# serycjon/MFT

Hardware: AMD Instinct MI355X
Metric: tracked frames/sec at 512x512, 12 RAFT iters; flow EPE vs reference (higher is better)
Workload: dtype f32 (update-block products as split fp16 x 3 on the fp16 matrix cores, fp32 accumulation; error per product <= ~2^-23, see DESIGN.md section 4 and parity below); 1 GPU; MFT.track on synthetic 512x512 video, deltas [inf,1,2,4,8,16,32], 7/7.00/7 (min/mean/max) flow pairs per timed frame, 12 RAFT iters, seeded synthetic weights (BASELINE.json configs[1]); parallelism=single GPU, frames_resident_in_hbm=True, preroll_frames=32

## Files before the change

include/mftx.h:

```cpp
#ifndef MFTX_H
#define MFTX_H

#include <stddef.h>
#include <stdint.h>

#ifdef __cplusplus
extern "C" {
#endif

#define MFTX_VERSION 400

#define MFTX_E_ARG (-1)
#define MFTX_E_ALIGN (-2)
#define MFTX_E_WORKSPACE (-3)
#define MFTX_E_STATE (-4)

#define MFTX_MAX_CANDIDATES 16

int mftx_version(void);
const char *mftx_last_error_string(void);

#define MFTX_PROFILE_CATEGORIES 14
int mftx_profile_begin(void);
int mftx_profile_end(double *ms, double *work, long long *count, int n);

int mftx_corr_pyramid(const float *f1, const float *f2, int P, int C, int h, int w,
                      float *lvl0, float *lvl1, float *lvl2, float *lvl3, void *stream);
int mftx_corr_pyramid_split(const float *f1, const float *f2, int P, int C, int h, int w,
                            float *lvl0, float *lvl1, float *lvl2, float *lvl3, float *f2_scratch, void *stream);
int mftx_corr_pyramid_layout(int h, int w, long long *stride, int *block_grid);

int mftx_corr_lookup(const float *lvl0, const float *lvl1, const float *lvl2, const float *lvl3,
                     const float *coords, int P, int h, int w, int r,
                     float *out, int ld_out, void *stream);

#define MFTX_LOOKUP_CONVC1_WEIGHT_BYTES 393216
int mftx_pack_lookup_convc1_weights(const float *wpk, int ld_w, void *wfused, void *stream);
int mftx_corr_lookup_convc1(const float *lvl0, const float *lvl1, const float *lvl2, const float *lvl3,
                            const float *coords, int P, int h, int w, const void *wfused, const float *bias,
                            float *out, int ld_out, int out_split, void *stream);

#define MFTX_FLOW_BRANCH_WEIGHT_BYTES 352256
int mftx_pack_flow_branch_weights(const float *w98, const float *w2pk, void *wflow, void *stream);
int mftx_flow_branch(const float *coords, int P, int h, int w, const void *wflow, const float *b1, const float *b2,
                     float *out, int ld_out, float *hx, int ld_hx, void *stream);

int mftx_fmap_pyramid(const float *f2, int P, int C, int h, int w, float *lvl1, float *lvl2, float *lvl3, void *stream);
int mftx_corr_lookup_ondemand(const float *f1, const float *f2l0, const float *f2l1, const float *f2l2, const float *f2l3,
                              const float *coords, int P, int C, int h, int w, int r,
                              float *out, int ld_out, void *stream);

typedef struct mftx_conv_desc {
    const float *a0; int lda0; int c0;
    const float *a1; int lda1; int c1;
    const float *wpk; const float *bias;
    float *out; int ldo;
    int P, h, w;
    int N;
    int kh, kw;
    int act;
    float out_scale;
    const float *addend; int ld_addend;
    int stride, hin, win, pad_y, pad_x, residual_mode;
    int arith;
    int a_split, out_split;
} mftx_conv_desc;
#define MFTX_ARITH_F32 0
#define MFTX_ARITH_SPLIT 1
int mftx_conv2d(const mftx_conv_desc *d, void *stream);
int mftx_conv2d_tile(const mftx_conv_desc *d, int tile, void *stream);

int mftx_pack_tile_conv_weights(const float *wpk, int N, int taps, int cin, int cin_pad, void *wtile, void *stream);
int mftx_tile_conv2d(const mftx_conv_desc *d, const void *wtile, void *stream);
#define MFTX_OU_HEADS_WTILE_BYTES 6635520
int mftx_pack_ou_heads_weights(const float *w1pk, int cin_pad, const float *w2pk, void *wtile, void *wproj, void *stream);
int mftx_ou_heads(const float *a_split, int lda, int P, int h, int w, const void *wtile, const float *b1, const void *wproj, const float *b2,
                  float *T, float *out, int ld_out, void *stream);
int mftx_gru_half(const float *h_in, int ld_hin, const float *motion, int ld_mo, const void *wzr, const void *wq, const float *pre_zr,
                  const float *pre_q, float *z, const float *hf_in, float *hf_out, float *h_out, int ld_hout, int P, int h, int w, int pass,
                  void *stream);
int mftx_tile_conv_fills_chip(int P, int h, int w);
#define MFTX_FLOW_HEAD_WEIGHT_BYTES 32768
int mftx_pack_flow_head_weights(const float *w2pk, void *wproj, void *stream);
int mftx_flow_head(const float *hsplit, int ld_h, int P, int h, int w, const void *wtile, const float *b1, const void *wproj,
                   const float *b2, float *T, float *delta, float *coords, void *stream);
int mftx_split_weights(const float *wpk, void *out, long long n_floats, void *stream);
#define MFTX_SPLIT_LIMIT 65504.0f
int mftx_count_not_below(const float *x, long long n, float limit, unsigned *count, void *stream);

typedef struct mftx_raft mftx_raft;
#define MFTX_RAFT_NUM_WEIGHTS 34
int mftx_raft_create(const float *const *weights, int n_weights, mftx_raft **out);
void mftx_raft_destroy(mftx_raft *r);
size_t mftx_raft_workspace_bytes(int P, int h, int w);
int mftx_raft_set_ondemand(mftx_raft *r, int on);
int mftx_raft_set_split_weights(mftx_raft *r, const void *const *split, int n);
int mftx_raft_arith(const mftx_raft *r);
int mftx_raft_set_lookup_fused(mftx_raft *r, const void *wfused);
int mftx_raft_set_flow_fused(mftx_raft *r, const void *wflow);
int mftx_raft_set_tile_weights(mftx_raft *r, const void *const *tile, int n);
int mftx_raft_set_flow_head(mftx_raft *r, const void *wproj);
int mftx_raft_set_ou_heads(mftx_raft *r, const void *wtile, const void *wproj);
int mftx_raft_set_coords_trace(mftx_raft *r, float *trace);
#define MFTX_RAFT_OPT_FORK 0
#define MFTX_RAFT_OPT_PRESPLIT 1
#define MFTX_RAFT_OPT_GROUP 2
#define MFTX_RAFT_OPT_FUSE_LOOKUP 3
#define MFTX_RAFT_OPT_GRAPH 4
#define MFTX_RAFT_OPT_FUSE_FLOW 5
#define MFTX_RAFT_OPT_TILE_CONV 6
#define MFTX_RAFT_OPT_FUSE_HEAD 7
#define MFTX_RAFT_OPT_TILE_VOLUME 8
#define MFTX_RAFT_OPT_FUSE_GRU 9
#define MFTX_RAFT_OPT_TILE_CELLS 10
#define MFTX_RAFT_OPT_FUSE_OU 11
#define MFTX_RAFT_OPT_TILE_CONV2P 12
int mftx_raft_set_option(mftx_raft *r, int option, int value);
#define MFTX_RAFT_PLAN_FIELDS 14
#define MFTX_FLOW_FUSED 0
#define MFTX_FLOW_SIDE 1
#define MFTX_FLOW_FIRST 2
#define MFTX_FLOW_AFTER_LOOKUP 3
#define MFTX_FLOW_WITH_LOOKUP 4
int mftx_raft_plan(const mftx_raft *r, int P, int h, int w, int ctx_supplied, int *out, int n);
int mftx_raft_set_nonfinite_counter(mftx_raft *r, unsigned *counter);
int mftx_raft_clear_graphs(mftx_raft *r);
int mftx_raft_graph_stats(const mftx_raft *r, unsigned long long *captures, unsigned long long *replays);
size_t mftx_raft_workspace_bytes_for(const mftx_raft *r, int P, int h, int w);
int mftx_raft_workspace_layout(int P, int h, int w, size_t *offsets, int n);
int mftx_raft_workspace_layout_for(const mftx_raft *r, int P, int h, int w, size_t *offsets, int n);
int mftx_raft_refine(mftx_raft *r, int P, int h, int w, int iters,
                     const float *fmap1, const float *fmap2, const float *net, const float *inp,
                     const float *flow_init,
                     int pad_left, int pad_right, int pad_top, int pad_bottom,
                     float *flow, float *occl, float *sigma, float *packed, float *flow_lr,
                     void *workspace, size_t workspace_bytes, void *stream);
int mftx_raft_refine_gather(mftx_raft *r, int P, int h, int w, int iters, const float *const *fmap1,
                            const float *const *fmap2, const float *const *net, const float *const *inp,
                            const float *flow_init, int pad_left, int pad_right, int pad_top, int pad_bottom,
                            float *flow, float *occl, float *sigma, float *packed, float *flow_lr_out,
                            void *workspace, size_t workspace_bytes, void *stream);
size_t mftx_raft_frame_prepare_bytes(int h, int w);
int mftx_raft_frame_prepare(mftx_raft *r, int h, int w, const float *fmap, const float *inp, float *ctx_zr1, float *ctx_q1,
                            float *ctx_zr2, float *ctx_q2, void *fmap_split, void *scratch, size_t scratch_bytes, void *stream);
int mftx_raft_refine_gather_ex(mftx_raft *r, int P, int h, int w, int iters, const float *const *fmap1,
                               const float *const *fmap2, const float *const *net, const float *const *inp,
                               const float *const *ctx_parts, const void *const *fmap1_split, const void *fmap2_split,
                               const float *flow_init, int pad_left, int pad_right, int pad_top, int pad_bottom,
                               float *flow, float *occl, float *sigma, float *packed, float *flow_lr_out,
                               void *workspace, size_t workspace_bytes, void *stream);
int mftx_volume_query_split(const float *in, void *out, long long n_floats, void *stream);

typedef struct mftx_encoder mftx_encoder;
int mftx_encoder_create(const float *const *weights, int n_weights, int instance_norm, mftx_encoder **out);
int mftx_encoder_set_split_weights(mftx_encoder *e, const void *const *split, int n);
int mftx_encoder_set_graph(mftx_encoder *e, int on);
void mftx_encoder_destroy(mftx_encoder *e);
size_t mftx_encoder_workspace_bytes(int H0, int W0);
int mftx_encoder_forward(mftx_encoder *e, const uint8_t *img, int H0, int W0, float *out0, float *out1,
                         void *workspace, size_t workspace_bytes, void *stream);
int mftx_encoder_prep(const uint8_t *img, int H0, int W0, float *out, void *stream);
size_t mftx_instance_norm_workspace_bytes(int C);
int mftx_instance_norm(float *x, int rows, int C, const float *res, int mode, int split, void *workspace,
                       size_t workspace_bytes, void *stream);

int mftx_convex_upsample(const float *flow_lr, const float *ou, int ld_ou, const float *mask,
                         int P, int h, int w,
                         int pad_left, int pad_right, int pad_top, int pad_bottom,
                         float *flow, float *occl, float *sigma, float *packed, void *stream);

int mftx_chain(const float *flowL, const float *occlL, const float *sigmaL,
               const float *flowR, const float *occlR, const float *sigmaR,
               int H, int W, float *flowO, float *occlO, float *sigmaO, void *stream);

int mftx_warp_backward(const float *flow, const float *img, int C, int H, int W, float *out, void *stream);

int mftx_select(int K, const float *const *flow, const float *const *occl, const float *const *sigma,
                float thr, int H, int W,
                float *flowO, float *occlO, float *sigmaO, int8_t *chosen, void *stream);

int mftx_chain_select(int K,
                      const float *const *flowL, const float *const *occlL, const float *const *sigmaL,
                      const float *const *flowR, const float *const *occlR, const float *const *sigmaR,
                      float thr, int H, int W,
                      float *flowO, float *occlO, float *sigmaO, int8_t *chosen, void *stream);

int mftx_chain_select_packed(int K,
                             const float *const *flowL, const float *const *occlL, const float *const *sigmaL,
                             const float *const *packedR,
                             float thr, int H, int W,
                             float *flowO, float *occlO, float *sigmaO, int8_t *chosen, void *stream);

int mftx_chain_select_multi(int T, const int *K,
                            const float *const *flowL, const float *const *occlL, const float *const *sigmaL,
                            const float *const *packedR,
                            float thr, int H, int W,
                            float *const *flowO, float *const *occlO, float *const *sigmaO, int8_t *const *chosen,
                            void *stream);

int mftx_sample_points(int T, const float *const *flow, const float *const *occl, const float *const *sigma,
                       int H, int W, int N, const int *tmpl, const float *xy,
                       float *table, long long row_stride, int column, void *stream);

#define MFTX_SPLAT_F32 0
#define MFTX_SPLAT_U8 1
int mftx_splat_forward(const float *flow, const void *img, int img_dtype, const uint8_t *mask, int C, int H, int W,
                       int S, int V, long long *acc, void *stream);

int mftx_splat_resolve(long long *acc, int C, int H, int W, int V, float fill, int clear, float *out, void *stream);

int mftx_overlay_edit(const float *flow, const float *occl, const uint8_t *edit, const uint8_t *frame, int H, int W,
                      int S, float alpha_div, long long *acc, uint8_t *out, void *stream);

int mftx_overlay_dots(const uint8_t *frame, uint8_t *out, int H, int W, const float *table, long long row_stride,
                      int N, double radius, int b, int g, int r, void *stream);

size_t mftx_quantize_workspace_bytes(void);
int mftx_quantize_u16(const float *x, long long n, uint16_t *q, float *lohi,
                      void *workspace, size_t workspace_bytes, void *stream);
int mftx_dequantize_u16(const uint16_t *q, long long n, float lo, float hi, float *x, void *stream);

size_t mftx_trackstore_workspace_bytes(void);
int mftx_trackstore_append(const float *flow, const float *occl, const float *sigma, int H, int W,
                           uint16_t *packed, float *lohi, void *workspace, size_t workspace_bytes, void *stream);

size_t mftx_trackstore_append_multi_workspace_bytes(int T);
int mftx_trackstore_append_multi(int T, const float *const *flow, const float *const *occl, const float *const *sigma,
                                 int H, int W, uint16_t *const *packed, float *const *lohi,
                                 void *workspace, size_t workspace_bytes, void *stream);

int mftx_trackstore_unpack(const uint16_t *packed, const float *lohi, int H, int W,
                           float *flow, float *occl, float *sigma, void *stream);

int mftx_trackstore_query(const uint16_t *const *chunks, const float *const *lohi_chunks, int n_chunks, int frames_per_chunk,
                          const int *slots, int T, int H, int W, int N, const float *xy,
                          float *table, long long row_stride, int column0, void *stream);

int mftx_trackstore_locate(const uint16_t *const *frames, const float *const *lohis, const int *group_start, int G,
                           const int *order, const int *group_of, int H, int W, int N, const float *xy,
                           float occlusion_threshold, unsigned long long *keys, float *table, int *cell, void *stream);

int mftx_trackstore_invert(const uint16_t *const *frames, const float *const *lohis, int G, int H, int W,
                           float occlusion_threshold, unsigned long long *keys ,
                           float *table, int *cell, void *stream);

int mftx_trackstore_invert_atlas(const uint16_t *const *frames, const float *const *lohis, const int *first_of ,
                                 const int *rank_of , int G, int J, int H, int W, float occlusion_threshold,
                                 unsigned long long *keys , float *table, int *cell, int *entry, void *stream);

int mftx_copy_bytes(const void *src, void *dst, long long n, void *stream);

int mftx_png_unfilter(uint8_t *rows, int height, int row_bytes, int bpp);

#ifdef __cplusplus
}
#endif
#endif
```

mft_amd/_lib.py:

```python
from __future__ import annotations

import ctypes as C
import os
from pathlib import Path

_HERE = Path(__file__).resolve().parent
LIB_PATH = _HERE / "libmftx.so"

MAX_CANDIDATES = 16
NUM_RAFT_WEIGHTS = 34
LOOKUP_CONVC1_WEIGHT_BYTES = 393216
FLOW_BRANCH_WEIGHT_BYTES = 352256
FLOW_HEAD_WEIGHT_BYTES = 32768
OU_HEADS_WTILE_BYTES = 6635520
SPLIT_LIMIT = 65504.0


class ConvDesc(C.Structure):
    _fields_ = [("a0", C.c_void_p), ("lda0", C.c_int), ("c0", C.c_int),
                ("a1", C.c_void_p), ("lda1", C.c_int), ("c1", C.c_int),
                ("wpk", C.c_void_p), ("bias", C.c_void_p),
                ("out", C.c_void_p), ("ldo", C.c_int),
                ("P", C.c_int), ("h", C.c_int), ("w", C.c_int),
                ("N", C.c_int), ("kh", C.c_int), ("kw", C.c_int),
                ("act", C.c_int), ("out_scale", C.c_float),
                ("addend", C.c_void_p), ("ld_addend", C.c_int),
                ("stride", C.c_int), ("hin", C.c_int), ("win", C.c_int), ("pad_y", C.c_int), ("pad_x", C.c_int),
                ("residual_mode", C.c_int), ("arith", C.c_int), ("a_split", C.c_int), ("out_split", C.c_int)]


_PP = C.POINTER(C.c_void_p)

SIGNATURES = {
    "mftx_version": (C.c_int, []),
    "mftx_last_error_string": (C.c_char_p, []),
    "mftx_profile_begin": (C.c_int, []),
    "mftx_profile_end": (C.c_int, [C.POINTER(C.c_double), C.POINTER(C.c_double), C.POINTER(C.c_longlong), C.c_int]),
    "mftx_corr_pyramid": (C.c_int, [C.c_void_p, C.c_void_p, C.c_int, C.c_int, C.c_int, C.c_int,
                                    C.c_void_p, C.c_void_p, C.c_void_p, C.c_void_p, C.c_void_p]),
    "mftx_corr_pyramid_split": (C.c_int, [C.c_void_p, C.c_void_p, C.c_int, C.c_int, C.c_int, C.c_int,
                                          C.c_void_p, C.c_void_p, C.c_void_p, C.c_void_p, C.c_void_p, C.c_void_p]),
    "mftx_corr_pyramid_layout": (C.c_int, [C.c_int, C.c_int, C.POINTER(C.c_longlong), C.POINTER(C.c_int)]),
    "mftx_corr_lookup": (C.c_int, [C.c_void_p] * 5 + [C.c_int] * 4 + [C.c_void_p, C.c_int, C.c_void_p]),
    "mftx_fmap_pyramid": (C.c_int, [C.c_void_p] + [C.c_int] * 4 + [C.c_void_p] * 4),
    "mftx_corr_lookup_ondemand": (C.c_int, [C.c_void_p] * 6 + [C.c_int] * 5 + [C.c_void_p, C.c_int, C.c_void_p]),
    "mftx_raft_set_ondemand": (C.c_int, [C.c_void_p, C.c_int]),
    "mftx_raft_workspace_bytes_for": (C.c_size_t, [C.c_void_p, C.c_int, C.c_int, C.c_int]),
    "mftx_conv2d": (C.c_int, [C.POINTER(ConvDesc), C.c_void_p]),
    "mftx_conv2d_tile": (C.c_int, [C.POINTER(ConvDesc), C.c_int, C.c_void_p]),
    "mftx_encoder_set_split_weights": (C.c_int, [C.c_void_p, _PP, C.c_int]),
    "mftx_raft_set_split_weights": (C.c_int, [C.c_void_p, _PP, C.c_int]),
    "mftx_raft_arith": (C.c_int, [C.c_void_p]),
    "mftx_raft_set_lookup_fused": (C.c_int, [C.c_void_p, C.c_void_p]),
    "mftx_raft_set_flow_fused": (C.c_int, [C.c_void_p, C.c_void_p]),
    "mftx_raft_set_tile_weights": (C.c_int, [C.c_void_p, _PP, C.c_int]),
    "mftx_raft_set_flow_head": (C.c_int, [C.c_void_p, C.c_void_p]),
    "mftx_raft_set_ou_heads": (C.c_int, [C.c_void_p, C.c_void_p, C.c_void_p]),
    "mftx_pack_ou_heads_weights": (C.c_int, [C.c_void_p, C.c_int, C.c_void_p, C.c_void_p, C.c_void_p, C.c_void_p]),
    "mftx_ou_heads": (C.c_int, [C.c_void_p, C.c_int, C.c_int, C.c_int, C.c_int, C.c_void_p, C.c_void_p, C.c_void_p, C.c_void_p, C.c_void_p,
                                C.c_void_p, C.c_int, C.c_void_p]),
    "mftx_pack_flow_head_weights": (C.c_int, [C.c_void_p, C.c_void_p, C.c_void_p]),
    "mftx_flow_head": (C.c_int, [C.c_void_p, C.c_int, C.c_int, C.c_int, C.c_int] + [C.c_void_p] * 8),
    "mftx_pack_tile_conv_weights": (C.c_int, [C.c_void_p, C.c_int, C.c_int, C.c_int, C.c_int, C.c_void_p, C.c_void_p]),
    "mftx_tile_conv2d": (C.c_int, [C.POINTER(ConvDesc), C.c_void_p, C.c_void_p]),
    "mftx_pack_flow_branch_weights": (C.c_int, [C.c_void_p, C.c_void_p, C.c_void_p, C.c_void_p]),
    "mftx_flow_branch": (C.c_int, [C.c_void_p, C.c_int, C.c_int, C.c_int, C.c_void_p, C.c_void_p, C.c_void_p, C.c_void_p,
                                   C.c_int, C.c_void_p, C.c_int, C.c_void_p]),
    "mftx_raft_set_option": (C.c_int, [C.c_void_p, C.c_int, C.c_int]),
    "mftx_raft_plan": (C.c_int, [C.c_void_p, C.c_int, C.c_int, C.c_int, C.c_int, C.POINTER(C.c_int), C.c_int]),
    "mftx_raft_set_coords_trace": (C.c_int, [C.c_void_p, C.c_void_p]),
    "mftx_gru_half": (C.c_int, [C.c_void_p, C.c_int, C.c_void_p, C.c_int, C.c_void_p, C.c_void_p, C.c_void_p, C.c_void_p, C.c_void_p, C.c_void_p,
                                C.c_void_p, C.c_void_p, C.c_int, C.c_int, C.c_int, C.c_int, C.c_int, C.c_void_p]),
    "mftx_tile_conv_fills_chip": (C.c_int, [C.c_int, C.c_int, C.c_int]),
    "mftx_raft_clear_graphs": (C.c_int, [C.c_void_p]),
    "mftx_raft_set_nonfinite_counter": (C.c_int, [C.c_void_p, C.c_void_p]),
    "mftx_raft_graph_stats": (C.c_int, [C.c_void_p, C.POINTER(C.c_ulonglong), C.POINTER(C.c_ulonglong)]),
    "mftx_pack_lookup_convc1_weights": (C.c_int, [C.c_void_p, C.c_int, C.c_void_p, C.c_void_p]),
    "mftx_corr_lookup_convc1": (C.c_int, [C.c_void_p] * 5 + [C.c_int] * 3 + [C.c_void_p, C.c_void_p, C.c_void_p,
                                                                            C.c_int, C.c_int, C.c_void_p]),
    "mftx_split_weights": (C.c_int, [C.c_void_p, C.c_void_p, C.c_longlong, C.c_void_p]),
    "mftx_count_not_below": (C.c_int, [C.c_void_p, C.c_longlong, C.c_float, C.c_void_p, C.c_void_p]),
    "mftx_raft_create": (C.c_int, [_PP, C.c_int, C.POINTER(C.c_void_p)]),
    "mftx_raft_destroy": (None, [C.c_void_p]),
    "mftx_raft_workspace_bytes": (C.c_size_t, [C.c_int, C.c_int, C.c_int]),
    "mftx_raft_workspace_layout": (C.c_int, [C.c_int, C.c_int, C.c_int, C.POINTER(C.c_size_t), C.c_int]),
    "mftx_raft_workspace_layout_for": (C.c_int, [C.c_void_p, C.c_int, C.c_int, C.c_int, C.POINTER(C.c_size_t), C.c_int]),
    "mftx_raft_refine": (C.c_int, [C.c_void_p, C.c_int, C.c_int, C.c_int, C.c_int,
                                   C.c_void_p, C.c_void_p, C.c_void_p, C.c_void_p, C.c_void_p,
                                   C.c_int, C.c_int, C.c_int, C.c_int,
                                   C.c_void_p, C.c_void_p, C.c_void_p, C.c_void_p, C.c_void_p,
                                   C.c_void_p, C.c_size_t, C.c_void_p]),
    "mftx_raft_refine_gather": (C.c_int, [C.c_void_p, C.c_int, C.c_int, C.c_int, C.c_int,
                                          _PP, _PP, _PP, _PP, C.c_void_p,
                                          C.c_int, C.c_int, C.c_int, C.c_int,
                                          C.c_void_p, C.c_void_p, C.c_void_p, C.c_void_p, C.c_void_p,
                                          C.c_void_p, C.c_size_t, C.c_void_p]),
    "mftx_raft_refine_gather_ex": (C.c_int, [C.c_void_p, C.c_int, C.c_int, C.c_int, C.c_int,
                                             _PP, _PP, _PP, _PP, _PP, _PP, C.c_void_p, C.c_void_p,
                                             C.c_int, C.c_int, C.c_int, C.c_int,
                                             C.c_void_p, C.c_void_p, C.c_void_p, C.c_void_p, C.c_void_p,
                                             C.c_void_p, C.c_size_t, C.c_void_p]),
    "mftx_raft_frame_prepare_bytes": (C.c_size_t, [C.c_int, C.c_int]),
    "mftx_raft_frame_prepare": (C.c_int, [C.c_void_p, C.c_int, C.c_int] + [C.c_void_p] * 8 + [C.c_size_t, C.c_void_p]),
    "mftx_volume_query_split": (C.c_int, [C.c_void_p, C.c_void_p, C.c_longlong, C.c_void_p]),
    "mftx_encoder_create": (C.c_int, [_PP, C.c_int, C.c_int, C.POINTER(C.c_void_p)]),
    "mftx_encoder_destroy": (None, [C.c_void_p]),
    "mftx_encoder_set_graph": (C.c_int, [C.c_void_p, C.c_int]),
    "mftx_encoder_workspace_bytes": (C.c_size_t, [C.c_int, C.c_int]),
    "mftx_encoder_forward": (C.c_int, [C.c_void_p, C.c_void_p, C.c_int, C.c_int, C.c_void_p, C.c_void_p,
                                       C.c_void_p, C.c_size_t, C.c_void_p]),
    "mftx_encoder_prep": (C.c_int, [C.c_void_p, C.c_int, C.c_int, C.c_void_p, C.c_void_p]),
    "mftx_instance_norm_workspace_bytes": (C.c_size_t, [C.c_int]),
    "mftx_instance_norm": (C.c_int, [C.c_void_p, C.c_int, C.c_int, C.c_void_p, C.c_int, C.c_int, C.c_void_p, C.c_size_t, C.c_void_p]),
    "mftx_convex_upsample": (C.c_int, [C.c_void_p, C.c_void_p, C.c_int, C.c_void_p] + [C.c_int] * 7
                             + [C.c_void_p] * 5),
    "mftx_chain": (C.c_int, [C.c_void_p] * 6 + [C.c_int, C.c_int] + [C.c_void_p] * 4),
    "mftx_warp_backward": (C.c_int, [C.c_void_p, C.c_void_p, C.c_int, C.c_int, C.c_int, C.c_void_p, C.c_void_p]),
    "mftx_select": (C.c_int, [C.c_int, _PP, _PP, _PP, C.c_float, C.c_int, C.c_int] + [C.c_void_p] * 5),
    "mftx_chain_select": (C.c_int, [C.c_int] + [_PP] * 6 + [C.c_float, C.c_int, C.c_int] + [C.c_void_p] * 5),
    "mftx_chain_select_packed": (C.c_int, [C.c_int] + [_PP] * 4 + [C.c_float, C.c_int, C.c_int] + [C.c_void_p] * 5),
    "mftx_chain_select_multi": (C.c_int, [C.c_int, C.POINTER(C.c_int)] + [_PP] * 4 + [C.c_float, C.c_int, C.c_int] + [_PP] * 4
                                + [C.c_void_p]),
    "mftx_sample_points": (C.c_int, [C.c_int, _PP, _PP, _PP, C.c_int, C.c_int, C.c_int, C.c_void_p, C.c_void_p,
                                     C.c_void_p, C.c_longlong, C.c_int, C.c_void_p]),
    "mftx_splat_forward": (C.c_int, [C.c_void_p, C.c_void_p, C.c_int, C.c_void_p, C.c_int, C.c_int, C.c_int, C.c_int, C.c_int,
                                     C.c_void_p, C.c_void_p]),
    "mftx_splat_resolve": (C.c_int, [C.c_void_p, C.c_int, C.c_int, C.c_int, C.c_int, C.c_float, C.c_int, C.c_void_p, C.c_void_p]),
    "mftx_overlay_edit": (C.c_int, [C.c_void_p, C.c_void_p, C.c_void_p, C.c_void_p, C.c_int, C.c_int, C.c_int, C.c_float,
                                    C.c_void_p, C.c_void_p, C.c_void_p]),
    "mftx_overlay_dots": (C.c_int, [C.c_void_p, C.c_void_p, C.c_int, C.c_int, C.c_void_p, C.c_longlong, C.c_int, C.c_double,
                                    C.c_int, C.c_int, C.c_int, C.c_void_p]),
    "mftx_quantize_workspace_bytes": (C.c_size_t, []),
    "mftx_quantize_u16": (C.c_int, [C.c_void_p, C.c_longlong, C.c_void_p, C.c_void_p, C.c_void_p, C.c_size_t, C.c_void_p]),
    "mftx_dequantize_u16": (C.c_int, [C.c_void_p, C.c_longlong, C.c_float, C.c_float, C.c_void_p, C.c_void_p]),
    "mftx_trackstore_workspace_bytes": (C.c_size_t, []),
    "mftx_trackstore_append": (C.c_int, [C.c_void_p, C.c_void_p, C.c_void_p, C.c_int, C.c_int, C.c_void_p, C.c_void_p,
                                         C.c_void_p, C.c_size_t, C.c_void_p]),
    "mftx_trackstore_append_multi_workspace_bytes": (C.c_size_t, [C.c_int]),
    "mftx_trackstore_append_multi": (C.c_int, [C.c_int, _PP, _PP, _PP, C.c_int, C.c_int, _PP, _PP, C.c_void_p, C.c_size_t,
                                               C.c_void_p]),
    "mftx_trackstore_invert_atlas": (C.c_int, [C.c_void_p, C.c_void_p, C.c_void_p, C.c_void_p, C.c_int, C.c_int, C.c_int, C.c_int,
                                               C.c_float, C.c_void_p, C.c_void_p, C.c_void_p, C.c_void_p, C.c_void_p]),
    "mftx_trackstore_unpack": (C.c_int, [C.c_void_p, C.c_void_p, C.c_int, C.c_int, C.c_void_p, C.c_void_p, C.c_void_p,
                                         C.c_void_p]),
    "mftx_trackstore_query": (C.c_int, [_PP, _PP, C.c_int, C.c_int, C.c_void_p, C.c_int, C.c_int, C.c_int, C.c_int, C.c_void_p,
                                        C.c_void_p, C.c_longlong, C.c_int, C.c_void_p]),
    "mftx_trackstore_locate": (C.c_int, [C.c_void_p, C.c_void_p, C.c_void_p, C.c_int, C.c_void_p, C.c_void_p, C.c_int, C.c_int,
                                         C.c_int, C.c_void_p, C.c_float, C.c_void_p, C.c_void_p, C.c_void_p, C.c_void_p]),
    "mftx_trackstore_invert": (C.c_int, [C.c_void_p, C.c_void_p, C.c_int, C.c_int, C.c_int, C.c_float, C.c_void_p, C.c_void_p,
                                         C.c_void_p, C.c_void_p]),
    "mftx_png_unfilter":(C.c_int, [C.c_void_p, C.c_int, C.c_int, C.c_int]),
    "mftx_copy_bytes": (C.c_int, [C.c_void_p, C.c_void_p, C.c_longlong, C.c_void_p]),
}

_lib = None


class MftxError(RuntimeError):
    pass


def load():
    global _lib
    if _lib is not None:
        return _lib
    path = Path(os.environ.get("MFTX_LIB", LIB_PATH))
    if not path.exists():
        raise MftxError(f"{path} not found: build it with `python -c 'import __graft_entry__ as g; g.build()'` "
                        "(there is no CPU fallback for the MFT hot path)")
    lib = C.CDLL(str(path))
    for name, (res, args) in SIGNATURES.items():
        fn = getattr(lib, name)
        fn.restype = res
        fn.argtypes = args
    _lib = lib
    return lib


def check(code, what):
    if code != 0:
        msg = load().mftx_last_error_string().decode(errors="replace")
        raise MftxError(f"{what} failed ({code}): {msg}")


def ptr_array(ptrs):
    arr = (C.c_void_p * len(ptrs))(*ptrs)
    return C.cast(arr, _PP), arr
```

mft_amd/csrc/flow_branch.hip:

```cpp
#include "common.h"
#include "profile.h"
#include "device_prims.h"

namespace mftx {

constexpr int FB_TH = 8, FB_TW = 16;
constexpr int FB_HW = FB_TW + 2;
constexpr int FB_HCELLS = (FB_TH + 2) * FB_HW;
constexpr int FB_CELL = 528;
constexpr int FB_FCOLS = 26;
constexpr int FB_FROW = 28;
constexpr int FB_OFF_FLOW = 192 * FB_CELL;
constexpr int FB_FLOW_BYTES = 4 * 2 * 16 * FB_FROW * 4;
constexpr int FB_RED_ROW = 68;
constexpr int FB_LDS = 4 * 128 * FB_RED_ROW * 4;
static_assert(FB_OFF_FLOW + FB_FLOW_BYTES <= FB_LDS, "stage 3 is the largest user of LDS");
constexpr unsigned FB_W1_BYTES = 7 * 4 * 2 * 1024;
constexpr unsigned FB_W2_BYTES = 2 * 4 * 18 * 2 * 1024;
constexpr unsigned FB_WBYTES = FB_W1_BYTES + FB_W2_BYTES;

#ifdef MFTX_LF_TRACE
__device__ unsigned long long fb_trace_buf[8][16];
#define FB_T(code) do { if (blockIdx.x == 0 && tcount < 16) { unsigned long long t_; asm volatile("s_memtime %0\n\ts_waitcnt lgkmcnt(0)" : "=s"(t_) :: "memory"); \
                        if ((threadIdx.x & 63) == 0) fb_trace_buf[threadIdx.x >> 6][tcount] = ((unsigned long long)(code) << 56) | (t_ & 0x00ffffffffffffffull); ++tcount; } } while (0)
#else
#define FB_T(code) do { } while (0)
#endif

struct FlowBranchArgs {
    const float *coords;
    const void *wf;
    const float *b1, *b2;
    float *out; int ld_out;
    float *hx; int ld_hx;
    const float *T, *b2h;
    float *coords_out, *delta_out;
    int P, h, w, tiles_x, tiles_y;
};

__global__ __launch_bounds__(512, 2) void flow_branch_kernel(FlowBranchArgs p) {
    extern __shared__ __attribute__((aligned(16))) unsigned char fb_lds[];
    unsigned char *lds = fb_lds;
    const int tid = (int)threadIdx.x, lane = tid & 63, wv = __builtin_amdgcn_readfirstlane(tid >> 6);
    const int tile = (int)blockIdx.x;
    const int tx_ = tile % p.tiles_x, ty_ = (tile / p.tiles_x) % p.tiles_y, img = tile / (p.tiles_x * p.tiles_y);
    const int x0 = tx_ * FB_TW, y0 = ty_ * FB_TH;
    const long long img_base = (long long)img * p.h * p.w;
    const float k2048 = __builtin_bit_cast(float, __builtin_amdgcn_readfirstlane(0x45000000));
    const uint4 *__restrict__ wf = reinterpret_cast<const uint4 *>(p.wf);
#ifdef MFTX_LF_TRACE
    int tcount = 0;
#endif
    FB_T(1);

    const int j1 = wv & 3;
    f16x8 w1h[7], w1l[7];
#pragma unroll
    for (int g = 0; g < 7; ++g) {
        const uint4 *src = wf + ((g * 4 + j1) * 2) * 64 + lane;
        w1h[g] = __builtin_bit_cast(f16x8, src[0]);
        w1l[g] = __builtin_bit_cast(f16x8, src[64]);
    }
    f32x4 bias1[4];
#pragma unroll
    for (int b = 0; b < 4; ++b) bias1[b] = *reinterpret_cast<const f32x4 *>(p.b1 + 32 * j1 + 8 * b + 4 * (lane >> 5));

    unsigned *fsp = reinterpret_cast<unsigned *>(lds + FB_OFF_FLOW);
    if (tid < 16 * FB_FCOLS) {
        const int r = tid / FB_FCOLS, c = tid - r * FB_FCOLS;
        const int yy = y0 - 4 + r, xx = x0 - 4 + c;
        float2 f = make_float2(0.f, 0.f);
        unsigned hw = 0u, lw = 0u;
        if (yy >= 0 && yy < p.h && xx >= 0 && xx < p.w) {
            const long long cell = img_base + (long long)yy * p.w + xx;
            float2 cd = *reinterpret_cast<const float2 *>(p.coords + 2 * cell);
            if (p.T) {
                float sx = 0.f, sy = 0.f;
#pragma unroll
                for (int dy = 0; dy < 3; ++dy)
#pragma unroll
                    for (int dx = 0; dx < 3; ++dx) {
                        const int ny = yy + dy - 1, nx = xx + dx - 1;
                        if (ny >= 0 && ny < p.h && nx >= 0 && nx < p.w) {
                            const float2 t = *reinterpret_cast<const float2 *>(p.T + (cell + (long long)(dy - 1) * p.w + (dx - 1)) * 18 + 2 * (3 * dy + dx));
                            sx += t.x;
                            sy += t.y;
                        }
                    }
                const float dlx = sx + p.b2h[0], dly = sy + p.b2h[1];
                cd.x += dlx;
                cd.y += dly;
                if (r >= 4 && r < 4 + FB_TH && c >= 4 && c < 4 + FB_TW) {
                    *reinterpret_cast<float2 *>(p.coords_out + 2 * cell) = cd;
                    *reinterpret_cast<float2 *>(p.delta_out + 2 * cell) = make_float2(dlx, dly);
                }
            }
            f.x = cd.x - (float)xx;
            f.y = cd.y - (float)yy;
            const unsigned sx = split_halves(f.x), sy = split_halves(f.y);
            hw = (sx & 0xffffu) | (sy << 16);
            lw = (sx >> 16) | (sy & 0xffff0000u);
            if (p.hx && r >= 4 && r < 4 + FB_TH && c >= 4 && c < 4 + FB_TW) {
                char *dst = reinterpret_cast<char *>(p.hx + cell * p.ld_hx) + split_row_offset(382);
                *reinterpret_cast<unsigned *>(dst) = hw;
                *reinterpret_cast<unsigned *>(dst + 16) = lw;
            }
        }
#pragma unroll
        for (int sft = 0; sft < 4; ++sft) {
            if (c >= sft) {
                fsp[((sft * 2 + 0) * 16 + r) * FB_FROW + c - sft] = hw;
                fsp[((sft * 2 + 1) * 16 + r) * FB_FROW + c - sft] = lw;
            }
            if (c >= FB_FCOLS - 4 && c - sft + 4 < FB_FROW) {
                fsp[((sft * 2 + 0) * 16 + r) * FB_FROW + c - sft + 4] = 0u;
                fsp[((sft * 2 + 1) * 16 + r) * FB_FROW + c - sft + 4] = 0u;
            }
        }
    }
    FB_T(2);
    lds_barrier();
    FB_T(3);

    const float inv2048 = 1.f / 2048.f;
    {
#pragma unroll 1
        for (int mi = 0; mi < 3; ++mi) {
            const int i = (wv >> 2) + 2 * mi;
            const int m = 32 * i + (lane & 31), mc = m < FB_HCELLS ? m : FB_HCELLS - 1;
            const int ry = mc / FB_HW, rx = mc - ry * FB_HW;
            const int c0 = rx + 4 * (lane >> 5), sft = c0 & 3;
            const unsigned char *arow = lds + FB_OFF_FLOW + (((sft * 2) * 16 + ry) * FB_FROW + (c0 - sft)) * 4;
            const unsigned padmask = (lane >> 5) ? 0u : 0xffffffffu;
            f32x16 acc1, accx1;
#pragma unroll
            for (int r = 0; r < 16; ++r) { acc1[r] = 0.f; accx1[r] = 0.f; }
            u32x4 ahw[7], alw[7];
#pragma unroll
            for (int g = 0; g < 7; ++g) {
                ahw[g] = *reinterpret_cast<const u32x4 *>(arow + g * FB_FROW * 4);
                alw[g] = *reinterpret_cast<const u32x4 *>(arow + (16 + g) * FB_FROW * 4);
            }
#pragma unroll
            for (int g = 0; g < 7; ++g) {
                ahw[g][3] &= padmask;
                alw[g][3] &= padmask;
                const f16x8 ah = __builtin_bit_cast(f16x8, ahw[g]), al = __builtin_bit_cast(f16x8, alw[g]);
                acc1 = mfma_f16(w1h[g], ah, acc1);
                accx1 = mfma_f16(w1l[g], ah, accx1);
                accx1 = mfma_f16(w1h[g], al, accx1);
            }
            FB_T(4);
            const int yy = y0 - 1 + ry, xx = x0 - 1 + rx;
            const unsigned keep = (m < FB_HCELLS && yy >= 0 && yy < p.h && xx >= 0 && xx < p.w) ? 0xffffffffu : 0u;
            unsigned char *cellp = lds + m * FB_CELL + (4 * j1) * 32 + (lane >> 5) * 8;
#pragma unroll
            for (int b = 0; b < 4; ++b) {
                float v[4];
#pragma unroll
                for (int e = 0; e < 4; ++e) {
                    const float t = acc1[4 * b + e] + accx1[4 * b + e] * inv2048 + bias1[b][e];
                    v[e] = (t + __builtin_fabsf(t)) * 0.5f;
                }
                unsigned h0, l0, h1, l1;
                split_pair(v[0], v[1], k2048, h0, l0);
                split_pair(v[2], v[3], k2048, h1, l1);
                *reinterpret_cast<uint2 *>(cellp + b * 32) = make_uint2(h0 & keep, h1 & keep);
                *reinterpret_cast<uint2 *>(cellp + b * 32 + 16) = make_uint2(l0 & keep, l1 & keep);
            }
            FB_T(5);
        }
    }
    lds_barrier();
    FB_T(6);

    const int nt = wv & 1, kq = wv >> 1;
    const uint4 *__restrict__ w2 = wf + FB_W1_BYTES / 16 + (nt * 4 + kq) * 18 * 128 + lane;
    f32x16 acc[4], accx[4];
#pragma unroll
    for (int i = 0; i < 4; ++i)
#pragma unroll
        for (int r = 0; r < 16; ++r) { acc[i][r] = 0.f; accx[i][r] = 0.f; }
    const unsigned char *abase[4];
    {
        const int r = lane & 31;
#pragma unroll
        for (int i = 0; i < 4; ++i)
            abase[i] = lds + ((2 * i + (r >> 4)) * FB_HW + (r & 15)) * FB_CELL + (lane >> 5) * 32 + kq * 128;
    }
    constexpr int PF = 3;
    uint4 bq[PF][2];
#pragma unroll
    for (int s = 0; s < PF; ++s) { bq[s][0] = w2[s * 128]; bq[s][1] = w2[s * 128 + 64]; }
    f16x8 ah[2][4], al[2][4];
    auto read_a = [&](int s, int set) {
        const int tap = s >> 1, gg = s & 1;
        const int off = ((tap / 3) * FB_HW + tap % 3) * FB_CELL + gg * 64;
#pragma unroll
        for (int i = 0; i < 4; ++i) {
            ah[set][i] = *reinterpret_cast<const f16x8 *>(abase[i] + off);
            al[set][i] = *reinterpret_cast<const f16x8 *>(abase[i] + off + 16);
        }
    };
    read_a(0, 0);
#pragma unroll
    for (int s = 0; s < 18; ++s) {
        const int set = s & 1;
        const f16x8 bh = __builtin_bit_cast(f16x8, bq[s % PF][0]), bl = __builtin_bit_cast(f16x8, bq[s % PF][1]);
        __builtin_amdgcn_sched_barrier(0);
        if (s + 1 < 18) read_a(s + 1, set ^ 1);
        if (s + PF < 18) { bq[s % PF][0] = w2[(s + PF) * 128]; bq[s % PF][1] = w2[(s + PF) * 128 + 64]; }
        __builtin_amdgcn_sched_barrier(0);
#pragma unroll
        for (int i = 0; i < 4; ++i) acc[i] = mfma_f16(bh, ah[set][i], acc[i]);
#pragma unroll
        for (int i = 0; i < 4; ++i) accx[i] = mfma_f16(bl, ah[set][i], accx[i]);
#pragma unroll
        for (int i = 0; i < 4; ++i) accx[i] = mfma_f16(bh, al[set][i], accx[i]);
        __builtin_amdgcn_sched_barrier(0);
    }
    FB_T(7);
    lds_barrier();

    float *red = reinterpret_cast<float *>(lds);
#pragma unroll
    for (int i = 0; i < 4; ++i)
#pragma unroll
        for (int b = 0; b < 4; ++b) {
            f32x4 v;
#pragma unroll
            for (int e = 0; e < 4; ++e) v[e] = acc[i][4 * b + e] + accx[i][4 * b + e] * inv2048;
            *reinterpret_cast<f32x4 *>(red + (kq * 128 + 32 * i + (lane & 31)) * FB_RED_ROW + 32 * nt + 8 * b + 4 * (lane >> 5)) = v;
        }
    FB_T(8);
    lds_barrier();
    FB_T(9);
#pragma unroll
    for (int it = 0; it < 2; ++it) {
        const int item = tid + 512 * it, m = item >> 3, g8 = item & 7;
        const int yy = y0 + (m >> 4), xx = x0 + (m & 15);
        const float *src = red + m * FB_RED_ROW + 8 * g8;
        f32x4 u = *reinterpret_cast<const f32x4 *>(src), v = *reinterpret_cast<const f32x4 *>(src + 4);
#pragma unroll
        for (int q = 1; q < 4; ++q) {
            u += *reinterpret_cast<const f32x4 *>(src + q * 128 * FB_RED_ROW);
            v += *reinterpret_cast<const f32x4 *>(src + q * 128 * FB_RED_ROW + 4);
        }
        const f32x4 bu = *reinterpret_cast<const f32x4 *>(p.b2 + 8 * g8), bv = *reinterpret_cast<const f32x4 *>(p.b2 + 8 * g8 + 4);
#pragma unroll
        for (int e = 0; e < 4; ++e) { u[e] = relu_keep_nan(u[e] + bu[e]); v[e] = relu_keep_nan(v[e] + bv[e]); }
        f16x8 hi, lo;
        split8(u, v, k2048, hi, lo);
        if (yy < p.h && xx < p.w) {
            const long long cell = img_base + (long long)yy * p.w + xx;
            uint4 *dst = reinterpret_cast<uint4 *>(reinterpret_cast<char *>(p.out + cell * p.ld_out) + g8 * 32);
            dst[0] = __builtin_bit_cast(uint4, hi);
            dst[1] = __builtin_bit_cast(uint4, lo);
        }
    }
    FB_T(10);
}

#ifdef MFTX_LF_TRACE
extern "C" int mftx_debug_fb_trace(unsigned long long *out) {
    if (hipMemcpyFromSymbol(out, HIP_SYMBOL(fb_trace_buf), sizeof(unsigned long long) * 8 * 16) != hipSuccess) return -1;
    unsigned long long z[8 * 16] = {};
    return hipMemcpyToSymbol(HIP_SYMBOL(fb_trace_buf), z, sizeof z) == hipSuccess ? 0 : -1;
}
#endif

__global__ void pack_flow_branch_kernel(const float *__restrict__ w98, const float *__restrict__ w2pk, uint4 *__restrict__ out) {
    const int idx = (int)(blockIdx.x * blockDim.x + threadIdx.x);
    const int n1 = (int)(FB_W1_BYTES / 16), n2 = (int)(FB_W2_BYTES / 16);
    if (idx >= n1 + n2) return;
    float v[8];
    int part;
    if (idx < n1) {
        const int lane = idx & 63, j = (idx >> 7) & 3, g = idx >> 9;
        part = (idx >> 6) & 1;
        const int n = 32 * j + (lane & 31);
#pragma unroll
        for (int e = 0; e < 8; ++e) {
            const int s = 8 * (lane >> 5) + e;
            v[e] = s < 14 ? w98[(g * 14 + s) * 128 + n] : 0.f;
        }
    } else {
        const int k = idx - n1;
        const int lane = k & 63, step = (k >> 7) % 18, kq = ((k >> 7) / 18) & 3, nt = (k >> 7) / 72;
        part = (k >> 6) & 1;
        const int tap = step >> 1, g = 2 * kq + (step & 1);
        const int n = 32 * nt + (lane & 31);
#pragma unroll
        for (int e = 0; e < 8; ++e) v[e] = w2pk[((long long)n * 9 + tap) * 128 + 16 * g + 8 * (lane >> 5) + e];
    }
    unsigned w[4];
#pragma unroll
    for (int e = 0; e < 4; ++e) {
        const unsigned a = split_halves(v[2 * e]), b = split_halves(v[2 * e + 1]);
        w[e] = part ? ((a >> 16) | (b & 0xffff0000u)) : ((a & 0xffffu) | (b << 16));
    }
    out[idx] = make_uint4(w[0], w[1], w[2], w[3]);
}

int launch_pack_flow_branch(const float *w98, const float *w2pk, void *out, hipStream_t s) {
    const int n = (int)(FB_WBYTES / 16);
    hipLaunchKernelGGL(pack_flow_branch_kernel, dim3((n + 255) / 256), dim3(256), 0, s, w98, w2pk, reinterpret_cast<uint4 *>(out));
    return check_launch("pack_flow_branch");
}

int launch_flow_branch(const float *coords, int P, int h, int w, const void *wf, const float *b1, const float *b2, float *out,
                       int ld_out, float *hx, int ld_hx, hipStream_t s, const float *T, const float *b2h, float *coords_out, float *delta_out) {
    if (T && (!b2h || !coords_out || !delta_out || coords_out == coords || (reinterpret_cast<uintptr_t>(T) & 7) || (reinterpret_cast<uintptr_t>(coords_out) & 7) ||
              (reinterpret_cast<uintptr_t>(delta_out) & 7)))
        return fail(MFTX_E_ARG, "flow_branch: a pending flow-head update needs its bias, a SECOND coordinate buffer and a delta buffer, 8-byte aligned");
    if (!coords || !wf || !b1 || !b2 || !out) return fail(MFTX_E_ARG, "flow_branch: null pointer");
    if (P <= 0 || h <= 0 || w <= 0) return fail(MFTX_E_ARG, "flow_branch: bad sizes");
    if (ld_out < 64 || ld_out % 8 || (reinterpret_cast<uintptr_t>(out) & 31) || (hx && (ld_hx < 384 || ld_hx % 8 || (reinterpret_cast<uintptr_t>(hx) & 31))))
        return fail(MFTX_E_ALIGN, "flow_branch: split-form rows are 32-byte aligned with strides in multiples of 8");
    if (!aligned16(wf) || !aligned16(b2) || (reinterpret_cast<uintptr_t>(coords) & 7)) return fail(MFTX_E_ALIGN, "flow_branch: weights / bias / coordinates misaligned");
    FlowBranchArgs a{coords, wf, b1, b2, out, ld_out, hx, ld_hx, T, b2h, coords_out, delta_out, P, h, w, cdiv(w, FB_TW), cdiv(h, FB_TH)};
    const long long tiles = (long long)P * a.tiles_x * a.tiles_y;
    if (tiles > 0x7fffffffLL) return fail(MFTX_E_ARG, "flow_branch: too many tiles");
    static bool attr_set = false;
    if (!attr_set) {
        if (hipFuncSetAttribute(reinterpret_cast<const void *>(flow_branch_kernel), hipFuncAttributeMaxDynamicSharedMemorySize, FB_LDS) != hipSuccess)
            return fail(MFTX_E_STATE, "flow_branch: cannot reserve %d bytes of LDS", FB_LDS);
        attr_set = true;
    }
    ProfScope prof(PC_FLOW_FUSED, s, 2.0 * P * h * w * (98.0 * 128 + 1152.0 * 64));
    hipLaunchKernelGGL(flow_branch_kernel, dim3((unsigned)tiles), dim3(512), FB_LDS, s, a);
    return check_launch("flow_branch");
}

}
```

mft_amd/csrc/raft_engine.hip:

```cpp
#include "common.h"
#include "profile.h"
#include "motion_front.h"
#include "graph_cache.h"
#include <cstdlib>
#include <new>

namespace mftx {


struct InitGather { int on; PairPtrs netp, inpp; };
struct CtxTable { const float **table; const float *own[4]; int supplied; PairPtrs parts[4]; };
__global__ void init_state_kernel(const float *__restrict__ net, const float *__restrict__ inp,
                                  const float *__restrict__ flow_init, float *hx, float *hf, float *coords1, int M, int h,
                                  int w, InitGather ga, CtxTable ct) {
    const long long i = (long long)blockIdx.x * blockDim.x + threadIdx.x;
    if (i >= (long long)M * 64) return;
    if (ct.table != nullptr && i < (long long)(M / (h * w)) * 4) {
        const int b = (int)(i >> 2), k = (int)(i & 3);
        ct.table[i] = ct.supplied ? ct.parts[k].p[b] : ct.own[k] + (long long)b * h * w * ((k & 1) ? 128 : 256);
    }
    const int m = (int)(i >> 6), q = (int)(i & 63);
    if (ga.on) {
        const int b = m / (h * w);
        net = ga.netp.p[b] - (long long)b * h * w * 128;
        inp = ga.inpp.p[b] - (long long)b * h * w * 128;
    }
    const float4 v = (q < 32) ? reinterpret_cast<const float4 *>(net)[(long long)m * 32 + q]
                              : reinterpret_cast<const float4 *>(inp)[(long long)m * 32 + (q - 32)];
    if (hf != nullptr) {
        store_split4v(hx + (long long)m * 384, 4 * q, v);
        if (q < 32) reinterpret_cast<float4 *>(hf + (long long)m * 128)[q] = v;
    } else {
        reinterpret_cast<float4 *>(hx + (long long)m * 384)[q] = v;
    }
    if (q == 0) {
        const int rem = m % (h * w);
        float cx = (float)(rem % w), cy = (float)(rem / w);
        if (flow_init != nullptr) {
            cx += flow_init[2 * (long long)m];
            cy += flow_init[2 * (long long)m + 1];
        }
        coords1[2 * (long long)m] = cx;
        coords1[2 * (long long)m + 1] = cy;
    }
}

__global__ __launch_bounds__(256) void convf1_kernel(ConvF1Args q) {
    __shared__ __attribute__((aligned(16))) float patch[2][7][48];
    const int half = threadIdx.x >> 7;
    convf1_strip(q, blockIdx.x * 2 + half, patch[half], threadIdx.x & 127);
}

__global__ __launch_bounds__(256) void lookup_convf1_kernel(LookupArgs lp, ConvF1Args q, int lookup_blocks, int f1_blocks) {
    __shared__ __attribute__((aligned(16))) float patch[2][7][48];
    const int total = lookup_blocks + f1_blocks;
    const int b = blockIdx.x;
    const int f_lo = (int)((long long)b * f1_blocks / total), f_hi = (int)((long long)(b + 1) * f1_blocks / total);
    if (f_hi > f_lo) {
        const int half = threadIdx.x >> 7;
        convf1_strip(q, f_lo * 2 + half, patch[half], threadIdx.x & 127);
    } else {
        lookup_block_body<2>(lp, b - f_lo, lookup_blocks);
    }
}

__global__ void ou_gather_kernel(const float *__restrict__ hx, const float *__restrict__ corr, int ld_corr,
                                 const float *__restrict__ coords1, const float *__restrict__ delta,
                                 float *__restrict__ ouin, float *__restrict__ flow_lr, int M, int h, int w, int split) {
    const long long i = (long long)blockIdx.x * blockDim.x + threadIdx.x;
    if (i >= (long long)M * 178) return;
    const int m = (int)(i / 178), q = (int)(i - (long long)m * 178);
    float4 v;
    if (split) {
        if (q < 64) v = load_split4(hx + (long long)m * 384, 4 * q);
        else if (q < 145) v = reinterpret_cast<const float4 *>(corr + (long long)m * ld_corr)[q - 64];
        else if (q == 145) {
            const int rem = m % (h * w);
            const float fx = coords1[2 * (long long)m] - (float)(rem % w);
            const float fy = coords1[2 * (long long)m + 1] - (float)(rem / w);
            v = make_float4(fx, fy, delta[2 * (long long)m], delta[2 * (long long)m + 1]);
            flow_lr[2 * (long long)m] = fx;
            flow_lr[2 * (long long)m + 1] = fy;
        } else v = load_split4(hx + (long long)m * 384 + 256, 4 * (q - 146));
        store_split4v(ouin + (long long)m * 712, 4 * q, v);
        return;
    }
    if (q < 64) v = reinterpret_cast<const float4 *>(hx + (long long)m * 384)[q];
    else if (q < 145) v = reinterpret_cast<const float4 *>(corr + (long long)m * ld_corr)[q - 64];
    else if (q == 145) {
        const int rem = m % (h * w);
        const float fx = coords1[2 * (long long)m] - (float)(rem % w);
        const float fy = coords1[2 * (long long)m + 1] - (float)(rem / w);
        v = make_float4(fx, fy, delta[2 * (long long)m], delta[2 * (long long)m + 1]);
        flow_lr[2 * (long long)m] = fx;
        flow_lr[2 * (long long)m + 1] = fy;
    } else v = reinterpret_cast<const float4 *>(hx + (long long)m * 384 + 256)[q - 146];
    reinterpret_cast<float4 *>(ouin + (long long)m * 712)[q] = v;
}

enum WeightSlot {
    W_CONVC1, B_CONVC1, W_CONVC2, B_CONVC2, W_CONVF1, B_CONVF1, W_CONVF2, B_CONVF2, W_CONV, B_CONV,
    W_ZR1_DYN, W_ZR1_INP, B_ZR1, W_Q1_DYN, W_Q1_INP, B_Q1, W_ZR2_DYN, W_ZR2_INP, B_ZR2, W_Q2_DYN, W_Q2_INP, B_Q2,
    W_FH1, B_FH1, W_FH2, B_FH2, W_MASK0, B_MASK0, W_MASK2, B_MASK2,
    W_OU1, B_OU1, W_OU2, B_OU2, W_COUNT
};

struct Workspace {
    float *lvl[4];
    float *f2l[3];
    float *coords1, *corr, *cor1, *corflo, *flo1, *hx, *z, *rh, *fh, *delta, *mask, *ouin, *ouh, *ou, *flow_lr;
    float *pre_zr[2], *pre_q[2];
    float *f2s;
    float *hf;
    float *hb, *hfb;
    const float **ctx;
    int ld_corr;
    size_t bytes;
};

static Workspace carve(void *base, int P, int h, int w, bool ondemand = false, bool split = false) {
    Workspace ws{};
    const size_t N = (size_t)h * w, M = (size_t)P * N;
    size_t off = 0;
    auto take = [&](size_t floats) {
        float *p = base ? reinterpret_cast<float *>(static_cast<char *>(base) + off) : nullptr;
        off += (floats * sizeof(float) + 255) & ~size_t(255);
        return p;
    };
    const PyramidLayout L = pyramid_layout(h, w);
    for (int l = 0; l < 4; ++l) ws.lvl[l] = take(ondemand ? 0 : M * (size_t)L.stride[l]);
    for (int l = 1; l < 4; ++l) ws.f2l[l - 1] = take(ondemand ? (size_t)P * (h >> l) * (w >> l) * 256 : 0);
    ws.coords1 = take(M * 2);
    ws.ld_corr = 324;
    ws.corr = take(M * ws.ld_corr);
    ws.cor1 = take(M * 256);
    ws.corflo = take(M * 256);
    ws.flo1 = take(M * 128);
    ws.hx = take(M * 384);
    ws.z = take(M * 128);
    ws.rh = take(M * 128);
    ws.fh = take(M * 256);
    ws.delta = take(M * 2);
    ws.mask = take(M * 576);
    ws.ouin = take(M * 712);
    ws.ouh = take(M * 256);
    ws.ou = take(M * 4);
    ws.flow_lr = take(M * 2);
    for (int pass = 0; pass < 2; ++pass) { ws.pre_zr[pass] = take(M * 256); ws.pre_q[pass] = take(M * 128); }
    ws.f2s = take(ondemand || !split ? 0 : M * 256);
    ws.hf = take(split ? M * 128 : 0);
    ws.hb = take(split ? M * 128 : 0);
    ws.hfb = take(split ? M * 128 : 0);
    ws.ctx = reinterpret_cast<const float **>(take(split ? (size_t)P * 8 : 0));
    ws.bytes = off;
    return ws;
}

}

using namespace mftx;

static constexpr uint32_t RAFT_MAGIC = 0x4d465458;
struct mftx_raft {
    uint32_t magic = RAFT_MAGIC;
    int ondemand = 0;
    int arith = MFTX_ARITH_F32;
    const float *w[W_COUNT] = {};
    const float *wg[W_COUNT] = {};
    hipStream_t side = nullptr;
    hipEvent_t ev_fork = nullptr, ev_join = nullptr;
    float *coords_trace = nullptr;
    GraphCache *graphs = nullptr;
    const void *wfused = nullptr;
    const void *wflow = nullptr;
    const void *wproj = nullptr;
    const void *wt[W_COUNT] = {};
    const void *wou = nullptr, *wouproj = nullptr;
    int opt[13] = { -1,  1,  1,  1,  1,  1,  1,
                    1,  1,  1,  0,  1,  1};
    unsigned *nonfinite = nullptr;
};
static_assert(MFTX_RAFT_OPT_TILE_CONV2P == 12, "mftx_raft::opt lists one default per option");
static constexpr int GEMM_SLOTS[] = {W_CONVC1, W_CONVC2, W_CONVF2, W_CONV, W_ZR1_DYN, W_ZR1_INP, W_Q1_DYN, W_Q1_INP,
                                     W_ZR2_DYN, W_ZR2_INP, W_Q2_DYN, W_Q2_INP, W_FH1, W_MASK0, W_MASK2, W_OU1};

extern "C" int mftx_raft_create(const float *const *weights, int n_weights, mftx_raft **out) {
    if (!weights || !out) return fail(MFTX_E_ARG, "raft_create: null pointer");
    if (n_weights != W_COUNT) return fail(MFTX_E_ARG, "raft_create: expected %d weight tensors, got %d", (int)W_COUNT, n_weights);
    for (int i = 0; i < W_COUNT; ++i) {
        if (!weights[i]) return fail(MFTX_E_ARG, "raft_create: weight %d is null", i);
        if (!aligned16(weights[i])) return fail(MFTX_E_ALIGN, "raft_create: weight %d not 16-byte aligned", i);
    }
    mftx_raft *r = new (std::nothrow) mftx_raft;
    if (!r) return fail(MFTX_E_ARG, "raft_create: out of host memory");
    r->graphs = new (std::nothrow) GraphCache;
    for (int i = 0; i < W_COUNT; ++i) r->w[i] = r->wg[i] = weights[i];
    *out = r;
    return 0;
}

extern "C" void mftx_raft_destroy(mftx_raft *r) {
    if (r && r->magic == RAFT_MAGIC) {
        r->magic = 0;
        if (r->ev_fork) (void)hipEventDestroy(r->ev_fork);
        if (r->ev_join) (void)hipEventDestroy(r->ev_join);
        if (r->side) (void)hipStreamDestroy(r->side);
        delete r->graphs;
        delete r;
    }
}

static int ensure_side_stream(mftx_raft *r) {
    if (r->side) return 0;
    hipError_t e = hipStreamCreateWithFlags(&r->side, hipStreamNonBlocking);
    if (e == hipSuccess) e = hipEventCreateWithFlags(&r->ev_fork, hipEventDisableTiming);
    if (e == hipSuccess) e = hipEventCreateWithFlags(&r->ev_join, hipEventDisableTiming);
    if (e != hipSuccess) return fail((int)e, "raft_refine: side stream: %s", hipGetErrorString(e));
    return 0;
}

extern "C" size_t mftx_raft_workspace_bytes(int P, int h, int w) {
    if (P <= 0 || h <= 0 || w <= 0) return 0;
    return carve(nullptr, P, h, w).bytes;
}

extern "C" int mftx_raft_set_ondemand(mftx_raft *r, int on) {
    if (!r || r->magic != RAFT_MAGIC) return fail(MFTX_E_STATE, "raft_set_ondemand: bad handle");
    r->ondemand = on ? 1 : 0;
    if (r->graphs) r->graphs->clear();
    return 0;
}

extern "C" int mftx_raft_set_split_weights(mftx_raft *r, const void *const *split, int n) {
    if (!r || r->magic != RAFT_MAGIC) return fail(MFTX_E_STATE, "raft_set_split_weights: bad handle");
    if (r->graphs) r->graphs->clear();
    if (!split) {
        for (int i = 0; i < W_COUNT; ++i) r->wg[i] = r->w[i];
        r->arith = MFTX_ARITH_F32;
        return 0;
    }
    if (n != W_COUNT) return fail(MFTX_E_ARG, "raft_set_split_weights: expected %d slots, got %d", (int)W_COUNT, n);
    for (int slot : GEMM_SLOTS) {
        if (!split[slot]) return fail(MFTX_E_ARG, "raft_set_split_weights: slot %d (a GEMM layer) is null", slot);
        if (!aligned16(split[slot])) return fail(MFTX_E_ALIGN, "raft_set_split_weights: slot %d not 16-byte aligned", slot);
    }
    for (int slot : GEMM_SLOTS) r->wg[slot] = static_cast<const float *>(split[slot]);
    r->arith = MFTX_ARITH_SPLIT;
    return 0;
}

extern "C" int mftx_raft_set_lookup_fused(mftx_raft *r, const void *wfused) {
    if (!r || r->magic != RAFT_MAGIC) return fail(MFTX_E_STATE, "raft_set_lookup_fused: bad handle");
    if (wfused && !aligned16(wfused)) return fail(MFTX_E_ALIGN, "raft_set_lookup_fused: weights not 16-byte aligned");
    r->wfused = wfused;
    if (r->graphs) r->graphs->clear();
    return 0;
}

extern "C" int mftx_raft_set_flow_fused(mftx_raft *r, const void *wflow) {
    if (!r || r->magic != RAFT_MAGIC) return fail(MFTX_E_STATE, "raft_set_flow_fused: bad handle");
    if (wflow && !aligned16(wflow)) return fail(MFTX_E_ALIGN, "raft_set_flow_fused: weights not 16-byte aligned");
    r->wflow = wflow;
    if (r->graphs) r->graphs->clear();
    return 0;
}

extern "C" int mftx_raft_set_tile_weights(mftx_raft *r, const void *const *tile, int n) {
    if (!r || r->magic != RAFT_MAGIC) return fail(MFTX_E_STATE, "raft_set_tile_weights: bad handle");
    if (r->graphs) r->graphs->clear();
    if (!tile) { for (int i = 0; i < W_COUNT; ++i) r->wt[i] = nullptr; return 0; }
    if (n != W_COUNT) return fail(MFTX_E_ARG, "raft_set_tile_weights: expected %d slots, got %d", (int)W_COUNT, n);
    for (int i = 0; i < W_COUNT; ++i)
        if (tile[i] && !aligned16(tile[i])) return fail(MFTX_E_ALIGN, "raft_set_tile_weights: slot %d not 16-byte aligned", i);
    for (int i = 0; i < W_COUNT; ++i) r->wt[i] = tile[i];
    return 0;
}

extern "C" int mftx_raft_set_flow_head(mftx_raft *r, const void *wproj) {
    if (!r || r->magic != RAFT_MAGIC) return fail(MFTX_E_STATE, "raft_set_flow_head: bad handle");
    if (wproj && !aligned16(wproj)) return fail(MFTX_E_ALIGN, "raft_set_flow_head: weights not 16-byte aligned");
    r->wproj = wproj;
    if (r->graphs) r->graphs->clear();
    return 0;
}

extern "C" int mftx_raft_set_ou_heads(mftx_raft *r, const void *wtile, const void *wproj) {
    if (!r || r->magic != RAFT_MAGIC) return fail(MFTX_E_STATE, "raft_set_ou_heads: bad handle");
    if ((wtile == nullptr) != (wproj == nullptr)) return fail(MFTX_E_ARG, "raft_set_ou_heads: both weight streams, or neither");
    if (wtile && (!aligned16(wtile) || !aligned16(wproj))) return fail(MFTX_E_ALIGN, "raft_set_ou_heads: weights not 16-byte aligned");
    r->wou = wtile; r->wouproj = wproj;
    if (r->graphs) r->graphs->clear();
    return 0;
}

extern "C" int mftx_raft_set_coords_trace(mftx_raft *r, float *trace) {
    if (!r || r->magic != RAFT_MAGIC) return fail(MFTX_E_STATE, "raft_set_coords_trace: bad handle");
    r->coords_trace = trace;
    return 0;
}

extern "C" int mftx_raft_clear_graphs(mftx_raft *r) {
    if (!r || r->magic != RAFT_MAGIC) return fail(MFTX_E_STATE, "raft_clear_graphs: bad handle");
    if (r->graphs) r->graphs->clear();
    return 0;
}

extern "C" int mftx_raft_set_nonfinite_counter(mftx_raft *r, unsigned *counter) {
    if (!r || r->magic != RAFT_MAGIC) return fail(MFTX_E_STATE, "raft_set_nonfinite_counter: bad handle");
    if (counter && (reinterpret_cast<uintptr_t>(counter) & 3)) return fail(MFTX_E_ALIGN, "raft_set_nonfinite_counter: counter not 4-byte aligned");
    r->nonfinite = counter;
    return 0;
}

extern "C" int mftx_raft_set_option(mftx_raft *r, int option, int value) {
    if (!r || r->magic != RAFT_MAGIC) return fail(MFTX_E_STATE, "raft_set_option: bad handle");
    if (option < 0 || option > MFTX_RAFT_OPT_TILE_CONV2P) return fail(MFTX_E_ARG, "raft_set_option: unknown option %d", option);
    r->opt[option] = value;
    if (r->graphs) r->graphs->clear();
    return 0;
}

extern "C" int mftx_raft_arith(const mftx_raft *r) {
    return (r && r->magic == RAFT_MAGIC) ? r->arith : -1;
}

extern "C" size_t mftx_raft_workspace_bytes_for(const mftx_raft *r, int P, int h, int w) {
    if (!r || r->magic != RAFT_MAGIC || P <= 0 || h <= 0 || w <= 0) return 0;
    return carve(nullptr, P, h, w, r->ondemand != 0, r->arith == MFTX_ARITH_SPLIT).bytes;
}

static int workspace_layout(const mftx_raft *r, int P, int h, int w, size_t *offsets, int n) {
    if (P <= 0 || h <= 0 || w <= 0 || !offsets || n != 19) return fail(MFTX_E_ARG, "workspace_layout: need 19 slots");
    char *base = reinterpret_cast<char *>(uintptr_t(1) << 40);
    Workspace ws = carve(base, P, h, w, r && r->ondemand != 0, r && r->arith == MFTX_ARITH_SPLIT);
    float *ptrs[19] = {ws.lvl[0], ws.lvl[1], ws.lvl[2], ws.lvl[3], ws.coords1, ws.corr, ws.cor1, ws.corflo, ws.flo1,
                       ws.hx, ws.z, ws.rh, ws.fh, ws.delta, ws.mask, ws.ouin, ws.ouh, ws.ou, ws.flow_lr};
    for (int i = 0; i < 19; ++i) offsets[i] = (size_t)(reinterpret_cast<char *>(ptrs[i]) - base);
    return 0;
}
extern "C" int mftx_raft_workspace_layout(int P, int h, int w, size_t *offsets, int n) {
    return workspace_layout(nullptr, P, h, w, offsets, n);
}
extern "C" int mftx_raft_workspace_layout_for(const mftx_raft *r, int P, int h, int w, size_t *offsets, int n) {
    if (!r || r->magic != RAFT_MAGIC) return fail(MFTX_E_STATE, "workspace_layout_for: bad handle");
    return workspace_layout(r, P, h, w, offsets, n);
}

#define TRY(expr) do { int _e = (expr); if (_e) return _e; } while (0)

enum FlowSchedule { FLOW_FUSED = MFTX_FLOW_FUSED, FLOW_SIDE = MFTX_FLOW_SIDE, FLOW_FIRST = MFTX_FLOW_FIRST, FLOW_AFTER_LOOKUP = MFTX_FLOW_AFTER_LOOKUP,
                    FLOW_WITH_LOOKUP = MFTX_FLOW_WITH_LOOKUP };

struct RefinePlan {
    bool SP, fuse_lookup, tiles_on, gru_fused, ctx_supplied, two_pass;
    FlowSchedule flow;
    bool pair_second;
    bool head_fused, defer_update, ou_fused, ou_materialised, use_graph, side_stream;
};

static RefinePlan refine_plan(const mftx_raft &r, int P, int h, int w, bool gather_has_ctx, bool prof, bool trace) {
    const int *opt = r.opt;
    const bool split = r.arith == MFTX_ARITH_SPLIT, ondemand = r.ondemand != 0;
    RefinePlan p{};
    p.SP = split && opt[MFTX_RAFT_OPT_PRESPLIT] != 0;
    p.fuse_lookup = p.SP && !ondemand && r.wfused != nullptr && opt[MFTX_RAFT_OPT_FUSE_LOOKUP] != 0 && lookup_convc1_applicable(P, h, w, 256);
    p.tiles_on = p.SP && opt[MFTX_RAFT_OPT_TILE_CONV] != 0 && (opt[MFTX_RAFT_OPT_TILE_CONV] == 2 ||
                 (tile_conv_fills_chip(P, h, w, 3, 3) && tile_conv_fills_chip(P, h, w, 1, 5) && tile_conv_fills_chip(P, h, w, 5, 1)));
    auto tile_w = [&](int slot) { return p.tiles_on && r.wt[slot] != nullptr; };
    p.gru_fused = tile_w(W_ZR1_DYN) && tile_w(W_Q1_DYN) && tile_w(W_ZR2_DYN) && tile_w(W_Q2_DYN) && opt[MFTX_RAFT_OPT_FUSE_GRU] != 0;
    p.ctx_supplied = gather_has_ctx && p.gru_fused;
    p.two_pass = p.tiles_on && opt[MFTX_RAFT_OPT_TILE_CONV2P] != 0 && r.wt[W_CONVC2] && r.wt[W_CONV];
    const bool grouped = opt[MFTX_RAFT_OPT_GROUP] != 0;
    const int fork = opt[MFTX_RAFT_OPT_FORK];
    const bool fuse_flow = p.SP && r.wflow != nullptr && opt[MFTX_RAFT_OPT_FUSE_FLOW] != 0 && grouped;
    const bool serial = fuse_flow || prof || !grouped || (split && (fork == 0 || fork == 2));
    const bool forked = !serial && split;
    const bool flow_first = !fuse_flow && serial && p.fuse_lookup && fork == 2 && !prof && grouped;
    const bool lookup_alone = p.fuse_lookup || prof || !grouped || ondemand;
    p.flow = fuse_flow ? FLOW_FUSED : forked ? FLOW_SIDE : flow_first ? FLOW_FIRST : lookup_alone ? FLOW_AFTER_LOOKUP : FLOW_WITH_LOOKUP;
    p.pair_second = !forked && grouped && r.arith == MFTX_ARITH_F32;
    p.head_fused = tile_w(W_FH1) && r.wproj != nullptr && opt[MFTX_RAFT_OPT_FUSE_HEAD] != 0;
    p.defer_update = p.head_fused && fuse_flow && opt[MFTX_RAFT_OPT_FUSE_HEAD] != 2 && !trace;
    p.ou_fused = p.tiles_on && r.wou != nullptr && opt[MFTX_RAFT_OPT_FUSE_OU] != 0;
    p.ou_materialised = !p.ou_fused || opt[MFTX_RAFT_OPT_FUSE_OU] == 2;
    p.use_graph = r.graphs && opt[MFTX_RAFT_OPT_GRAPH] != 0 && !prof && !trace && !ondemand;
    p.side_stream = split && fork != 0;
    return p;
}

extern "C" int mftx_raft_plan(const mftx_raft *r, int P, int h, int w, int ctx_supplied, int *out, int n) {
    if (!r || r->magic != RAFT_MAGIC) return fail(MFTX_E_STATE, "raft_plan: bad handle");
    if (P <= 0 || h <= 0 || w <= 0) return fail(MFTX_E_ARG, "raft_plan: need P, h, w >= 1");
    if (!out || n != MFTX_RAFT_PLAN_FIELDS) return fail(MFTX_E_ARG, "raft_plan: need %d slots", MFTX_RAFT_PLAN_FIELDS);
    const RefinePlan p = refine_plan(*r, P, h, w, ctx_supplied != 0, prof_enabled(), r->coords_trace != nullptr);
    const int v[MFTX_RAFT_PLAN_FIELDS] = {p.SP, p.fuse_lookup, p.tiles_on, p.gru_fused, p.ctx_supplied, p.two_pass, (int)p.flow, p.pair_second,
                                          p.head_fused, p.defer_update, p.ou_fused, p.ou_materialised, p.use_graph, p.side_stream};
    for (int i = 0; i < n; ++i) out[i] = v[i];
    return 0;
}

struct RefineGather { PairPtrs f1, f2, net, inp; bool f2_shared; bool has_ctx, has_f1s; PairPtrs ctx[4], f1s; const float *f2s; };

struct Coords { float *cur, *alt; bool pending; };
struct Seg { const float *p; int ld, c; };
struct Out { float *p; int ld, N; };
enum { ACT_NONE, ACT_RELU, ACT_GRU_ZR, ACT_GRU_Q };

struct RefineCall {
    mftx_raft *r;
    const float *const *W, *const *G;
    RefinePlan plan;
    hipStream_t s;
    int P, h, w, iters;
    Workspace ws;
    const float *lv[4];
    const float *fmap1, *f2lv[4];
    float *flow_lr;

    mftx_conv_desc conv_desc(Seg a0, Seg a1, const float *wpk, const float *bias, Out out, int kh, int kw, int act) const {
        mftx_conv_desc d{};
        d.a0 = a0.p; d.lda0 = a0.ld; d.c0 = a0.c; d.a1 = a1.p; d.lda1 = a1.ld; d.c1 = a1.c;
        d.wpk = wpk; d.bias = bias; d.out = out.p; d.ldo = out.ld; d.N = out.N; d.P = P; d.h = h; d.w = w;
        d.kh = kh; d.kw = kw; d.act = act; d.out_scale = 1.f;
        return d;
    }
    mftx_conv_desc gemm(mftx_conv_desc d, bool a = true, bool o = false) const {
        d.arith = r->arith; d.a_split = plan.SP && a; d.out_split = plan.SP && o; return d;
    }
    TileConvLaunch tile_launch(int slot, const float *bias, Seg a0, Seg a1, int N, int kh, int kw, int epi) const {
        TileConvLaunch t{};
        t.a0 = a0.p; t.lda0 = a0.ld; t.a1 = a1.p; t.lda1 = a1.ld; t.cin = a1.p ? 256 : 128; t.wf = r->wt[slot]; t.bias = bias;
        t.P = P; t.h = h; t.w = w; t.N = N; t.kh = kh; t.kw = kw; t.epi = epi;
        t.cells = r->opt[MFTX_RAFT_OPT_TILE_CELLS];
        return t;
    }
    int conv_layer(int slot, const float *bias, Seg a0, Seg a1, Out out, int kh, int kw, int act, bool out_split, const GruEpilogue *g = nullptr,
                   const float *addend = nullptr, int ld_addend = 0) const {
        if (plan.tiles_on && r->wt[slot]) {
            TileConvLaunch t = tile_launch(slot, bias, a0, a1, out.N, kh, kw, act);
            t.addend = addend; t.ld_addend = ld_addend;
            if (!g) { t.out = out.p; t.ldo = out.ld; t.out_split = out_split ? 1 : 0; }
            else {
                t.z = g->z; t.hf = g->hf; t.ld_hf = g->ld_hf;
                if (act == ACT_GRU_ZR) t.rh = g->rh; else { t.hx = g->hx; t.ld_hx = g->ld_hx; }
            }
            return launch_tile_conv(t, s);
        }
        mftx_conv_desc d = gemm(conv_desc(a0, a1, G[slot], bias, out, kh, kw, act), true, out_split);
        d.addend = addend; d.ld_addend = ld_addend;
        return g ? launch_conv_gru(d, *g, s) : launch_conv(d, s);
    }
    int context_parts(const float *inp, int ld, float *const zr[2], float *const q[2]) const {
        for (int pass = 0; pass < 2; ++pass) {
            const int kh = pass ? 5 : 1, kw = pass ? 1 : 5;
            TRY(conv_layer(pass ? W_ZR2_INP : W_ZR1_INP, W[pass ? B_ZR2 : B_ZR1], Seg{inp, ld, 128}, Seg{}, Out{zr[pass], 256, 256}, kh, kw, ACT_NONE, false));
            TRY(conv_layer(pass ? W_Q2_INP : W_Q1_INP, W[pass ? B_Q2 : B_Q1], Seg{inp, ld, 128}, Seg{}, Out{q[pass], 128, 128}, kh, kw, ACT_NONE, false));
        }
        return 0;
    }
    int volume(const float *fmap2, const RefineGather *gather) const {
        if (r->ondemand) return launch_fmap_pyramid(fmap2, P, 256, h, w, ws.f2l, s);
        if (!gather) return launch_corr_pyramid(fmap1, fmap2, P, 256, h, w, ws.lvl, s, r->arith == MFTX_ARITH_SPLIT ? ws.f2s : nullptr, r->opt[MFTX_RAFT_OPT_TILE_VOLUME]);
        const long long pair_floats = (long long)h * w * 256;
        const float *f2s = ws.f2s;
        if (gather->f2_shared && gather->f2s) f2s = gather->f2s;
        else if (gather->f2_shared) TRY(launch_split_weights(gather->f2.p[0], ws.f2s, pair_floats, s));
        else for (int b = 0; b < P; ++b) TRY(launch_split_weights(gather->f2.p[b], ws.f2s + b * pair_floats, pair_floats, s));
        return launch_volume_tile(nullptr, f2s, P, h, w, ws.lvl, s, gather->has_f1s ? &gather->f1s : &gather->f1, gather->f2_shared ? 0 : pair_floats,
                                  gather->has_f1s);
    }
    int init_state(const float *net, const float *inp, const float *flow_init, const RefineGather *gather) const {
        const int M = P * h * w;
        const long long slots = (long long)M * 64;
        ProfScope prof(PC_GLUE, s, 0);
        InitGather ga{};
        if (gather) { ga.on = 1; ga.netp = gather->net; ga.inpp = gather->inp; }
        CtxTable ct{};
        if (plan.gru_fused) {
            ct.table = ws.ctx;
            ct.own[0] = ws.pre_zr[0]; ct.own[1] = ws.pre_q[0]; ct.own[2] = ws.pre_zr[1]; ct.own[3] = ws.pre_q[1];
            ct.supplied = plan.ctx_supplied ? 1 : 0;
            if (plan.ctx_supplied) for (int k = 0; k < 4; ++k) ct.parts[k] = gather->ctx[k];
        }
        hipLaunchKernelGGL(init_state_kernel, dim3((unsigned)((slots + 255) / 256)), dim3(256), 0, s, net, inp,
                           flow_init, ws.hx, plan.SP ? ws.hf : nullptr, ws.coords1, M, h, w, ga, ct);
        return check_launch("init_state");
    }
    int conv256(int slot, const float *bias, const float *in, Out out, const mftx_conv_desc *pair = nullptr) const {
        if (plan.two_pass) return launch_tile_conv2p(in, 256, r->wt[slot], bias, out.p, out.ld, out.N, P, h, w, r->opt[MFTX_RAFT_OPT_TILE_CELLS], s);
        const mftx_conv_desc d = gemm(conv_desc(Seg{in, 256, 256}, Seg{}, G[slot], bias, out, 3, 3, ACT_RELU), true, true);
        return pair ? launch_conv_pair(d, *pair, s) : launch_conv(d, s);
    }
    int corr_branch(const float *coords, bool last, const ConvF1Args *f1 = nullptr, int f1_blocks = 0, const mftx_conv_desc *pair = nullptr) const {
        if (plan.flow == FLOW_WITH_LOOKUP) {
            const LookupArgs la = make_lookup_args(lv, coords, P, h, w, ws.corr, ws.ld_corr);
            const int lookup_blocks = cdiv(cdiv(la.cells, 2), LK_WAVES);
            hipLaunchKernelGGL(lookup_convf1_kernel, dim3(lookup_blocks + f1_blocks), dim3(256), 0, s, la, *f1, lookup_blocks, f1_blocks);
        } else {
            if (plan.fuse_lookup) {
                if (last && plan.flow != FLOW_SIDE) TRY(launch_corr_lookup(lv, coords, P, h, w, ws.corr, ws.ld_corr, s));
                TRY(launch_lookup_convc1(lv, coords, P, h, w, r->wfused, W[B_CONVC1], ws.cor1, 256, 1, s));
            } else if (r->ondemand) TRY(launch_corr_ondemand(fmap1, f2lv, coords, P, h, w, ws.corr, ws.ld_corr, s));
            else TRY(launch_corr_lookup(lv, coords, P, h, w, ws.corr, ws.ld_corr, s));
            if (f1) {
                ProfScope prof(PC_CONVF1, s, 2.0 * P * h * w * 128 * 98);
                hipLaunchKernelGGL(convf1_kernel, dim3(f1_blocks), dim3(256), 0, s, *f1);
            }
        }
        TRY(check_launch("lookup + convf1"));
        if (!plan.fuse_lookup)
            TRY(launch_conv(gemm(conv_desc(Seg{ws.corr, ws.ld_corr, ws.ld_corr}, Seg{}, G[W_CONVC1], W[B_CONVC1], Out{ws.cor1, 256, 256}, 1, 1, ACT_RELU), false, true), s));
        return conv256(W_CONVC2, W[B_CONVC2], ws.cor1, Out{ws.corflo, 256, 192}, pair);
    }
    int motion_encoder(Coords &x, bool last) const {
        const int strips = cdiv(w, F1_CELLS);
        const ConvF1Args f1{x.cur, W[W_CONVF1], W[B_CONVF1], ws.flo1, ws.hx, h, w, strips, P * h * strips, plan.SP ? 1 : 0};
        const int f1_blocks = cdiv(f1.n_strips, 2);
        const Out flo{ws.corflo + 192, 256, 64};
        const mftx_conv_desc f2 = gemm(conv_desc(Seg{ws.flo1, 128, 128}, Seg{}, G[W_CONVF2], W[B_CONVF2], flo, 3, 3, ACT_RELU), true, true);
        switch (plan.flow) {
        case FLOW_FUSED:
            if (x.pending) {
                TRY(launch_flow_branch(x.cur, P, h, w, r->wflow, W[B_CONVF1], W[B_CONVF2], flo.p, flo.ld, ws.hx, 384, s, ws.fh, W[B_FH2], x.alt, ws.delta));
                x = Coords{x.alt, x.cur, false};
            } else TRY(launch_flow_branch(x.cur, P, h, w, r->wflow, W[B_CONVF1], W[B_CONVF2], flo.p, flo.ld, ws.hx, 384, s));
            TRY(corr_branch(x.cur, last));
            break;
        case FLOW_SIDE:
            TRY(ensure_side_stream(r));
            if (hipEventRecord(r->ev_fork, s) != hipSuccess || hipStreamWaitEvent(r->side, r->ev_fork, 0) != hipSuccess)
                return fail(MFTX_E_STATE, "raft_refine: fork onto the side stream failed");
            hipLaunchKernelGGL(convf1_kernel, dim3(f1_blocks), dim3(256), 0, r->side, f1);
            TRY(check_launch("convf1"));
            TRY(launch_conv(f2, r->side));
            if (plan.fuse_lookup && last) TRY(launch_corr_lookup(lv, x.cur, P, h, w, ws.corr, ws.ld_corr, r->side));
            if (hipEventRecord(r->ev_join, r->side) != hipSuccess) return fail(MFTX_E_STATE, "raft_refine: join event failed");
            TRY(corr_branch(x.cur, last));
            if (hipStreamWaitEvent(s, r->ev_join, 0) != hipSuccess) return fail(MFTX_E_STATE, "raft_refine: join failed");
            break;
        case FLOW_FIRST:
            hipLaunchKernelGGL(convf1_kernel, dim3(f1_blocks), dim3(256), 0, s, f1);
            TRY(check_launch("convf1"));
            TRY(launch_conv(f2, s));
            TRY(corr_branch(x.cur, last));
            break;
        case FLOW_AFTER_LOOKUP: case FLOW_WITH_LOOKUP:
            TRY(corr_branch(x.cur, last, &f1, f1_blocks, plan.pair_second ? &f2 : nullptr));
            if (!plan.pair_second) TRY(launch_conv(f2, s));
            break;
        }
        return conv256(W_CONV, W[B_CONV], ws.corflo, Out{ws.hx + 256, 384, 126});
    }
    int gru() const {
        for (int pass = 0; pass < 2; ++pass) {
            const int kh = pass ? 5 : 1, kw = pass ? 1 : 5;
            const int szr = pass ? W_ZR2_DYN : W_ZR1_DYN, sq = pass ? W_Q2_DYN : W_Q1_DYN;
            if (plan.gru_fused) {
                GruHalfLaunch g{};
                g.h_in = pass ? ws.hb : ws.hx; g.ld_hin = pass ? 128 : 384; g.h_out = pass ? ws.hx : ws.hb; g.ld_hout = pass ? 384 : 128;
                g.mo = ws.hx + 256; g.ld_mo = 384; g.wzr = r->wt[szr]; g.wq = r->wt[sq]; g.pre_zr = ws.pre_zr[pass]; g.pre_q = ws.pre_q[pass]; g.ctx = ws.ctx;
                g.z = ws.z; g.hf_in = pass ? ws.hfb : ws.hf; g.hf_out = pass ? ws.hf : ws.hfb; g.P = P; g.h = h; g.w = w; g.pass = pass; g.cells = r->opt[MFTX_RAFT_OPT_TILE_CELLS];
                TRY(launch_gru_half(g, s));
                continue;
            }
            const Seg motion{ws.hx + 256, 384, 128};
            const GruEpilogue g1{1, ws.hx, 384, ws.z, ws.rh, plan.SP ? ws.hf : nullptr, 128}, g2{2, ws.hx, 384, ws.z, ws.rh, plan.SP ? ws.hf : nullptr, 128};
            TRY(conv_layer(szr, nullptr, Seg{ws.hx, 384, 128}, motion, Out{ws.z, 128, 256}, kh, kw, ACT_GRU_ZR, true, &g1, ws.pre_zr[pass], 256));
            TRY(conv_layer(sq, nullptr, Seg{ws.rh, 128, 128}, motion, Out{ws.hx, 384, 128}, kh, kw, ACT_GRU_Q, true, &g2, ws.pre_q[pass], 128));
        }
        return 0;
    }
    int flow_head(Coords &x, bool last) const {
        const Seg hidden{ws.hx, 384, 128};
        if (plan.head_fused) {
            TileConvLaunch t = tile_launch(W_FH1, W[B_FH1], hidden, Seg{}, 256, 3, 3, 4);
            t.wproj = r->wproj; t.tout = ws.fh;
            TRY(launch_tile_conv(t, s));
            if (!last && plan.defer_update) { x.pending = true; return 0; }
            float *dst = last ? ws.coords1 : x.cur;
            TRY(launch_flow_head_sum(ws.fh, W[B_FH2], ws.delta, x.cur, dst, P, h, w, s));
            x.cur = dst;
            return 0;
        }
        TRY(conv_layer(W_FH1, W[B_FH1], hidden, Seg{}, Out{ws.fh, 256, 256}, 3, 3, ACT_RELU, false));
        const mftx_conv_desc fh2 = conv_desc(Seg{ws.fh, 256, 256}, Seg{}, W[W_FH2], W[B_FH2], Out{ws.delta, 2, 2}, 3, 3, ACT_NONE);
        if (!conv_small_applicable(fh2)) return fail(MFTX_E_STATE, "raft_refine: flow-head layer does not fit the small-N kernel");
        return launch_conv_small(fh2, s, x.cur, 2);
    }
    int final_heads(const float *coords) const {
        const int M = P * h * w;
        TRY(conv_layer(W_MASK0, W[B_MASK0], Seg{ws.hx, 384, 128}, Seg{}, Out{ws.fh, 256, 256}, 3, 3, ACT_RELU, true));
        mftx_conv_desc mask2 = gemm(conv_desc(Seg{ws.fh, 256, 256}, Seg{}, G[W_MASK2], W[B_MASK2], Out{ws.mask, 576, 576}, 1, 1, ACT_NONE));
        mask2.out_scale = 0.25f;
        TRY(launch_conv(mask2, s));
        if (plan.ou_materialised) {
            const long long slots = (long long)M * 178;
            ProfScope prof(PC_GLUE, s, 0);
            hipLaunchKernelGGL(ou_gather_kernel, dim3((unsigned)((slots + 255) / 256)), dim3(256), 0, s, ws.hx,
                               ws.corr, ws.ld_corr, coords, ws.delta, ws.ouin, flow_lr, M, h, w, plan.SP ? 1 : 0);
            TRY(check_launch("ou_gather"));
        }
        if (plan.ou_fused) {
            const OuGather ga{ws.hx, ws.corr, ws.ld_corr, coords, ws.delta, flow_lr};
            return launch_ou_heads(plan.ou_materialised ? ws.ouin : nullptr, 712, P, h, w, r->wou, W[B_OU1], r->wouproj, W[B_OU2], ws.ouh, ws.ou, 4, r->opt[MFTX_RAFT_OPT_TILE_CELLS], s,
                                   plan.ou_materialised ? nullptr : &ga);
        }
        TRY(launch_conv(gemm(conv_desc(Seg{ws.ouin, 712, 712}, Seg{}, G[W_OU1], W[B_OU1], Out{ws.ouh, 256, 256}, 3, 3, ACT_RELU)), s));
        return launch_conv(conv_desc(Seg{ws.ouh, 256, 256}, Seg{}, W[W_OU2], W[B_OU2], Out{ws.ou, 4, 3}, 3, 3, ACT_NONE), s);
    }
    int core() const {
        const size_t n = (size_t)P * h * w * 2;
        float *trace = r->coords_trace;
        if (!plan.ctx_supplied) TRY(context_parts(ws.hx + 128, 384, ws.pre_zr, ws.pre_q));
        Coords x{ws.coords1, ws.flo1, false};
        for (int it = 0; it < iters; ++it) {
            const bool last = (it == iters - 1);
            if (trace && hipMemcpyAsync(trace + it * n, x.cur, n * 4, hipMemcpyDeviceToDevice, s) != hipSuccess)
                return fail(MFTX_E_STATE, "raft_refine: coords trace copy failed");
            TRY(motion_encoder(x, last));
            TRY(gru());
            TRY(flow_head(x, last));
        }
        if (trace && hipMemcpyAsync(trace + iters * n, x.cur, n * 4, hipMemcpyDeviceToDevice, s) != hipSuccess)
            return fail(MFTX_E_STATE, "raft_refine: coords trace copy failed");
        return final_heads(x.cur);
    }
};

static int refine_impl(mftx_raft *r, int P, int h, int w, int iters, const float *fmap1, const float *fmap2, const float *net,
                       const float *inp, const float *flow_init, int pad_left, int pad_right, int pad_top, int pad_bottom, float *flow, float *occl,
                       float *sigma, float *packed, float *flow_lr_out, void *workspace, size_t workspace_bytes, void *stream, const RefineGather *gather) {
    if (!r || r->magic != RAFT_MAGIC) return fail(MFTX_E_STATE, "raft_refine: bad handle");
    const bool planar = flow && occl && sigma;
    if (gather) { fmap1 = gather->f1.p[0]; fmap2 = gather->f2.p[0]; net = gather->net.p[0]; inp = gather->inp.p[0]; }
    if (!fmap1 || !fmap2 || !net || !inp || !workspace || (!planar && (flow || occl || sigma || !packed)))
        return fail(MFTX_E_ARG, "raft_refine: null pointer (outputs: flow + occl + sigma, or packed, or both)");
    if (P <= 0 || h < 16 || w < 16 || iters < 1)
        return fail(MFTX_E_ARG, "raft_refine: need P >= 1, h, w >= 16 (level 3 of the pyramid needs >= 2 cells), iters >= 1");
    if ((long long)P * h * w > (1ll << 24)) return fail(MFTX_E_ARG, "raft_refine: batch too large");
    if (!aligned16(fmap1) || !aligned16(fmap2) || !aligned16(net) || !aligned16(inp) || (reinterpret_cast<uintptr_t>(workspace) & 255))
        return fail(MFTX_E_ALIGN, "raft_refine: inputs must be 16-byte and the workspace 256-byte aligned");
    if (pad_left < 0 || pad_right < 0 || pad_top < 0 || pad_bottom < 0 || pad_left + pad_right >= 8 || pad_top + pad_bottom >= 8)
        return fail(MFTX_E_ARG, "raft_refine: bad padding");
    const RefinePlan plan = refine_plan(*r, P, h, w, gather && gather->has_ctx, prof_enabled(), r->coords_trace != nullptr);
    const Workspace ws = carve(workspace, P, h, w, r->ondemand != 0, r->arith == MFTX_ARITH_SPLIT);
    if (ws.bytes > workspace_bytes)
        return fail(MFTX_E_WORKSPACE, "raft_refine: workspace %zu < %zu bytes", workspace_bytes, ws.bytes);
    hipStream_t s = (hipStream_t)stream, caller = s;
    bool proxied = false;
    if (plan.use_graph && s == nullptr) {
        hipStream_t own = r->graphs->proxy.enter(s);
        if (own) { s = own; proxied = true; }
    }
    struct Leave { GraphCache *g; hipStream_t caller; bool on; ~Leave() { if (on) g->proxy.leave(caller); } } leave{r->graphs, caller, proxied};
    const RefineCall c{r, r->w, r->wg, plan, s, P, h, w, iters, ws, {ws.lvl[0], ws.lvl[1], ws.lvl[2], ws.lvl[3]},
                       fmap1, {fmap2, ws.f2l[0], ws.f2l[1], ws.f2l[2]}, flow_lr_out ? flow_lr_out : ws.flow_lr};
    TRY(c.volume(fmap2, gather));
    TRY(c.init_state(net, inp, flow_init, gather));
    if (plan.use_graph) {
        if (plan.side_stream) TRY(ensure_side_stream(r));
        GraphKey key{};
        key.v[0] = (uintptr_t)P; key.v[1] = (uintptr_t)h; key.v[2] = (uintptr_t)w; key.v[3] = (uintptr_t)iters;
        key.v[4] = reinterpret_cast<uintptr_t>(workspace); key.v[5] = reinterpret_cast<uintptr_t>(flow_lr_out);
        key.v[6] = (uintptr_t)r->arith; key.v[7] = reinterpret_cast<uintptr_t>(r->wfused); key.v[8] = reinterpret_cast<uintptr_t>(s);
        key.v[9] = reinterpret_cast<uintptr_t>(r->wflow); key.v[10] = reinterpret_cast<uintptr_t>(r->wt[W_ZR1_DYN]); key.v[11] = reinterpret_cast<uintptr_t>(r->wproj);
        key.v[12] = reinterpret_cast<uintptr_t>(r->wou); key.v[13] = plan.ctx_supplied ? 1 : 0;
        TRY(r->graphs->run(key, s, [&c]() { return c.core(); }));
    } else TRY(c.core());
    return launch_convex_upsample(c.flow_lr, ws.ou, 4, ws.mask, P, h, w, pad_left, pad_right, pad_top, pad_bottom,
                                  flow, occl, sigma, packed, s, r->nonfinite);
}

extern "C" int mftx_raft_refine(mftx_raft *r, int P, int h, int w, int iters, const float *fmap1,
                                const float *fmap2, const float *net, const float *inp, const float *flow_init,
                                int pad_left, int pad_right, int pad_top, int pad_bottom, float *flow, float *occl,
                                float *sigma, float *packed, float *flow_lr_out, void *workspace,
                                size_t workspace_bytes, void *stream) {
    return refine_impl(r, P, h, w, iters, fmap1, fmap2, net, inp, flow_init, pad_left, pad_right, pad_top, pad_bottom, flow, occl, sigma,
                       packed, flow_lr_out, workspace, workspace_bytes, stream, nullptr);
}

extern "C" int mftx_raft_refine_gather(mftx_raft *r, int P, int h, int w, int iters, const float *const *fmap1,
                                       const float *const *fmap2, const float *const *net, const float *const *inp,
                                       const float *flow_init, int pad_left, int pad_right, int pad_top, int pad_bottom,
                                       float *flow, float *occl, float *sigma, float *packed, float *flow_lr_out,
                                       void *workspace, size_t workspace_bytes, void *stream) {
    return mftx_raft_refine_gather_ex(r, P, h, w, iters, fmap1, fmap2, net, inp, nullptr, nullptr, nullptr, flow_init, pad_left, pad_right, pad_top,
                                      pad_bottom, flow, occl, sigma, packed, flow_lr_out, workspace, workspace_bytes, stream);
}

extern "C" int mftx_raft_refine_gather_ex(mftx_raft *r, int P, int h, int w, int iters, const float *const *fmap1,
                                          const float *const *fmap2, const float *const *net, const float *const *inp,
                                          const float *const *ctx_parts, const void *const *fmap1_split, const void *fmap2_split,
                                          const float *flow_init, int pad_left, int pad_right, int pad_top, int pad_bottom,
                                          float *flow, float *occl, float *sigma, float *packed, float *flow_lr_out,
                                          void *workspace, size_t workspace_bytes, void *stream) {
    if (!r || r->magic != RAFT_MAGIC) return fail(MFTX_E_STATE, "raft_refine_gather: bad handle");
    if (!fmap1 || !fmap2 || !net || !inp) return fail(MFTX_E_ARG, "raft_refine_gather: null pointer");
    if (P < 1 || P > MFTX_MAX_GATHER) return fail(MFTX_E_ARG, "raft_refine_gather: 1 .. %d pairs", MFTX_MAX_GATHER);
    if (r->arith != MFTX_ARITH_SPLIT || r->ondemand || r->opt[MFTX_RAFT_OPT_TILE_VOLUME] == 0)
        return fail(MFTX_E_STATE, "raft_refine_gather: needs the split arithmetic with the stored, tile-resident correlation volume (use mftx_raft_refine)");
    RefineGather g{};
    g.f2_shared = true;
    for (int b = 0; b < P; ++b) {
        if (!fmap1[b] || !fmap2[b] || !net[b] || !inp[b]) return fail(MFTX_E_ARG, "raft_refine_gather: pair %d has a null map", b);
        if (!aligned16(fmap1[b]) || !aligned16(fmap2[b]) || !aligned16(net[b]) || !aligned16(inp[b])) return fail(MFTX_E_ALIGN, "raft_refine_gather: maps must be 16-byte aligned");
        g.f1.p[b] = fmap1[b]; g.f2.p[b] = fmap2[b]; g.net.p[b] = net[b]; g.inp.p[b] = inp[b];
        if (fmap2[b] != fmap2[0]) g.f2_shared = false;
    }
    if (ctx_parts) {
        for (int i = 0; i < 4 * P; ++i)
            if (!ctx_parts[i] || !aligned16(ctx_parts[i])) return fail(MFTX_E_ALIGN, "raft_refine_gather: context part %d of pair %d null or not 16-byte aligned", i & 3, i >> 2);
        g.has_ctx = true;
        for (int b = 0; b < P; ++b) for (int k = 0; k < 4; ++k) g.ctx[k].p[b] = ctx_parts[4 * b + k];
    }
    if (fmap1_split) {
        for (int b = 0; b < P; ++b) {
            if (!fmap1_split[b] || !aligned16(fmap1_split[b])) return fail(MFTX_E_ALIGN, "raft_refine_gather: split map of pair %d null or not 16-byte aligned", b);
            g.f1s.p[b] = static_cast<const float *>(fmap1_split[b]);
        }
        g.has_f1s = true;
    }
    if (fmap2_split) {
        if (!aligned16(fmap2_split)) return fail(MFTX_E_ALIGN, "raft_refine_gather: the second map's split form must be 16-byte aligned");
        if (!g.f2_shared) return fail(MFTX_E_ARG, "raft_refine_gather: a split second map goes with ONE second map for all pairs");
        g.f2s = static_cast<const float *>(fmap2_split);
    }
    return refine_impl(r, P, h, w, iters, nullptr, nullptr, nullptr, nullptr, flow_init, pad_left, pad_right, pad_top, pad_bottom, flow, occl,
                       sigma, packed, flow_lr_out, workspace, workspace_bytes, stream, &g);
}

__global__ void split_rows_kernel(const float *__restrict__ in, float *__restrict__ out, long long slots, int c4) {
    const long long i = (long long)blockIdx.x * blockDim.x + threadIdx.x;
    if (i >= slots) return;
    const long long m = i / c4;
    const int q = (int)(i - m * c4);
    store_split4v(out + m * 4 * c4, 4 * q, reinterpret_cast<const float4 *>(in)[i]);
}

extern "C" size_t mftx_raft_frame_prepare_bytes(int h, int w) {
    if (h <= 0 || w <= 0) return 0;
    return ((size_t)h * w * 128 * sizeof(float) + 255) & ~size_t(255);
}

extern "C" int mftx_raft_frame_prepare(mftx_raft *r, int h, int w, const float *fmap, const float *inp, float *ctx_zr1, float *ctx_q1,
                                       float *ctx_zr2, float *ctx_q2, void *fmap_split, void *scratch, size_t scratch_bytes, void *stream) {
    if (!r || r->magic != RAFT_MAGIC) return fail(MFTX_E_STATE, "raft_frame_prepare: bad handle");
    if (h < 16 || w < 16 || (long long)h * w > (1ll << 24)) return fail(MFTX_E_ARG, "raft_frame_prepare: bad size");
    const bool want_ctx = ctx_zr1 || ctx_q1 || ctx_zr2 || ctx_q2;
    if (!want_ctx && !fmap_split) return fail(MFTX_E_ARG, "raft_frame_prepare: nothing to write");
    if (r->arith != MFTX_ARITH_SPLIT || r->opt[MFTX_RAFT_OPT_PRESPLIT] == 0)
        return fail(MFTX_E_STATE, "raft_frame_prepare: needs the split arithmetic with split-form activations");
    hipStream_t s = (hipStream_t)stream;
    const long long N = (long long)h * w;
    if (fmap_split) {
        if (!fmap) return fail(MFTX_E_ARG, "raft_frame_prepare: a split map needs fmap");
        TRY(launch_split_weights(fmap, fmap_split, N * 256, s));
    }
    if (!want_ctx) return 0;
    if (!inp || !ctx_zr1 || !ctx_q1 || !ctx_zr2 || !ctx_q2 || !scratch) return fail(MFTX_E_ARG, "raft_frame_prepare: the context parts need inp, all four outputs and the scratch");
    if (r->opt[MFTX_RAFT_OPT_TILE_CONV] == 1)
        return fail(MFTX_E_STATE, "raft_frame_prepare: MFTX_RAFT_OPT_TILE_CONV must be pinned (0 or 2), the batch decides otherwise");
    if (!aligned16(inp) || !aligned16(ctx_zr1) || !aligned16(ctx_q1) || !aligned16(ctx_zr2) || !aligned16(ctx_q2) ||
        (reinterpret_cast<uintptr_t>(scratch) & 255))
        return fail(MFTX_E_ALIGN, "raft_frame_prepare: maps must be 16-byte and the scratch 256-byte aligned");
    if (scratch_bytes < mftx_raft_frame_prepare_bytes(h, w))
        return fail(MFTX_E_WORKSPACE, "raft_frame_prepare: scratch %zu < %zu bytes", scratch_bytes, mftx_raft_frame_prepare_bytes(h, w));
    float *inps = static_cast<float *>(scratch);
    {
        const long long slots = N * 32;
        hipLaunchKernelGGL(split_rows_kernel, dim3((unsigned)((slots + 255) / 256)), dim3(256), 0, s, inp, inps, slots, 32);
        TRY(check_launch("split_rows"));
    }
    float *const zr[2] = {ctx_zr1, ctx_zr2}, *const q[2] = {ctx_q1, ctx_q2};
    RefinePlan plan{};
    plan.SP = true; plan.tiles_on = r->opt[MFTX_RAFT_OPT_TILE_CONV] == 2;
    const RefineCall c{r, r->w, r->wg, plan, s, 1, h, w};
    return c.context_parts(inps, 128, zr, q);
}

extern "C" int mftx_volume_query_split(const float *in, void *out, long long n_floats, void *stream) {
    if (!in || !out) return fail(MFTX_E_ARG, "volume_query_split: null pointer");
    return launch_volume_query_split(in, out, n_floats, (hipStream_t)stream);
}

extern "C" int mftx_raft_graph_stats(const mftx_raft *r, unsigned long long *captures, unsigned long long *replays) {
    if (!r || r->magic != RAFT_MAGIC || !captures || !replays) return fail(MFTX_E_STATE, "raft_graph_stats: bad arguments");
    *captures = r->graphs ? r->graphs->captures : 0;
    *replays = r->graphs ? r->graphs->replays : 0;
    return 0;
}

extern "C" int mftx_corr_pyramid(const float *f1, const float *f2, int P, int C, int h, int w, float *lvl0,
                                 float *lvl1, float *lvl2, float *lvl3, void *stream) {
    if (!f1 || !f2 || !lvl0 || !lvl1 || !lvl2 || !lvl3) return fail(MFTX_E_ARG, "corr_pyramid: null pointer");
    if (P <= 0 || C <= 0 || C % 32 || h < 8 || w < 8) return fail(MFTX_E_ARG, "corr_pyramid: need C %% 32 == 0, h, w >= 8");
    if (!aligned16(f1) || !aligned16(f2)) return fail(MFTX_E_ALIGN, "corr_pyramid: features must be 16-byte aligned");
    if (!aligned16(lvl0) || !aligned16(lvl1) || !aligned16(lvl2) || !aligned16(lvl3))
        return fail(MFTX_E_ALIGN, "corr_pyramid: levels must be 16-byte aligned");
    float *const lv[4] = {lvl0, lvl1, lvl2, lvl3};
    return launch_corr_pyramid(f1, f2, P, C, h, w, lv, (hipStream_t)stream);
}

extern "C" int mftx_corr_pyramid_split(const float *f1, const float *f2, int P, int C, int h, int w, float *lvl0,
                                       float *lvl1, float *lvl2, float *lvl3, float *f2_scratch, void *stream) {
    if (!f1 || !f2 || !lvl0 || !lvl1 || !lvl2 || !lvl3 || !f2_scratch) return fail(MFTX_E_ARG, "corr_pyramid_split: null pointer");
    if (P <= 0 || C <= 0 || C % 32 || h < 8 || w < 8) return fail(MFTX_E_ARG, "corr_pyramid_split: need C %% 32 == 0, h, w >= 8");
    if (!aligned16(f1) || !aligned16(f2) || (reinterpret_cast<uintptr_t>(f2_scratch) & 31))
        return fail(MFTX_E_ALIGN, "corr_pyramid_split: features must be 16-byte aligned, the scratch 32-byte aligned");
    if (!aligned16(lvl0) || !aligned16(lvl1) || !aligned16(lvl2) || !aligned16(lvl3))
        return fail(MFTX_E_ALIGN, "corr_pyramid_split: levels must be 16-byte aligned");
    float *const lv[4] = {lvl0, lvl1, lvl2, lvl3};
    return launch_corr_pyramid(f1, f2, P, C, h, w, lv, (hipStream_t)stream, f2_scratch);
}

extern "C" int mftx_corr_pyramid_layout(int h, int w, long long *stride, int *block_grid) {
    if (h < 8 || w < 8 || !stride || !block_grid) return fail(MFTX_E_ARG, "corr_pyramid_layout: bad arguments");
    const PyramidLayout L = pyramid_layout(h, w);
    for (int l = 0; l < 4; ++l) stride[l] = L.stride[l];
// ... 155 lines not shown
```

mft_amd/csrc/volume_tile.hip:

```cpp
#include "common.h"
#include "profile.h"
#include "device_prims.h"

namespace mftx {

constexpr int VT_C = 256;
constexpr int VT_ROW = VT_C * 4 + 16;
constexpr int VT_TARGETS = 128 * VT_ROW;
constexpr int VT_LDS = VT_TARGETS + 8 * 1024;

struct VolTileArgs {
    const float *f1;
    const float *f2s;
    float *lvl0, *lvl1, *lvl2, *lvl3;
    long long s0, s1, s2, s3;
    int P, N, h, w, sbw, n_sb, wb0;
    float scale;
    int qchunks, blocks_per_chunk;
    int ablate;
    int gathered;
    long long f2_bstride;
    PairPtrs f1p;
};

// ... 123 lines not shown
        const unsigned v0off4 = (unsigned)((le >> 3) * s0b) + (unsigned)((blk0 - m) * 4) + (unsigned)(le & 7) * 16u;
        float acc2 = 0.f, acc3 = 0.f;
#pragma unroll
        for (int g = 0; g < 4; ++g) {
#ifdef MFTX_TUNING
            const bool st0g = !(p.ablate & 1);
#else
            const bool st0g = true;
#endif
            float vv[4][4];
#pragma unroll
            for (int i = 0; i < 4; ++i)
#pragma unroll
                for (int j = 0; j < 4; ++j) vv[i][j] = (acc[j][4 * g + i] + accx[j][4 * g + i] * inv2048) * p.scale;
            f32x4 line[4];
#pragma unroll
            for (int j = 0; j < 4; ++j) {
#pragma unroll
                for (int i = 0; i < 4; ++i) slab[(4 * hf + i) * 32 + m] = vv[i][j];
                line[j] = *reinterpret_cast<const f32x4 *>(slab + (le >> 3) * 32 + (le & 7) * 4);
            }
            if (st0g) {
#pragma unroll
                for (int j = 0; j < 4; ++j)
                    __builtin_amdgcn_raw_buffer_store_b128(__builtin_bit_cast(u32x4, line[j]), r0, v0off4 + (j >> 1) * jrow + (j & 1) * 128u, (unsigned)(8 * g) * s0b, 0);
            }
#pragma unroll
        for (int i = 0; i < 4; ++i) {
            const int r = 4 * g + i;
            const int qrow = q0 + 8 * (r >> 2) + 4 * hf + (r & 3);
            const bool row_ok = qrow < p.N;
#ifdef MFTX_TUNING
            const bool st1 = row_ok && !(p.ablate & 2);
#define MFTX_VT_ST23 (!(p.ablate & 10))
#else
            const bool st1 = row_ok;
#define MFTX_VT_ST23 true
#endif
            float merged = 0.f;
#pragma unroll
            for (int j = 0; j < 4; ++j) {
                const float v = vv[i][j];
                float t = v + vt_shl<1>(v);
                t = t + vt_shl<8>(v);
                t = (t + vt_shl<9>(v)) * 0.25f;
                if (j == 0) merged = t;
                else {
                    float sh = j == 1 ? vt_shr<1>(t) : (j == 2 ? vt_shr<8>(t) : vt_shr<9>(t));
                    asm volatile("" : "+v"(sh));
                    const bool take = j == 1 ? (m & 1) != 0 : (j == 2 ? ((m >> 3) & 1) && !(m & 1) : ((m >> 3) & 1) && (m & 1));
                    merged = take ? sh : merged;
                }
            }
            const float l1 = __builtin_bit_cast(float, __builtin_amdgcn_ds_bpermute(l1_src, __builtin_bit_cast(int, merged)));
            if (st1) __builtin_amdgcn_raw_buffer_store_b32(__builtin_bit_cast(unsigned, l1), r1, v1off, (unsigned)(8 * (r >> 2) + (r & 3)) * s1b, 0);
            float t2 = l1 + vt_shl<1>(l1);
            t2 = t2 + vt_shl<8>(l1);
            t2 = (t2 + vt_shl<9>(l1)) * 0.25f;
            asm volatile("" : "+v"(t2));
            {
                const float pulled = __builtin_bit_cast(float, __builtin_amdgcn_ds_bpermute(l2_pull, __builtin_bit_cast(int, t2)));
                acc2 = d2i == (r & 3) ? pulled : acc2;
                if ((r & 3) == 3) {
                    const int row2 = q0 + 8 * (r >> 2) + l2_row;
                    if (MFTX_VT_ST23 && l2_ok && row2 < p.N) p.lvl2[(qbase + row2) * p.s2 + l2_off] = acc2;
                }
            }
            const float bq = vt_shl<2>(t2);
            const float cq = __builtin_bit_cast(float, __builtin_amdgcn_ds_bpermute(l3_src, __builtin_bit_cast(int, t2)));
            const float dq = __builtin_bit_cast(float, __builtin_amdgcn_ds_bpermute(l3_src + 8, __builtin_bit_cast(int, t2)));
            float v3 = (((t2 + bq) + cq) + dq) * 0.25f;
            asm volatile("" : "+v"(v3));
            {
                const float pulled = __builtin_bit_cast(float, __builtin_amdgcn_ds_bpermute(l3_pull, __builtin_bit_cast(int, v3)));
                acc3 = d3r == r ? pulled : acc3;
                if (r == 15) {
                    const int row3 = q0 + l3_row;
                    if (MFTX_VT_ST23 && l3_ok && row3 < p.N) p.lvl3[(qbase + row3) * p.s3 + l3_off] = acc3;
                }
            }
        }
        }
    }
}

static int vt_num_cus() {
    static const int n = [] {
        int dev = 0, cus = 256;
        hipDeviceProp_t prop;
        if (hipGetDevice(&dev) == hipSuccess && hipGetDeviceProperties(&prop, dev) == hipSuccess && prop.multiProcessorCount > 0) cus = prop.multiProcessorCount;
        return cus;
    }();
    return n;
}

bool volume_tile_applicable(int C) { return C == VT_C; }

__global__ void vt_query_split_kernel(const float *__restrict__ in, uint4 *__restrict__ out, long long n8) {
    const long long i = (long long)blockIdx.x * blockDim.x + threadIdx.x;
    const float k2048 = __builtin_bit_cast(float, __builtin_amdgcn_readfirstlane(0x45000000));
    if (i >= n8) return;
    const f32x4 u = *reinterpret_cast<const f32x4 *>(in + i * 8), v = *reinterpret_cast<const f32x4 *>(in + i * 8 + 4);
    f16x8 hi, lo;
    split8(u, v, k2048, hi, lo);
    out[2 * i] = __builtin_bit_cast(uint4, hi);
    out[2 * i + 1] = __builtin_bit_cast(uint4, lo);
}

int launch_volume_query_split(const float *in, void *out, long long n, hipStream_t s) {
    if (n <= 0 || n % 8) return fail(MFTX_E_ARG, "volume_query_split: a positive multiple of 8 floats");
    if (!aligned16(in) || !aligned16(out)) return fail(MFTX_E_ALIGN, "volume_query_split: operands must be 16-byte aligned");
    const long long n8 = n / 8;
    hipLaunchKernelGGL(vt_query_split_kernel, dim3((unsigned)((n8 + 255) / 256)), dim3(256), 0, s, in, reinterpret_cast<uint4 *>(out), n8);
    return check_launch("volume_query_split");
}

int launch_volume_tile(const float *f1, const float *f2s, int P, int h, int w, float *const lvl[4], hipStream_t s, const PairPtrs *f1p, long long f2_bstride,
                       bool f1_split) {
    if (f1p && P > MFTX_MAX_GATHER) return fail(MFTX_E_ARG, "corr_pyramid: at most %d gathered pairs", MFTX_MAX_GATHER);
    const PyramidLayout L = pyramid_layout(h, w);
    VolTileArgs a{};
    a.f1 = f1; a.f2s = f2s; a.lvl0 = lvl[0]; a.lvl1 = lvl[1]; a.lvl2 = lvl[2]; a.lvl3 = lvl[3];
    a.s0 = L.stride[0]; a.s1 = L.stride[1]; a.s2 = L.stride[2]; a.s3 = L.stride[3];
    a.P = P; a.N = h * w; a.h = h; a.w = w; a.sbw = L.sbw; a.n_sb = L.sbh * L.sbw; a.wb0 = L.wb[0];
    a.scale = 1.0f / sqrtf((float)VT_C);
    a.gathered = f1p ? 1 : 0;
    if (f1p) a.f1p = *f1p;
    a.f2_bstride = f2_bstride >= 0 ? f2_bstride : (long long)a.N * VT_C;
    const int n_blocks = (a.N + 31) / 32;
    const long long base = (long long)P * a.n_sb;
    a.ablate = tune_env("MFTX_VT_ABLATE", 0);
    static const int q_forced = tune_env("MFTX_VT_QCHUNKS", 0);
    int qchunks = q_forced > 0 ? q_forced : (base * 4 >= 3LL * vt_num_cus() ? 1 : (int)((vt_num_cus() + base - 1) / base));
    if (qchunks < 1) qchunks = 1;
    if (qchunks > (n_blocks + 7) / 8) qchunks = (n_blocks + 7) / 8;
    a.blocks_per_chunk = (n_blocks + qchunks - 1) / qchunks;
    a.qchunks = (n_blocks + a.blocks_per_chunk - 1) / a.blocks_per_chunk;
    const long long wgs = base * a.qchunks;
    if (wgs > 0x7fffffffLL) return fail(MFTX_E_ARG, "corr_pyramid: too many workgroups");
    static bool attr_set = false;
    if (!attr_set) {
        if (hipFuncSetAttribute(reinterpret_cast<const void *>(volume_tile_kernel<false>), hipFuncAttributeMaxDynamicSharedMemorySize, VT_LDS) != hipSuccess ||
            hipFuncSetAttribute(reinterpret_cast<const void *>(volume_tile_kernel<true>), hipFuncAttributeMaxDynamicSharedMemorySize, VT_LDS) != hipSuccess)
            return fail(MFTX_E_STATE, "corr_pyramid: cannot reserve %d bytes of LDS", VT_LDS);
        attr_set = true;
    }
    ProfScope prof(PC_CORR_VOLUME, s, 2.0 * a.N * a.N * (double)VT_C * P);
    if (f1_split) hipLaunchKernelGGL(volume_tile_kernel<true>, dim3((unsigned)wgs), dim3(512), VT_LDS, s, a);
    else hipLaunchKernelGGL(volume_tile_kernel<false>, dim3((unsigned)wgs), dim3(512), VT_LDS, s, a);
    return check_launch("volume_tile");
}

}
```

mft_amd/ops.py:

```python
from __future__ import annotations

import ctypes as C
import math
from typing import NamedTuple

import numpy as np
import torch

from . import _lib
from ._lib import ConvDesc, MftxError, check

ACT = {None: 0, "none": 0, "relu": 1, "sigmoid": 2, "tanh": 3}


def _stream():
    return C.c_void_p(torch.cuda.current_stream().cuda_stream)


def _device_visible(t):
    return isinstance(t, torch.Tensor) and (t.is_cuda or t.is_pinned())


def copy_bytes(src: torch.Tensor, dst: torch.Tensor):
    if not (_device_visible(src) and _device_visible(dst)):
# ... 127 lines not shown
    g = lambda k: sd[f"{prefix}.{k}"].to(device=device, dtype=torch.float32)
    out = []
    for name in _ENC_CONVS:
        w, b = g(name + ".weight"), g(name + ".bias")
        bn = _bn_name(name) if batch_norm else None
        if bn is not None:
            s_ = g(bn + ".weight") / torch.sqrt(g(bn + ".running_var") + 1e-5)
            t_ = g(bn + ".bias") - g(bn + ".running_mean") * s_
            w = w * s_.reshape(-1, 1, 1, 1)
            b = b * s_ + t_
        if name == "conv1":
            w4 = torch.zeros(64, 7, 7, 4, dtype=torch.float32, device=device)
            w4[..., :3] = w.permute(0, 2, 3, 1)
            pk = torch.zeros(128, 7, 32, dtype=torch.float32, device=device)
            pk[:64, :, :28] = w4.reshape(64, 7, 28)
            out += [pk.contiguous(), b.contiguous()]
        elif name == "conv2" and batch_norm:
            out += [pack_conv_weight(w[:128].contiguous()), b[:128].contiguous(),
                    pack_conv_weight(w[128:].contiguous()), b[128:].contiguous()]
        else:
            out += [pack_conv_weight(w.contiguous()), b.contiguous()]
    return out


class EncoderEngine:

    def __init__(self, state_dict: dict, prefix: str, instance_norm: bool, device, arith=None, graph=True):
        lib = _lib.load()
        self.device = torch.device(device)
        self.instance_norm = instance_norm
        self.weights = pack_encoder_weights(state_dict, prefix, not instance_norm, self.device)
        arr, self._keep = _lib.ptr_array([_chk(t, "weight") for t in self.weights])
        handle = C.c_void_p()
        check(lib.mftx_encoder_create(arr, len(self.weights), int(instance_norm), C.byref(handle)),
              "mftx_encoder_create")
        self._h = handle
        self._ws = None
        if not graph:
            check(lib.mftx_encoder_set_graph(self._h, 0), "mftx_encoder_set_graph")
        self.arith = ARITH_SPLIT if arith is None else int(arith)
        if self.arith == ARITH_SPLIT:
            self.split = [split_weights(t) for t in self.weights[0::2]]
            sarr, self._keep_split = _lib.ptr_array([t.data_ptr() for t in self.split])
            check(lib.mftx_encoder_set_split_weights(self._h, sarr, len(self.split)), "mftx_encoder_set_split_weights")
        elif self.arith != ARITH_F32:
            raise MftxError(f"unknown arithmetic {arith!r}")

    def __del__(self):
        try:
            if getattr(self, "_h", None):
                _lib.load().mftx_encoder_destroy(self._h)
                self._h = None
        except Exception:
            pass

    def forward(self, img_u8: torch.Tensor, out=None):
        lib = _lib.load()
        H0, W0 = img_u8.shape[:2]
        h, w = -(-H0 // 8), -(-W0 // 8)
        need = lib.mftx_encoder_workspace_bytes(H0, W0)
        if self._ws is None or self._ws.numel() < need:
            self._ws = torch.empty(need, dtype=torch.uint8, device=self.device)
        if out is not None:
            outs = out
            want = ((h * w, 256), None) if self.instance_norm else ((h * w, 128), (h * w, 128))
            for t, shp in zip(outs, want):
                if shp is not None and (t is None or tuple(t.shape) != shp):
                    raise MftxError(f"encoder output must be {shp}")
        elif self.instance_norm:
            outs = (torch.empty(h * w, 256, dtype=torch.float32, device=self.device), None)
        else:
            outs = (torch.empty(h * w, 128, dtype=torch.float32, device=self.device),
                    torch.empty(h * w, 128, dtype=torch.float32, device=self.device))
        check(lib.mftx_encoder_forward(self._h, _chk(img_u8, "img", torch.uint8), H0, W0, _chk(outs[0], "out0"),
                                       _chk(outs[1], "out1") if outs[1] is not None else None,
                                       self._ws.data_ptr(), self._ws.numel(), _stream()), "mftx_encoder_forward")
        return outs


def encoder_prep(img_u8: torch.Tensor) -> torch.Tensor:
    lib = _lib.load()
    if img_u8.dim() != 3 or img_u8.shape[2] != 3:
        raise MftxError("encoder_prep: img must be [H0, W0, 3]")
    H0, W0 = int(img_u8.shape[0]), int(img_u8.shape[1])
    Hp, Wp = -(-H0 // 8) * 8, -(-W0 // 8) * 8
    out = torch.empty(Hp, Wp + 6, 4, dtype=torch.float32, device=img_u8.device)
    check(lib.mftx_encoder_prep(_chk(img_u8, "img", torch.uint8), H0, W0, out.data_ptr(), _stream()), "mftx_encoder_prep")
    return out


def instance_norm(x: torch.Tensor, mode: int, res: torch.Tensor = None, split: bool = False) -> torch.Tensor:
    lib = _lib.load()
    if x.dim() != 2:
        raise MftxError("instance_norm: x must be [rows, C]")
    rows, Cc = int(x.shape[0]), int(x.shape[1])
    if res is not None and tuple(res.shape) != (rows, Cc):
        raise MftxError("instance_norm: res must have the shape of x")
    need = lib.mftx_instance_norm_workspace_bytes(Cc)
    ws = torch.empty(max(need, 16), dtype=torch.uint8, device=x.device)
    check(lib.mftx_instance_norm(_chk(x, "x"), rows, Cc, _chk(res, "res") if res is not None else None, int(mode),
                                 int(bool(split)), ws.data_ptr(), ws.numel(), _stream()), "mftx_instance_norm")
    return x



def pyramid_layout(h: int, w: int):
    stride, grid = (C.c_longlong * 4)(), (C.c_int * 4)()
    check(_lib.load().mftx_corr_pyramid_layout(h, w, stride, grid), "mftx_corr_pyramid_layout")
    return list(stride), tuple(grid)


def _level_index(l: int, h: int, w: int, device):
    stride, (hb0, wb0, hb1, wb1) = pyramid_layout(h, w)
    hl, wl = h >> l, w >> l
    ys, xs = torch.meshgrid(torch.arange(hl, device=device), torch.arange(wl, device=device), indexing="ij")
    if l < 2:
        wb = (wb0, wb1)[l]
        idx = ((ys >> 2) * wb + (xs >> 3)) * 32 + (ys & 3) * 8 + (xs & 7)
    else:
        idx = ys * wl + xs
    return idx.reshape(-1), stride[l]


def unblock_level(t: torch.Tensor, l: int, h: int, w: int) -> torch.Tensor:
    idx, _ = _level_index(l, h, w, t.device)
    return t[..., idx].contiguous()


def block_level(t: torch.Tensor, l: int, h: int, w: int) -> torch.Tensor:
    idx, stride = _level_index(l, h, w, t.device)
    out = torch.zeros(t.shape[:-1] + (stride,), dtype=t.dtype, device=t.device)
    out[..., idx] = t
    return out


def corr_pyramid(f1: torch.Tensor, f2: torch.Tensor, h: int, w: int, arith: int = ARITH_F32):
    lib = _lib.load()
    P, N, Cc = f1.shape
    assert N == h * w and f2.shape == f1.shape
    stride, _ = pyramid_layout(h, w)
    lv = [torch.empty(P, N, stride[l], dtype=torch.float32, device=f1.device) for l in range(4)]
    if arith == ARITH_SPLIT:
        scratch = torch.empty_like(f2)
        check(lib.mftx_corr_pyramid_split(_chk(f1, "f1"), _chk(f2, "f2"), P, Cc, h, w,
                                          *[t.data_ptr() for t in lv], scratch.data_ptr(), _stream()), "mftx_corr_pyramid_split")
        return lv
    if arith != ARITH_F32:
        raise MftxError("corr_pyramid: arith must be ARITH_F32 or ARITH_SPLIT")
    check(lib.mftx_corr_pyramid(_chk(f1, "f1"), _chk(f2, "f2"), P, Cc, h, w,
                                *[t.data_ptr() for t in lv], _stream()), "mftx_corr_pyramid")
    return lv


def corr_lookup(lv, coords: torch.Tensor, h: int, w: int, r: int = 4):
    lib = _lib.load()
    P = coords.shape[0]
    stride, _ = pyramid_layout(h, w)
    for l, t in enumerate(lv):
        if tuple(t.shape) != (P, h * w, stride[l]):
            raise MftxError(f"corr_lookup: level {l} must be [{P}, {h * w}, {stride[l]}]")
    out = torch.empty(P, h * w, 324, dtype=torch.float32, device=coords.device)
    check(lib.mftx_corr_lookup(*[_chk(t, "level") for t in lv], _chk(coords, "coords"), P, h, w, r,
                               out.data_ptr(), 324, _stream()), "mftx_corr_lookup")
    return out


def pack_lookup_convc1_weights(wpk: torch.Tensor) -> torch.Tensor:
    lib = _lib.load()
    if wpk.dim() != 3 or wpk.shape[0] != 256 or wpk.shape[1] != 1 or wpk.shape[2] < 324:
        raise MftxError("pack_lookup_convc1_weights: expected the packed convc1 weight [256, 1, >= 324]")
    out = torch.empty(_lib.LOOKUP_CONVC1_WEIGHT_BYTES, dtype=torch.uint8, device=wpk.device)
    check(lib.mftx_pack_lookup_convc1_weights(_chk(wpk, "wpk"), wpk.shape[2], out.data_ptr(), _stream()),
          "mftx_pack_lookup_convc1_weights")
    return out


def pack_tile_conv_weights(wpk: torch.Tensor, N: int, cin: int, check_range: bool = True) -> torch.Tensor:
    lib = _lib.load()
    if wpk.dim() != 3 or wpk.shape[0] < N or wpk.shape[2] < cin:
        raise MftxError("pack_tile_conv_weights: expected the packed weight [>= N, taps, >= cin]")
    if check_range:
        bad = count_not_below(wpk, _lib.SPLIT_LIMIT)
        if bad:
            raise SplitRangeError(f"pack_tile_conv_weights: {bad} weights are not below {_lib.SPLIT_LIMIT} in magnitude")
    taps = wpk.shape[1]
    out = torch.empty(N * taps * cin * 4, dtype=torch.uint8, device=wpk.device)
    check(lib.mftx_pack_tile_conv_weights(_chk(wpk, "wpk"), N, taps, cin, wpk.shape[2], out.data_ptr(), _stream()),
          "mftx_pack_tile_conv_weights")
    return out


def tile_conv2d(x: torch.Tensor, wtile: torch.Tensor, bias, P, h, w, N, kh, kw, act=None, x2=None, addend=None,
                out_split=False, out=None):
    lib = _lib.load()
    if out is None:
        out = torch.empty(P * h * w, N, dtype=torch.float32, device=x.device)
    d = ConvDesc()
    d.a0, d.lda0, d.c0 = _chk(x, "x"), x.shape[1], x.shape[1]
    if x2 is not None:
        d.a1, d.lda1, d.c1 = _chk(x2, "x2"), x2.shape[1], x2.shape[1]
    else:
        d.a1, d.lda1, d.c1 = None, 0, 0
    d.wpk = None
    d.bias = _chk(bias, "bias") if bias is not None else None
    d.out, d.ldo = _chk(out, "out"), out.shape[1]
    d.P, d.h, d.w, d.N, d.kh, d.kw = P, h, w, N, kh, kw
    d.act, d.out_scale = ACT[act], 1.0
    d.addend, d.ld_addend = (_chk(addend, "addend"), addend.shape[1]) if addend is not None else (None, 0)
    d.arith, d.a_split, d.out_split = ARITH_SPLIT, 1, int(bool(out_split))
    check(lib.mftx_tile_conv2d(C.byref(d), _chk(wtile, "wtile", torch.uint8), _stream()), "mftx_tile_conv2d")
    return out


def gru_half(h_split, motion_split, wzr_tile, wq_tile, pre_zr, pre_q, hf, P, h, w, vertical=False):
    M = P * h * w
    z = torch.empty(M, 128, dtype=torch.float32, device=hf.device)
    h_out = torch.empty(M, 128, dtype=torch.float32, device=hf.device)
    hf_out = torch.empty(M, 128, dtype=torch.float32, device=hf.device)
    check(_lib.load().mftx_gru_half(_chk(h_split, "h"), h_split.shape[1], _chk(motion_split, "motion"), motion_split.shape[1],
                                    _chk(wzr_tile, "wzr", torch.uint8), _chk(wq_tile, "wq", torch.uint8), _chk(pre_zr, "pre_zr"),
                                    _chk(pre_q, "pre_q"), _chk(z, "z"), _chk(hf, "hf"), _chk(hf_out, "hf_out"), _chk(h_out, "h_out"), 128, P, h, w,
                                    1 if vertical else 0, _stream()), "mftx_gru_half")
    return hf_out, h_out, z


def pack_flow_head_weights(w2pk: torch.Tensor, check_range: bool = True) -> torch.Tensor:
    lib = _lib.load()
    if w2pk.dim() != 3 or w2pk.shape[0] < 2 or tuple(w2pk.shape[1:]) != (9, 256):
        raise MftxError("pack_flow_head_weights: expected the packed weight [>= 2, 9, 256]")
    if check_range and count_not_below(w2pk, _lib.SPLIT_LIMIT):
        raise SplitRangeError(f"pack_flow_head_weights: weights not below {_lib.SPLIT_LIMIT} in magnitude")
    out = torch.empty(_lib.FLOW_HEAD_WEIGHT_BYTES, dtype=torch.uint8, device=w2pk.device)
    check(lib.mftx_pack_flow_head_weights(_chk(w2pk, "w2pk"), out.data_ptr(), _stream()), "mftx_pack_flow_head_weights")
    return out


def pack_ou_heads_weights(w1pk: torch.Tensor, w2pk: torch.Tensor, check_range: bool = True):
    lib = _lib.load()
    if w1pk.dim() != 3 or w1pk.shape[0] < 256 or w1pk.shape[1] != 9 or w1pk.shape[2] < 712:
        raise MftxError("pack_ou_heads_weights: expected the packed first layers [>= 256, 9, >= 712]")
    if w2pk.dim() != 3 or w2pk.shape[0] < 3 or tuple(w2pk.shape[1:]) != (9, 256):
        raise MftxError("pack_ou_heads_weights: expected the packed second layers [>= 3, 9, 256]")
    if check_range and (count_not_below(w1pk, _lib.SPLIT_LIMIT) or count_not_below(w2pk, _lib.SPLIT_LIMIT)):
        raise SplitRangeError(f"pack_ou_heads_weights: weights not below {_lib.SPLIT_LIMIT} in magnitude")
    wtile = torch.empty(_lib.OU_HEADS_WTILE_BYTES, dtype=torch.uint8, device=w1pk.device)
    wproj = torch.empty(_lib.FLOW_HEAD_WEIGHT_BYTES, dtype=torch.uint8, device=w1pk.device)
    check(lib.mftx_pack_ou_heads_weights(_chk(w1pk, "w1pk"), w1pk.shape[2], _chk(w2pk, "w2pk"), wtile.data_ptr(), wproj.data_ptr(), _stream()),
          "mftx_pack_ou_heads_weights")
    return wtile, wproj


def ou_heads(a_split: torch.Tensor, h: int, w: int, wtile: torch.Tensor, b1, wproj: torch.Tensor, b2):
    lib = _lib.load()
    M = a_split.shape[0]
    P = M // (h * w)
    T = torch.empty(M, 27, dtype=torch.float32, device=a_split.device)
    out = torch.zeros(M, 4, dtype=torch.float32, device=a_split.device)
    check(lib.mftx_ou_heads(_chk(a_split, "a"), a_split.shape[1], P, h, w, _chk(wtile, "wtile", torch.uint8), _chk(b1, "b1"),
                            _chk(wproj, "wproj", torch.uint8), _chk(b2, "b2"), T.data_ptr(), out.data_ptr(), 4, _stream()), "mftx_ou_heads")
    return out


def flow_head(hsplit: torch.Tensor, h: int, w: int, wtile: torch.Tensor, b1, wproj: torch.Tensor, b2, coords=None):
    lib = _lib.load()
    M = hsplit.shape[0]
    P = M // (h * w)
    T = torch.empty(M, 18, dtype=torch.float32, device=hsplit.device)
    delta = torch.empty(M, 2, dtype=torch.float32, device=hsplit.device)
    check(lib.mftx_flow_head(_chk(hsplit, "hsplit"), hsplit.stride(0), P, h, w, _chk(wtile, "wtile", torch.uint8), _chk(b1, "b1"),
                             _chk(wproj, "wproj", torch.uint8), _chk(b2, "b2"), T.data_ptr(), delta.data_ptr(),
                             _chk(coords, "coords") if coords is not None else None, _stream()), "mftx_flow_head")
    return delta


def pack_flow_branch_weights(w98: torch.Tensor, w2pk: torch.Tensor, check_range: bool = True) -> torch.Tensor:
    lib = _lib.load()
    if tuple(w98.shape) != (98, 128) or w2pk.dim() != 3 or w2pk.shape[0] < 64 or tuple(w2pk.shape[1:]) != (9, 128):
        raise MftxError("pack_flow_branch_weights: expected convf1 as [98, 128] and convf2 as [>= 64, 9, 128]")
    if check_range:
        bad = count_not_below(w98, _lib.SPLIT_LIMIT) + count_not_below(w2pk, _lib.SPLIT_LIMIT)
        if bad:
            raise SplitRangeError(f"pack_flow_branch_weights: {bad} weights are not below {_lib.SPLIT_LIMIT} in magnitude")
    out = torch.empty(_lib.FLOW_BRANCH_WEIGHT_BYTES, dtype=torch.uint8, device=w98.device)
    check(lib.mftx_pack_flow_branch_weights(_chk(w98, "w98"), _chk(w2pk, "w2pk"), out.data_ptr(), _stream()),
          "mftx_pack_flow_branch_weights")
    return out


def flow_branch(coords: torch.Tensor, h: int, w: int, wflow: torch.Tensor, b1: torch.Tensor, b2: torch.Tensor,
                out: torch.Tensor = None, hx: torch.Tensor = None) -> torch.Tensor:
    lib = _lib.load()
    P = coords.shape[0]
    if out is None:
        out = torch.empty(P * h * w, 64, dtype=torch.float32, device=coords.device)
    check(lib.mftx_flow_branch(_chk(coords, "coords"), P, h, w, _chk(wflow, "wflow", torch.uint8), _chk(b1, "b1"),
                               _chk(b2, "b2"), out.data_ptr(), out.stride(0),
                               hx.data_ptr() if hx is not None else None, hx.stride(0) if hx is not None else 0, _stream()),
          "mftx_flow_branch")
    return out


def corr_lookup_convc1(lv, coords: torch.Tensor, h: int, w: int, wfused: torch.Tensor, bias: torch.Tensor,
                       out_split: bool = False):
    lib = _lib.load()
    P = coords.shape[0]
    stride, _ = pyramid_layout(h, w)
    for l, t in enumerate(lv):
        if tuple(t.shape) != (P, h * w, stride[l]):
            raise MftxError(f"corr_lookup_convc1: level {l} must be [{P}, {h * w}, {stride[l]}]")
    out = torch.empty(P * h * w, 256, dtype=torch.float32, device=coords.device)
    check(lib.mftx_corr_lookup_convc1(*[_chk(t, "level") for t in lv], _chk(coords, "coords"), P, h, w,
                                      _chk(wfused, "wfused", torch.uint8), _chk(bias, "bias"), out.data_ptr(), 256,
                                      int(bool(out_split)), _stream()), "mftx_corr_lookup_convc1")
    return out


def fmap_pyramid(f2: torch.Tensor, h: int, w: int):
    lib = _lib.load()
    P, N, Cc = f2.shape
    assert N == h * w
    lv = [torch.empty(P, (h >> l) * (w >> l), Cc, dtype=torch.float32, device=f2.device) for l in (1, 2, 3)]
    check(lib.mftx_fmap_pyramid(_chk(f2, "f2"), P, Cc, h, w, *[t.data_ptr() for t in lv], _stream()), "mftx_fmap_pyramid")
    return [f2] + lv


def corr_lookup_ondemand(f1: torch.Tensor, f2_levels, coords: torch.Tensor, h: int, w: int, r: int = 4):
    lib = _lib.load()
    P, N, Cc = f1.shape
    out = torch.empty(P, N, 324, dtype=torch.float32, device=f1.device)
    check(lib.mftx_corr_lookup_ondemand(_chk(f1, "f1"), *[_chk(t, "f2 level") for t in f2_levels], _chk(coords, "coords"),
                                        P, Cc, h, w, r, out.data_ptr(), 324, _stream()), "mftx_corr_lookup_ondemand")
    return out


def conv2d(x: torch.Tensor, wpk: torch.Tensor, bias, P, h, w, N, kh, kw, act=None, out_scale=1.0, x2=None,
           addend=None, stride=0, hin=0, win=0, pad_y=0, pad_x=0, residual_mode=0, arith=ARITH_F32, a_split=False,
           out_split=False, out=None, tile=None, lda0=None, c0=None):
    lib = _lib.load()
    if out is None:
        out = torch.empty(P * h * w, N, dtype=torch.float32, device=x.device)
    d = ConvDesc()
    d.a0, d.lda0, d.c0 = _chk(x, "x"), x.shape[1] if lda0 is None else int(lda0), x.shape[1] if c0 is None else int(c0)
    if x2 is not None:
        d.a1, d.lda1, d.c1 = _chk(x2, "x2"), x2.shape[1], x2.shape[1]
    else:
        d.a1, d.lda1, d.c1 = None, 0, 0
    d.wpk = _chk(wpk, "wpk")
    d.bias = _chk(bias, "bias") if bias is not None else None
    d.out, d.ldo = _chk(out, "out"), out.shape[1]
    d.P, d.h, d.w, d.N, d.kh, d.kw = P, h, w, N, kh, kw
    d.act, d.out_scale = ACT[act], out_scale
    d.addend, d.ld_addend = (_chk(addend, "addend"), addend.shape[1]) if addend is not None else (None, 0)
    d.stride, d.hin, d.win, d.pad_y, d.pad_x, d.residual_mode = stride, hin, win, pad_y, pad_x, residual_mode
    d.arith = arith
    d.a_split, d.out_split = int(bool(a_split)), int(bool(out_split))
    if tile is None:
        check(lib.mftx_conv2d(C.byref(d), _stream()), "mftx_conv2d")
    else:
        check(lib.mftx_conv2d_tile(C.byref(d), int(tile), _stream()), "mftx_conv2d_tile")
    return out


def convex_upsample(flow_lr, ou, mask, P, h, w, pads=(0, 0, 0, 0), want_packed=False):
    lib = _lib.load()
    pl, pr, pt, pb = pads
    H0, W0 = 8 * h - pt - pb, 8 * w - pl - pr
    dev = flow_lr.device
    flow = torch.empty(P, 2, H0, W0, dtype=torch.float32, device=dev)
    occl = torch.empty(P, 1, H0, W0, dtype=torch.float32, device=dev)
    sigma = torch.empty(P, 1, H0, W0, dtype=torch.float32, device=dev)
    packed = torch.empty(P, H0, W0, 4, dtype=torch.float32, device=dev) if want_packed else None
    check(lib.mftx_convex_upsample(_chk(flow_lr, "flow_lr"), _chk(ou, "ou"), ou.shape[1], _chk(mask, "mask"),
                                   P, h, w, pl, pr, pt, pb, flow.data_ptr(), occl.data_ptr(), sigma.data_ptr(),
                                   packed.data_ptr() if want_packed else None, _stream()), "mftx_convex_upsample")
    return (flow, occl, sigma, packed) if want_packed else (flow, occl, sigma)


def _planes(res, H, W):
    flow, occl, sigma = res
    if flow.shape != (2, H, W) or occl.shape != (1, H, W) or sigma.shape != (1, H, W):
        raise MftxError("FlowOU planes must be [2,H,W], [1,H,W], [1,H,W]")
    return _chk(flow, "flow"), _chk(occl, "occlusion"), _chk(sigma, "sigma")


def _new_result(H, W, device):
    return (torch.empty(2, H, W, dtype=torch.float32, device=device),
            torch.empty(1, H, W, dtype=torch.float32, device=device),
            torch.empty(1, H, W, dtype=torch.float32, device=device))


def chain(L, R):
    lib = _lib.load()
    _, H, W = L[0].shape
    out = _new_result(H, W, L[0].device)
    check(lib.mftx_chain(*_planes(L, H, W), *_planes(R, H, W), H, W, *[t.data_ptr() for t in out], _stream()),
          "mftx_chain")
    return out


def warp_backward(flow, img):
    lib = _lib.load()
    Cc, H, W = img.shape
    if flow.shape != (2, H, W):
        raise MftxError("warp_backward: flow must be [2,H,W] matching img")
    out = torch.empty_like(img)
    check(lib.mftx_warp_backward(_chk(flow, "flow"), _chk(img, "img"), Cc, H, W, out.data_ptr(), _stream()),
          "mftx_warp_backward")
    return out


def select(cands, thr, want_chosen=False):
    lib = _lib.load()
    K = len(cands)
    _, H, W = cands[0][0].shape
    cols = list(zip(*[_planes(c, H, W) for c in cands]))
    arrs = [_lib.ptr_array(list(c)) for c in cols]
    out = _new_result(H, W, cands[0][0].device)
    chosen = torch.empty(H, W, dtype=torch.int8, device=out[0].device) if want_chosen else None
    check(lib.mftx_select(K, arrs[0][0], arrs[1][0], arrs[2][0], float(thr), H, W, *[t.data_ptr() for t in out],
                          chosen.data_ptr() if want_chosen else None, _stream()), "mftx_select")
    return out + (chosen,)


def chain_select(Ls, Rs, thr, want_chosen=False):
    lib = _lib.load()
    K = len(Ls)
    assert len(Rs) == K
    _, H, W = Ls[0][0].shape
    lcols = list(zip(*[_planes(c, H, W) for c in Ls]))
    rcols = list(zip(*[_planes(c, H, W) for c in Rs]))
    arrs = [_lib.ptr_array(list(c)) for c in lcols + rcols]
    out = _new_result(H, W, Ls[0][0].device)
    chosen = torch.empty(H, W, dtype=torch.int8, device=out[0].device) if want_chosen else None
    check(lib.mftx_chain_select(K, *[a[0] for a in arrs], float(thr), H, W, *[t.data_ptr() for t in out],
                                chosen.data_ptr() if want_chosen else None, _stream()), "mftx_chain_select")
    return out + (chosen,)


def chain_select_packed(Ls, Rs, thr, want_chosen=False):
    lib = _lib.load()
    K = len(Ls)
    assert len(Rs) == K
    _, H, W = Ls[0][0].shape
    lcols = list(zip(*[_planes(c, H, W) for c in Ls]))
    for r in Rs:
        if tuple(r.shape) != (H, W, 4):
            raise MftxError("packed FlowOU must be [H, W, 4]")
    arrs = [_lib.ptr_array(list(c)) for c in lcols] + [_lib.ptr_array([_chk(r, "packed") for r in Rs])]
    out = _new_result(H, W, Ls[0][0].device)
    chosen = torch.empty(H, W, dtype=torch.int8, device=out[0].device) if want_chosen else None
# ... 378 lines not shown
    if xy.dim() != 2 or int(xy.shape[1]) != 2:
        raise MftxError("trackstore_locate_frames: xy must be [N, 2]")
    N = int(xy.shape[0])
    which = np.asarray(point_frame, dtype=np.int64).reshape(-1)
    if int(which.shape[0]) != N or (N and (which.min() < 0 or which.max() >= len(pptr))):
        raise MftxError("trackstore_locate_frames: point_frame must be N indices into frames")
    if tuple(table.shape) != (N, 4) or tuple(cell.shape) != (N,):
        raise MftxError("trackstore_locate_frames: the table must be [N, 4], cell [N]")
    xp, tp, cp = _chk(xy, "xy"), _chk(table, "table"), _chk(cell, "cell", torch.int32)
    if N == 0:
        return table, cell
    buf, G, off = locate_tables(which, pptr, lptr, 1, H * W * 8)
    tables = torch.from_numpy(buf).pin_memory().to(xy.device, non_blocking=True)
    keys = torch.empty(N, dtype=torch.int64, device=xy.device)
    base = tables.data_ptr()
    check(lib.mftx_trackstore_locate(base + off[0], base + off[1], base + off[2], G, base + off[3], base + off[4], H, W, N, xp,
                                     float(occlusion_threshold), keys.data_ptr(), tp, cp, _stream()), "mftx_trackstore_locate")
    return table, cell


TRACKSTORE_ATLAS_ENTRIES = 256
TRACKSTORE_ATLAS_CELLS = 1 << 24


def trackstore_invert_atlas(frames, first_of, rank_of, table, cell, entry, occlusion_threshold=0.5):
    lib = _lib.load()
    frames = list(frames)
    first_of = np.asarray(first_of, dtype=np.int64).reshape(-1)
    rank_of = np.asarray(rank_of, dtype=np.int64).reshape(-1)
    G, J = int(first_of.shape[0]) - 1, len(frames)
    if table.dim() != 4 or int(table.shape[3]) != 4 or int(table.shape[0]) != G or tuple(cell.shape) != tuple(table.shape[:3]) \
            or tuple(entry.shape) != tuple(table.shape[:3]):
        raise MftxError("trackstore_invert_atlas: the table must be [G, H, W, 4], cell and entry [G, H, W], first_of [G + 1]")
    H, W = int(table.shape[1]), int(table.shape[2])
    if G < 0 or int(rank_of.shape[0]) != J or first_of[0] != 0 or first_of[-1] != J or (np.diff(first_of) < 0).any():
        raise MftxError("trackstore_invert_atlas: first_of must ascend from 0 to the number of frames, rank_of name every frame")
    if G and np.diff(first_of).max() > TRACKSTORE_ATLAS_ENTRIES:
        raise MftxError(f"trackstore_invert_atlas: more than {TRACKSTORE_ATLAS_ENTRIES} entries in a plane")
    if (H - 1) * (W - 1) > TRACKSTORE_ATLAS_CELLS:
        raise MftxError("trackstore_invert_atlas: more than 2^24 cells")
    tp, cp, ep = _chk(table, "table"), _chk(cell, "cell", torch.int32), _chk(entry, "entry", torch.int32)
    if J:
        fH, fW, pptr, lptr = _trackstore_frame_ptrs(frames, "trackstore_invert_atlas")
        if (fH, fW) != (H, W):
            raise MftxError("trackstore_invert_atlas: the frames must be of the table's H x W")
    else:
        pptr = lptr = np.zeros(0, np.int64)
    if G == 0:
        return table, cell, entry
    n32 = (G + 1) + J
    buf = np.zeros(2 * J + (n32 + 1) // 2, np.int64)
    buf[0:J], buf[J:2 * J] = pptr, lptr
    tail = buf[2 * J:].view(np.int32)
    tail[0:G + 1], tail[G + 1:G + 1 + J] = first_of, rank_of
    tables = torch.from_numpy(buf).pin_memory().to(table.device, non_blocking=True)
    keys = torch.empty(G * H * W, dtype=torch.int64, device=table.device)
    base = tables.data_ptr()
    check(lib.mftx_trackstore_invert_atlas(base if J else None, base + 8 * J if J else None, base + 16 * J,
                                           base + 16 * J + 4 * (G + 1) if J else None, G, J, H, W, float(occlusion_threshold),
                                           keys.data_ptr(), tp, cp, ep, _stream()), "mftx_trackstore_invert_atlas")
    return table, cell, entry


class RaftEngine:

    GEMM_SLOTS = (0, 2, 6, 8, 10, 11, 13, 14, 16, 17, 19, 20, 22, 26, 28, 30)

    OPTIONS = {"fork": 0, "presplit": 1, "group": 2, "fuse_lookup": 3, "graph": 4, "fuse_flow": 5, "tile_conv": 6, "fuse_head": 7, "tile_volume": 8, "fuse_gru": 9, "tile_cells": 10, "fuse_ou": 11, "tile_conv2p": 12}
    TILE_SLOTS = {2: (192, 256), 8: (128, 256), 10: (256, 256), 11: (256, 128), 13: (128, 256), 14: (128, 128), 16: (256, 256),
                  17: (256, 128), 19: (128, 256), 20: (128, 128), 22: (256, 128), 26: (256, 128)}

    def __init__(self, state_dict: dict, device, ondemand_corr=False, arith=ARITH_SPLIT, options=None):
        lib = _lib.load()
        self.device = torch.device(device)
        self.weights = pack_raft_weights(state_dict, self.device)
        arr, self._keep = _lib.ptr_array([_chk(t, "weight") for t in self.weights])
        handle = C.c_void_p()
        check(lib.mftx_raft_create(arr, len(self.weights), C.byref(handle)), "mftx_raft_create")
        self._h = handle
        self._ws = None
        self.arith = int(arith)
        if self.arith == ARITH_SPLIT:
            self.split = [split_weights(t) if i in self.GEMM_SLOTS else None for i, t in enumerate(self.weights)]
            sarr, self._keep_split = _lib.ptr_array([t.data_ptr() if t is not None else None for t in self.split])
            check(lib.mftx_raft_set_split_weights(self._h, sarr, len(self.split)), "mftx_raft_set_split_weights")
            self.wfused = pack_lookup_convc1_weights(self.weights[0])
            check(lib.mftx_raft_set_lookup_fused(self._h, self.wfused.data_ptr()), "mftx_raft_set_lookup_fused")
            self.wflow = pack_flow_branch_weights(self.weights[4], self.weights[6])
            check(lib.mftx_raft_set_flow_fused(self._h, self.wflow.data_ptr()), "mftx_raft_set_flow_fused")
            self.wtile = [pack_tile_conv_weights(t, *self.TILE_SLOTS[i]) if i in self.TILE_SLOTS else None
                          for i, t in enumerate(self.weights)]
            tarr, self._keep_tile = _lib.ptr_array([t.data_ptr() if t is not None else None for t in self.wtile])
            check(lib.mftx_raft_set_tile_weights(self._h, tarr, len(self.wtile)), "mftx_raft_set_tile_weights")
            self.wproj = pack_flow_head_weights(self.weights[24])
            check(lib.mftx_raft_set_flow_head(self._h, self.wproj.data_ptr()), "mftx_raft_set_flow_head")
            self.wou, self.wouproj = pack_ou_heads_weights(self.weights[30], self.weights[32])
            check(lib.mftx_raft_set_ou_heads(self._h, self.wou.data_ptr(), self.wouproj.data_ptr()), "mftx_raft_set_ou_heads")
        elif self.arith != ARITH_F32:
            raise MftxError(f"unknown arithmetic {arith!r}")
        self._nonfinite = torch.zeros(4, dtype=torch.int32, device=self.device)
        check(lib.mftx_raft_set_nonfinite_counter(self._h, self._nonfinite.data_ptr()), "mftx_raft_set_nonfinite_counter")
        options = dict(options or {})
        self._gather = bool(options.pop("gather", 1))
        for k, v in options.items():
            self.set_option(k, v)
        self.ondemand_corr = bool(ondemand_corr)
        if self.ondemand_corr:
            check(lib.mftx_raft_set_ondemand(self._h, 1), "mftx_raft_set_ondemand")

    def __del__(self):
        try:
            if getattr(self, "_h", None):
                _lib.load().mftx_raft_destroy(self._h)
                self._h = None
        except Exception:
            pass

    def debug_refine(self, fmap1, fmap2, net, inp, h, w, iters, pads=(0, 0, 0, 0), flow_init=None):
        lib = _lib.load()
        P = fmap1.shape[0]
        M = P * h * w
        trace = torch.empty(iters + 1, M, 2, dtype=torch.float32, device=self.device)
        check(lib.mftx_raft_set_coords_trace(self._h, trace.data_ptr()), "mftx_raft_set_coords_trace")
        try:
            out = self.refine(fmap1, fmap2, net, inp, h, w, iters, pads=pads, flow_init=flow_init)
        finally:
            check(lib.mftx_raft_set_coords_trace(self._h, None), "mftx_raft_set_coords_trace")
        if self.ondemand_corr:
            pyramid = None
        else:
            stride, _ = pyramid_layout(h, w)
            pyramid = []
            for l in range(4):
                lvl = self.region(f"lvl{l}", P, h, w, stride[l]).reshape(P, h * w, stride[l])
                pyramid.append(unblock_level(lvl, l, h, w).reshape(M, 1, h >> l, w >> l).cpu())
        to_map = lambda t: t.reshape(P, h, w, 2).permute(0, 3, 1, 2).contiguous().cpu()
        ys, xs = torch.meshgrid(torch.arange(h, dtype=torch.float32), torch.arange(w, dtype=torch.float32), indexing="ij")
        debug = {"costvolume_pyramid": pyramid,
                 "coords_left": torch.stack([xs, ys])[None].repeat(P, 1, 1, 1),
                 "iterations": [{"coords": to_map(trace[i])} for i in range(iters + 1)]}
        return out, debug

    PLAN_FIELDS = ("presplit", "fuse_lookup", "tiles_on", "gru_fused", "ctx_supplied", "two_pass", "flow", "pair_second", "head_fused",
                   "defer_update", "ou_fused", "ou_materialised", "use_graph", "side_stream")
    FLOW_SCHEDULES = ("fused", "side", "first", "after_lookup", "with_lookup")

    def plan(self, P, h, w, ctx_supplied=False):
        out = (C.c_int * len(self.PLAN_FIELDS))()
        check(_lib.load().mftx_raft_plan(self._h, P, h, w, int(bool(ctx_supplied)), out, len(out)), "mftx_raft_plan")
        plan = {k: bool(v) for k, v in zip(self.PLAN_FIELDS, out)}
        plan["flow"] = self.FLOW_SCHEDULES[out[self.PLAN_FIELDS.index("flow")]]
        return plan

    def graph_stats(self):
        c, r = C.c_ulonglong(), C.c_ulonglong()
        check(_lib.load().mftx_raft_graph_stats(self._h, C.byref(c), C.byref(r)), "mftx_raft_graph_stats")
        return int(c.value), int(r.value)

    def nonfinite_count(self, reset=False):
        n = int(self._nonfinite[0].item())
        if reset and n:
            self._nonfinite.zero_()
        return n

    def nonfinite_snapshot(self, host_words):
        copy_bytes(self._nonfinite, host_words)

    def set_option(self, name, value):
        if name not in self.OPTIONS:
            raise MftxError(f"unknown engine option {name!r} (known: {', '.join(sorted(self.OPTIONS))}, gather)")
        check(_lib.load().mftx_raft_set_option(self._h, self.OPTIONS[name], int(value)), "mftx_raft_set_option")
        if name == "tile_conv":
            self._tile_conv = int(value)
        if name == "tile_volume":
            self._tile_volume = int(value)

    def workspace(self, P, h, w):
        need = _lib.load().mftx_raft_workspace_bytes_for(self._h, P, h, w)
        if self._ws is None or self._ws.numel() < need:
            if self._ws is not None:
                check(_lib.load().mftx_raft_clear_graphs(self._h), "mftx_raft_clear_graphs")
            self._ws = torch.empty(need, dtype=torch.uint8, device=self.device)
        return self._ws

    REGIONS = ("lvl0", "lvl1", "lvl2", "lvl3", "coords1", "corr", "cor1", "corflo", "flo1", "hx", "z", "rh", "fh",
               "delta", "mask", "ouin", "ouh", "ou", "flow_lr")

    SPLIT_REGIONS = {"cor1": 256, "corflo": 256, "flo1": 128, "hx": 384, "rh": 128, "ouin": 712}

    def region(self, name, P, h, w, cols, split=None):
        offs = (C.c_size_t * 19)()
        check(_lib.load().mftx_raft_workspace_layout_for(self._h, P, h, w, offs, 19), "mftx_raft_workspace_layout_for")
        off = offs[self.REGIONS.index(name)]
        M = P * h * w
        if split is None:
            split = self.arith == ARITH_SPLIT and name in self.SPLIT_REGIONS and self.plan(P, h, w)["presplit"]
        if split:
            ld = self.SPLIT_REGIONS.get(name, cols)
            raw = self._ws[off: off + 4 * M * ld].view(torch.float32).reshape(M, ld)
            return unsplit_activations(raw)[:, :cols]
        return self._ws[off: off + 4 * M * cols].view(torch.float32).reshape(M, cols)

    MAX_GATHER = 16

    def can_gather(self, P):
        return (self.arith == ARITH_SPLIT and not self.ondemand_corr and P <= self.MAX_GATHER and
                getattr(self, "_tile_volume", 1) != 0 and getattr(self, "_gather", True))

    def prepare_frame(self, fmap, inp, h, w, context=True, split=True):
        lib = _lib.load()
        N = h * w
        dev = self.device
        ctx = fsplit = scratch = None
        if context:
            ctx = tuple(torch.empty(N, c, dtype=torch.float32, device=dev) for c in (256, 128, 256, 128))
            scratch = torch.empty(lib.mftx_raft_frame_prepare_bytes(h, w), dtype=torch.uint8, device=dev)
        if split:
            fsplit = torch.empty(N, 256, dtype=torch.float32, device=dev)
        cp = [t.data_ptr() for t in ctx] if context else [None] * 4
        check(lib.mftx_raft_frame_prepare(self._h, h, w, _chk(fmap, "fmap") if split else None, _chk(inp, "inp") if context else None,
                                          *cp, fsplit.data_ptr() if split else None,
                                          scratch.data_ptr() if context else None, scratch.numel() if context else 0, _stream()),
              "mftx_raft_frame_prepare")
        return ctx, fsplit

    def refine(self, fmap1, fmap2, net, inp, h, w, iters, pads=(0, 0, 0, 0), want_flow_lr=False, flow_init=None,
               packed=None, planar=True, prepared=None):
        lib = _lib.load()
        gathered = isinstance(fmap1, (list, tuple))
        P = len(fmap1) if gathered else fmap1.shape[0]
        pl, pr, pt, pb = pads
        H0, W0 = 8 * h - pt - pb, 8 * w - pl - pr
        dev = self.device
        if not planar and packed is None:
            raise MftxError("refine: planar=False needs a packed output")
        flow = torch.empty(P, 2, H0, W0, dtype=torch.float32, device=dev) if planar else None
        occl = torch.empty(P, 1, H0, W0, dtype=torch.float32, device=dev) if planar else None
        sigma = torch.empty(P, 1, H0, W0, dtype=torch.float32, device=dev) if planar else None
        flow_lr = torch.empty(P, h * w, 2, dtype=torch.float32, device=dev) if want_flow_lr else None
        if flow_init is not None and tuple(flow_init.shape) != (P, h * w, 2):
            raise MftxError("flow_init must be [P, h*w, 2]")
        if packed is not None and tuple(packed.shape) != (P, H0, W0, 4):
            raise MftxError("packed must be [P, H0, W0, 4]")
        ws = self.workspace(P, h, w)

        def tail():
            return (_chk(flow_init, "flow_init") if flow_init is not None else None, pl, pr, pt, pb,
                    flow.data_ptr() if planar else None, occl.data_ptr() if planar else None, sigma.data_ptr() if planar else None,
                    _chk(packed, "packed") if packed is not None else None, flow_lr.data_ptr() if want_flow_lr else None,
                    ws.data_ptr(), ws.numel(), _stream())

        if gathered:
            if not self.can_gather(P) or not (len(fmap2) == len(net) == len(inp) == P):
                raise MftxError("refine: per-pair map lists need the split arithmetic with the tile-resident volume and P <= 16")
            arrs = [_lib.ptr_array([_chk(t, "map") for t in lst]) for lst in (fmap1, fmap2, net, inp)]
            maps = [a[0] for a in arrs]
            if prepared:
                ctx, f1s, f2s = prepared.get("ctx"), prepared.get("f1s"), prepared.get("f2s")
                if (ctx is not None and len(ctx) != P) or (f1s is not None and len(f1s) != P):
                    raise MftxError("refine: prepared parts for every pair, or none")
                carr = _lib.ptr_array([_chk(t, "context part") for parts in ctx for t in parts]) if ctx is not None else (None, None)
                sarr = _lib.ptr_array([_chk(t, "split map") for t in f1s]) if f1s is not None else (None, None)
                check(lib.mftx_raft_refine_gather_ex(self._h, P, h, w, iters, *maps, carr[0], sarr[0],
                                                     _chk(f2s, "split map") if f2s is not None else None, *tail()),
                      "mftx_raft_refine_gather_ex")
            else:
                check(lib.mftx_raft_refine_gather(self._h, P, h, w, iters, *maps, *tail()), "mftx_raft_refine_gather")
        elif prepared:
            raise MftxError("refine: prepared parts go with per-pair map lists")
        else:
            check(lib.mftx_raft_refine(self._h, P, h, w, iters, _chk(fmap1, "fmap1"), _chk(fmap2, "fmap2"),
                                       _chk(net, "net"), _chk(inp, "inp"), *tail()), "mftx_raft_refine")
        return (flow, occl, sigma, flow_lr) if want_flow_lr else (flow, occl, sigma)
```

Baseline: 194.3 frames/s.

## Cache zero-flow motion-branch output per shape and pipeline flow-branch stage-one MFMAs

When no flow_init is given, the first iteration's motion-encoder input is pure zero flow. Its output then depends only on weights and shape. The engine computes that block once per shape, stores it with an event, and broadcasts it into the output and hx buffers, instead of running the flow branch for that iteration. The change also software-pipelines the first conv stage of the flow branch: it loads A rows for the next cell group while the current MFMAs and the previous epilogue run, using double-buffered accumulators. It pads the LDS shifted-copy stride to reduce bank conflicts and hoists the b2 bias load ahead of a barrier. New entry points expose a flow-branch-with-update variant and a standalone volume_tile call. The cache must be invalidated whenever any weights or options change, and it adds a graph-key field.

```diff
diff --git a/include/mftx.h b/include/mftx.h
--- a/include/mftx.h
+++ b/include/mftx.h
@@ -44,6 +44,9 @@
 int mftx_pack_flow_branch_weights(const float *w98, const float *w2pk, void *wflow, void *stream);
 int mftx_flow_branch(const float *coords, int P, int h, int w, const void *wflow, const float *b1, const float *b2,
                      float *out, int ld_out, float *hx, int ld_hx, void *stream);
+int mftx_flow_branch_update(const float *coords, int P, int h, int w, const void *wflow, const float *b1, const float *b2,
+                            float *out, int ld_out, float *hx, int ld_hx, const float *T, const float *b2h, float *coords_out,
+                            float *delta_out, void *stream);
 
 int mftx_fmap_pyramid(const float *f2, int P, int C, int h, int w, float *lvl1, float *lvl2, float *lvl3, void *stream);
 int mftx_corr_lookup_ondemand(const float *f1, const float *f2l0, const float *f2l1, const float *f2l2, const float *f2l3,
@@ -116,7 +119,11 @@
 #define MFTX_RAFT_OPT_FUSE_OU 11
 #define MFTX_RAFT_OPT_TILE_CONV2P 12
 int mftx_raft_set_option(mftx_raft *r, int option, int value);
+int mftx_raft_set_zero_flow_cache(mftx_raft *r, int on);
 #define MFTX_RAFT_PLAN_FIELDS 14
+#define MFTX_RAFT_PLAN_FIELDS_EX 15
+#define MFTX_RAFT_PLAN_CTX_SUPPLIED 1
+#define MFTX_RAFT_PLAN_FLOW_INIT 2
 #define MFTX_FLOW_FUSED 0
 #define MFTX_FLOW_SIDE 1
 #define MFTX_FLOW_FIRST 2
@@ -150,6 +157,8 @@
                                float *flow, float *occl, float *sigma, float *packed, float *flow_lr_out,
                                void *workspace, size_t workspace_bytes, void *stream);
 int mftx_volume_query_split(const float *in, void *out, long long n_floats, void *stream);
+int mftx_volume_tile(const float *const *f1, int f1_split, const void *f2s, long long f2_stride, int P, int h, int w, float *lvl0, float *lvl1,
+                     float *lvl2, float *lvl3, void *stream);
 
 typedef struct mftx_encoder mftx_encoder;
 int mftx_encoder_create(const float *const *weights, int n_weights, int instance_norm, mftx_encoder **out);
diff --git a/mft_amd/_lib.py b/mft_amd/_lib.py
--- a/mft_amd/_lib.py
+++ b/mft_amd/_lib.py
@@ -67,6 +67,9 @@
     "mftx_flow_branch": (C.c_int, [C.c_void_p, C.c_int, C.c_int, C.c_int, C.c_void_p, C.c_void_p, C.c_void_p, C.c_void_p,
                                    C.c_int, C.c_void_p, C.c_int, C.c_void_p]),
     "mftx_raft_set_option": (C.c_int, [C.c_void_p, C.c_int, C.c_int]),
+    "mftx_raft_set_zero_flow_cache": (C.c_int, [C.c_void_p, C.c_int]),
+    "mftx_flow_branch_update": (C.c_int, [C.c_void_p, C.c_int, C.c_int, C.c_int, C.c_void_p, C.c_void_p, C.c_void_p, C.c_void_p,
+                                          C.c_int, C.c_void_p, C.c_int, C.c_void_p, C.c_void_p, C.c_void_p, C.c_void_p, C.c_void_p]),
     "mftx_raft_plan": (C.c_int, [C.c_void_p, C.c_int, C.c_int, C.c_int, C.c_int, C.POINTER(C.c_int), C.c_int]),
     "mftx_raft_set_coords_trace": (C.c_int, [C.c_void_p, C.c_void_p]),
     "mftx_gru_half": (C.c_int, [C.c_void_p, C.c_int, C.c_void_p, C.c_int, C.c_void_p, C.c_void_p, C.c_void_p, C.c_void_p, C.c_void_p, C.c_void_p,
@@ -103,6 +106,8 @@
     "mftx_raft_frame_prepare_bytes": (C.c_size_t, [C.c_int, C.c_int]),
     "mftx_raft_frame_prepare": (C.c_int, [C.c_void_p, C.c_int, C.c_int] + [C.c_void_p] * 8 + [C.c_size_t, C.c_void_p]),
     "mftx_volume_query_split": (C.c_int, [C.c_void_p, C.c_void_p, C.c_longlong, C.c_void_p]),
+    "mftx_volume_tile": (C.c_int, [C.c_void_p, C.c_int, C.c_void_p, C.c_longlong, C.c_int, C.c_int, C.c_int, C.c_void_p, C.c_void_p,
+                                   C.c_void_p, C.c_void_p, C.c_void_p]),
     "mftx_encoder_create": (C.c_int, [_PP, C.c_int, C.c_int, C.POINTER(C.c_void_p)]),
     "mftx_encoder_destroy": (None, [C.c_void_p]),
     "mftx_encoder_set_graph": (C.c_int, [C.c_void_p, C.c_int]),
diff --git a/mft_amd/csrc/flow_branch.hip b/mft_amd/csrc/flow_branch.hip
--- a/mft_amd/csrc/flow_branch.hip
+++ b/mft_amd/csrc/flow_branch.hip
@@ -10,8 +10,9 @@
 constexpr int FB_CELL = 528;
 constexpr int FB_FCOLS = 26;
 constexpr int FB_FROW = 28;
+constexpr int FB_FCOPY = 2 * 16 * FB_FROW + 20;
 constexpr int FB_OFF_FLOW = 192 * FB_CELL;
-constexpr int FB_FLOW_BYTES = 4 * 2 * 16 * FB_FROW * 4;
+constexpr int FB_FLOW_BYTES = 4 * FB_FCOPY * 4;
 constexpr int FB_RED_ROW = 68;
 constexpr int FB_LDS = 4 * 128 * FB_RED_ROW * 4;
 static_assert(FB_OFF_FLOW + FB_FLOW_BYTES <= FB_LDS, "stage 3 is the largest user of LDS");
@@ -109,12 +110,12 @@
 #pragma unroll
         for (int sft = 0; sft < 4; ++sft) {
             if (c >= sft) {
-                fsp[((sft * 2 + 0) * 16 + r) * FB_FROW + c - sft] = hw;
-                fsp[((sft * 2 + 1) * 16 + r) * FB_FROW + c - sft] = lw;
+                fsp[sft * FB_FCOPY + r * FB_FROW + c - sft] = hw;
+                fsp[sft * FB_FCOPY + (16 + r) * FB_FROW + c - sft] = lw;
             }
             if (c >= FB_FCOLS - 4 && c - sft + 4 < FB_FROW) {
-                fsp[((sft * 2 + 0) * 16 + r) * FB_FROW + c - sft + 4] = 0u;
-                fsp[((sft * 2 + 1) * 16 + r) * FB_FROW + c - sft + 4] = 0u;
+                fsp[sft * FB_FCOPY + r * FB_FROW + c - sft + 4] = 0u;
+                fsp[sft * FB_FCOPY + (16 + r) * FB_FROW + c - sft + 4] = 0u;
             }
         }
     }
@@ -124,52 +125,74 @@
 
     const float inv2048 = 1.f / 2048.f;
     {
-#pragma unroll 1
-        for (int mi = 0; mi < 3; ++mi) {
-            const int i = (wv >> 2) + 2 * mi;
-            const int m = 32 * i + (lane & 31), mc = m < FB_HCELLS ? m : FB_HCELLS - 1;
-            const int ry = mc / FB_HW, rx = mc - ry * FB_HW;
+        u32x4 ahw[7], alw[7];
+        f32x16 acc1[2], accx1[2];
+        auto cell_of = [&](int mi, int &m, int &ry, int &rx) {
+            m = 32 * ((wv >> 2) + 2 * mi) + (lane & 31);
+            const int mc = m < FB_HCELLS ? m : FB_HCELLS - 1;
+            ry = mc / FB_HW; rx = mc - ry * FB_HW;
+        };
+        const unsigned padmask = (lane >> 5) ? 0u : 0xffffffffu;
+        auto read_a1 = [&](int mi, int g) {
+            int m, ry, rx;
+            cell_of(mi, m, ry, rx);
             const int c0 = rx + 4 * (lane >> 5), sft = c0 & 3;
-            const unsigned char *arow = lds + FB_OFF_FLOW + (((sft * 2) * 16 + ry) * FB_FROW + (c0 - sft)) * 4;
-            const unsigned padmask = (lane >> 5) ? 0u : 0xffffffffu;
-            f32x16 acc1, accx1;
-#pragma unroll
-            for (int r = 0; r < 16; ++r) { acc1[r] = 0.f; accx1[r] = 0.f; }
-            u32x4 ahw[7], alw[7];
-#pragma unroll
-            for (int g = 0; g < 7; ++g) {
-                ahw[g] = *reinterpret_cast<const u32x4 *>(arow + g * FB_FROW * 4);
-                alw[g] = *reinterpret_cast<const u32x4 *>(arow + (16 + g) * FB_FROW * 4);
-            }
-#pragma unroll
-            for (int g = 0; g < 7; ++g) {
-                ahw[g][3] &= padmask;
-                alw[g][3] &= padmask;
-                const f16x8 ah = __builtin_bit_cast(f16x8, ahw[g]), al = __builtin_bit_cast(f16x8, alw[g]);
-                acc1 = mfma_f16(w1h[g], ah, acc1);
-                accx1 = mfma_f16(w1l[g], ah, accx1);
-                accx1 = mfma_f16(w1h[g], al, accx1);
-            }
-            FB_T(4);
+            const unsigned char *arow = lds + FB_OFF_FLOW + (sft * FB_FCOPY + ry * FB_FROW + (c0 - sft)) * 4;
+            ahw[g] = *reinterpret_cast<const u32x4 *>(arow + g * FB_FROW * 4);
+            alw[g] = *reinterpret_cast<const u32x4 *>(arow + (16 + g) * FB_FROW * 4);
+        };
+        auto mfma_row = [&](int g, int set) {
+            ahw[g][3] &= padmask;
+            alw[g][3] &= padmask;
+            const f16x8 ah = __builtin_bit_cast(f16x8, ahw[g]), al = __builtin_bit_cast(f16x8, alw[g]);
+            acc1[set] = mfma_f16(w1h[g], ah, acc1[set]);
+            accx1[set] = mfma_f16(w1l[g], ah, accx1[set]);
+            accx1[set] = mfma_f16(w1h[g], al, accx1[set]);
+        };
+        auto epilogue = [&](int mi, int b) {
+            int m, ry, rx;
+            cell_of(mi, m, ry, rx);
+            const int set = mi & 1;
             const int yy = y0 - 1 + ry, xx = x0 - 1 + rx;
             const unsigned keep = (m < FB_HCELLS && yy >= 0 && yy < p.h && xx >= 0 && xx < p.w) ? 0xffffffffu : 0u;
             unsigned char *cellp = lds + m * FB_CELL + (4 * j1) * 32 + (lane >> 5) * 8;
+            float v[4];
+#pragma unroll
+            for (int e = 0; e < 4; ++e) {
+                const float t = acc1[set][4 * b + e] + accx1[set][4 * b + e] * inv2048 + bias1[b][e];
+                v[e] = (t + __builtin_fabsf(t)) * 0.5f;
+            }
+            unsigned h0, l0, h1, l1;
+            split_pair(v[0], v[1], k2048, h0, l0);
+            split_pair(v[2], v[3], k2048, h1, l1);
+            *reinterpret_cast<uint2 *>(cellp + b * 32) = make_uint2(h0 & keep, h1 & keep);
+            *reinterpret_cast<uint2 *>(cellp + b * 32 + 16) = make_uint2(l0 & keep, l1 & keep);
+        };
+        auto clear = [&](int set) {
+#pragma unroll
+            for (int r = 0; r < 16; ++r) { acc1[set][r] = 0.f; accx1[set][r] = 0.f; }
+        };
+#pragma unroll
+        for (int g = 0; g < 7; ++g) read_a1(0, g);
+        __builtin_amdgcn_sched_barrier(0);
+#pragma unroll
+        for (int mi = 0; mi < 3; ++mi) {
+            clear(mi & 1);
 #pragma unroll
             for (int b = 0; b < 4; ++b) {
-                float v[4];
-#pragma unroll
-                for (int e = 0; e < 4; ++e) {
-                    const float t = acc1[4 * b + e] + accx1[4 * b + e] * inv2048 + bias1[b][e];
-                    v[e] = (t + __builtin_fabsf(t)) * 0.5f;
+#pragma unroll
+                for (int g = 2 * b; g < 2 * b + 2 && g < 7; ++g) {
+                    mfma_row(g, mi & 1);
+                    if (mi + 1 < 3) read_a1(mi + 1, g);
                 }
-                unsigned h0, l0, h1, l1;
-                split_pair(v[0], v[1], k2048, h0, l0);
-                split_pair(v[2], v[3], k2048, h1, l1);
-                *reinterpret_cast<uint2 *>(cellp + b * 32) = make_uint2(h0 & keep, h1 & keep);
-                *reinterpret_cast<uint2 *>(cellp + b * 32 + 16) = make_uint2(l0 & keep, l1 & keep);
-            }
-            FB_T(5);
-        }
+                if (mi > 0) epilogue(mi - 1, b);
+                __builtin_amdgcn_sched_barrier(0);
+            }
+            FB_T(4);
+        }
+#pragma unroll
+        for (int b = 0; b < 4; ++b) epilogue(2, b);
+        FB_T(5);
     }
     lds_barrier();
     FB_T(6);
@@ -232,6 +255,7 @@
             for (int e = 0; e < 4; ++e) v[e] = acc[i][4 * b + e] + accx[i][4 * b + e] * inv2048;
             *reinterpret_cast<f32x4 *>(red + (kq * 128 + 32 * i + (lane & 31)) * FB_RED_ROW + 32 * nt + 8 * b + 4 * (lane >> 5)) = v;
         }
+    const f32x4 bu = *reinterpret_cast<const f32x4 *>(p.b2 + 8 * (tid & 7)), bv = *reinterpret_cast<const f32x4 *>(p.b2 + 8 * (tid & 7) + 4);
     FB_T(8);
     lds_barrier();
     FB_T(9);
@@ -246,7 +270,6 @@
             u += *reinterpret_cast<const f32x4 *>(src + q * 128 * FB_RED_ROW);
             v += *reinterpret_cast<const f32x4 *>(src + q * 128 * FB_RED_ROW + 4);
         }
-        const f32x4 bu = *reinterpret_cast<const f32x4 *>(p.b2 + 8 * g8), bv = *reinterpret_cast<const f32x4 *>(p.b2 + 8 * g8 + 4);
 #pragma unroll
         for (int e = 0; e < 4; ++e) { u[e] = relu_keep_nan(u[e] + bu[e]); v[e] = relu_keep_nan(v[e] + bv[e]); }
         f16x8 hi, lo;
@@ -333,3 +356,10 @@
 }
 
 }
+
+extern "C" int mftx_flow_branch_update(const float *coords, int P, int h, int w, const void *wflow, const float *b1, const float *b2,
+                                       float *out, int ld_out, float *hx, int ld_hx, const float *T, const float *b2h, float *coords_out,
+                                       float *delta_out, void *stream) {
+    if (!T) return mftx::fail(MFTX_E_ARG, "flow_branch_update: null pointer");
+    return mftx::launch_flow_branch(coords, P, h, w, wflow, b1, b2, out, ld_out, hx, ld_hx, (hipStream_t)stream, T, b2h, coords_out, delta_out);
+}
diff --git a/mft_amd/csrc/raft_engine.hip b/mft_amd/csrc/raft_engine.hip
--- a/mft_amd/csrc/raft_engine.hip
+++ b/mft_amd/csrc/raft_engine.hip
@@ -96,6 +96,19 @@
         flow_lr[2 * (long long)m + 1] = fy;
     } else v = reinterpret_cast<const float4 *>(hx + (long long)m * 384 + 256)[q - 146];
     reinterpret_cast<float4 *>(ouin + (long long)m * 712)[q] = v;
+}
+
+__global__ __launch_bounds__(256) void zero_flow_broadcast_kernel(const uint4 *__restrict__ block, float *out, int ld_out, float *hx, int ld_hx,
+                                                                  int N, int P) {
+    const int i = (int)(blockIdx.x * blockDim.x + threadIdx.x);
+    if (i >= N * 16) return;
+    const int n = i >> 4, q = i & 15;
+    const uint4 v = block[i];
+    for (int b = 0; b < P; ++b) {
+        const long long cell = (long long)b * N + n;
+        reinterpret_cast<uint4 *>(out + cell * ld_out)[q] = v;
+        if (q < 2) *reinterpret_cast<unsigned *>(reinterpret_cast<char *>(hx + cell * ld_hx) + split_row_offset(382) + 16 * q) = 0u;
+    }
 }
 
 enum WeightSlot {
@@ -179,7 +192,20 @@
     int opt[13] = { -1,  1,  1,  1,  1,  1,  1,
                     1,  1,  1,  0,  1,  1};
     unsigned *nonfinite = nullptr;
+    struct ZeroFlow { int h, w; float *block; hipEvent_t ev; hipStream_t made_on; bool done; };
+    static constexpr int ZERO_FLOW_SHAPES = 4;
+    ZeroFlow zero_flow[ZERO_FLOW_SHAPES] = {};
+    int zero_flow_n = 0;
+    int zero_flow_on = 1;
 };
+static void clear_caches(mftx_raft *r) {
+    if (r->graphs) r->graphs->clear();
+    for (int i = 0; i < r->zero_flow_n; ++i) {
+        (void)hipEventDestroy(r->zero_flow[i].ev);
+        (void)hipFree(r->zero_flow[i].block);
+    }
+    r->zero_flow_n = 0;
+}
 static_assert(MFTX_RAFT_OPT_TILE_CONV2P == 12, "mftx_raft::opt lists one default per option");
 static constexpr int GEMM_SLOTS[] = {W_CONVC1, W_CONVC2, W_CONVF2, W_CONV, W_ZR1_DYN, W_ZR1_INP, W_Q1_DYN, W_Q1_INP,
                                      W_ZR2_DYN, W_ZR2_INP, W_Q2_DYN, W_Q2_INP, W_FH1, W_MASK0, W_MASK2, W_OU1};
@@ -205,6 +231,7 @@
         if (r->ev_fork) (void)hipEventDestroy(r->ev_fork);
         if (r->ev_join) (void)hipEventDestroy(r->ev_join);
         if (r->side) (void)hipStreamDestroy(r->side);
+        clear_caches(r);
         delete r->graphs;
         delete r;
     }
@@ -227,13 +254,13 @@
 extern "C" int mftx_raft_set_ondemand(mftx_raft *r, int on) {
     if (!r || r->magic != RAFT_MAGIC) return fail(MFTX_E_STATE, "raft_set_ondemand: bad handle");
     r->ondemand = on ? 1 : 0;
-    if (r->graphs) r->graphs->clear();
+    clear_caches(r);
     return 0;
 }
 
 extern "C" int mftx_raft_set_split_weights(mftx_raft *r, const void *const *split, int n) {
     if (!r || r->magic != RAFT_MAGIC) return fail(MFTX_E_STATE, "raft_set_split_weights: bad handle");
-    if (r->graphs) r->graphs->clear();
+    clear_caches(r);
     if (!split) {
         for (int i = 0; i < W_COUNT; ++i) r->wg[i] = r->w[i];
         r->arith = MFTX_ARITH_F32;
@@ -253,7 +280,7 @@
     if (!r || r->magic != RAFT_MAGIC) return fail(MFTX_E_STATE, "raft_set_lookup_fused: bad handle");
     if (wfused && !aligned16(wfused)) return fail(MFTX_E_ALIGN, "raft_set_lookup_fused: weights not 16-byte aligned");
     r->wfused = wfused;
-    if (r->graphs) r->graphs->clear();
+    clear_caches(r);
     return 0;
 }
 
@@ -261,13 +288,13 @@
     if (!r || r->magic != RAFT_MAGIC) return fail(MFTX_E_STATE, "raft_set_flow_fused: bad handle");
     if (wflow && !aligned16(wflow)) return fail(MFTX_E_ALIGN, "raft_set_flow_fused: weights not 16-byte aligned");
     r->wflow = wflow;
-    if (r->graphs) r->graphs->clear();
+    clear_caches(r);
     return 0;
 }
 
 extern "C" int mftx_raft_set_tile_weights(mftx_raft *r, const void *const *tile, int n) {
     if (!r || r->magic != RAFT_MAGIC) return fail(MFTX_E_STATE, "raft_set_tile_weights: bad handle");
-    if (r->graphs) r->graphs->clear();
+    clear_caches(r);
     if (!tile) { for (int i = 0; i < W_COUNT; ++i) r->wt[i] = nullptr; return 0; }
     if (n != W_COUNT) return fail(MFTX_E_ARG, "raft_set_tile_weights: expected %d slots, got %d", (int)W_COUNT, n);
     for (int i = 0; i < W_COUNT; ++i)
@@ -280,7 +307,7 @@
     if (!r || r->magic != RAFT_MAGIC) return fail(MFTX_E_STATE, "raft_set_flow_head: bad handle");
     if (wproj && !aligned16(wproj)) return fail(MFTX_E_ALIGN, "raft_set_flow_head: weights not 16-byte aligned");
     r->wproj = wproj;
-    if (r->graphs) r->graphs->clear();
+    clear_caches(r);
     return 0;
 }
 
@@ -289,7 +316,7 @@
     if ((wtile == nullptr) != (wproj == nullptr)) return fail(MFTX_E_ARG, "raft_set_ou_heads: both weight streams, or neither");
     if (wtile && (!aligned16(wtile) || !aligned16(wproj))) return fail(MFTX_E_ALIGN, "raft_set_ou_heads: weights not 16-byte aligned");
     r->wou = wtile; r->wouproj = wproj;
-    if (r->graphs) r->graphs->clear();
+    clear_caches(r);
     return 0;
 }
 
@@ -301,7 +328,7 @@
 
 extern "C" int mftx_raft_clear_graphs(mftx_raft *r) {
     if (!r || r->magic != RAFT_MAGIC) return fail(MFTX_E_STATE, "raft_clear_graphs: bad handle");
-    if (r->graphs) r->graphs->clear();
+    clear_caches(r);
     return 0;
 }
 
@@ -316,7 +343,14 @@
     if (!r || r->magic != RAFT_MAGIC) return fail(MFTX_E_STATE, "raft_set_option: bad handle");
     if (option < 0 || option > MFTX_RAFT_OPT_TILE_CONV2P) return fail(MFTX_E_ARG, "raft_set_option: unknown option %d", option);
     r->opt[option] = value;
-    if (r->graphs) r->graphs->clear();
+    clear_caches(r);
+    return 0;
+}
+
+extern "C" int mftx_raft_set_zero_flow_cache(mftx_raft *r, int on) {
+    if (!r || r->magic != RAFT_MAGIC) return fail(MFTX_E_STATE, "raft_set_zero_flow_cache: bad handle");
+    r->zero_flow_on = on ? 1 : 0;
+    clear_caches(r);
     return 0;
 }
 
@@ -356,9 +390,10 @@
     FlowSchedule flow;
     bool pair_second;
     bool head_fused, defer_update, ou_fused, ou_materialised, use_graph, side_stream;
+    bool zero_flow_cached;
 };
 
-static RefinePlan refine_plan(const mftx_raft &r, int P, int h, int w, bool gather_has_ctx, bool prof, bool trace) {
+static RefinePlan refine_plan(const mftx_raft &r, int P, int h, int w, bool gather_has_ctx, bool prof, bool trace, bool has_flow_init) {
     const int *opt = r.opt;
     const bool split = r.arith == MFTX_ARITH_SPLIT, ondemand = r.ondemand != 0;
     RefinePlan p{};
@@ -385,16 +420,19 @@
     p.ou_materialised = !p.ou_fused || opt[MFTX_RAFT_OPT_FUSE_OU] == 2;
     p.use_graph = r.graphs && opt[MFTX_RAFT_OPT_GRAPH] != 0 && !prof && !trace && !ondemand;
     p.side_stream = split && fork != 0;
+    p.zero_flow_cached = p.flow == FLOW_FUSED && !has_flow_init && r.zero_flow_on != 0;
     return p;
 }
 
 extern "C" int mftx_raft_plan(const mftx_raft *r, int P, int h, int w, int ctx_supplied, int *out, int n) {
     if (!r || r->magic != RAFT_MAGIC) return fail(MFTX_E_STATE, "raft_plan: bad handle");
     if (P <= 0 || h <= 0 || w <= 0) return fail(MFTX_E_ARG, "raft_plan: need P, h, w >= 1");
-    if (!out || n != MFTX_RAFT_PLAN_FIELDS) return fail(MFTX_E_ARG, "raft_plan: need %d slots", MFTX_RAFT_PLAN_FIELDS);
-    const RefinePlan p = refine_plan(*r, P, h, w, ctx_supplied != 0, prof_enabled(), r->coords_trace != nullptr);
-    const int v[MFTX_RAFT_PLAN_FIELDS] = {p.SP, p.fuse_lookup, p.tiles_on, p.gru_fused, p.ctx_supplied, p.two_pass, (int)p.flow, p.pair_second,
-                                          p.head_fused, p.defer_update, p.ou_fused, p.ou_materialised, p.use_graph, p.side_stream};
+    if (!out || (n != MFTX_RAFT_PLAN_FIELDS && n != MFTX_RAFT_PLAN_FIELDS_EX))
+        return fail(MFTX_E_ARG, "raft_plan: need %d or %d slots", MFTX_RAFT_PLAN_FIELDS, MFTX_RAFT_PLAN_FIELDS_EX);
+    const RefinePlan p = refine_plan(*r, P, h, w, (ctx_supplied & MFTX_RAFT_PLAN_CTX_SUPPLIED) != 0, prof_enabled(), r->coords_trace != nullptr,
+                                     (ctx_supplied & MFTX_RAFT_PLAN_FLOW_INIT) != 0);
+    const int v[MFTX_RAFT_PLAN_FIELDS_EX] = {p.SP, p.fuse_lookup, p.tiles_on, p.gru_fused, p.ctx_supplied, p.two_pass, (int)p.flow, p.pair_second,
+                                             p.head_fused, p.defer_update, p.ou_fused, p.ou_materialised, p.use_graph, p.side_stream, p.zero_flow_cached};
     for (int i = 0; i < n; ++i) out[i] = v[i];
     return 0;
 }
@@ -416,6 +454,7 @@
     const float *lv[4];
     const float *fmap1, *f2lv[4];
     float *flow_lr;
+    const float *zero_flow = nullptr;
 
     mftx_conv_desc conv_desc(Seg a0, Seg a1, const float *wpk, const float *bias, Out out, int kh, int kw, int act) const {
         mftx_conv_desc d{};
@@ -512,7 +551,7 @@
             TRY(launch_conv(gemm(conv_desc(Seg{ws.corr, ws.ld_corr, ws.ld_corr}, Seg{}, G[W_CONVC1], W[B_CONVC1], Out{ws.cor1, 256, 256}, 1, 1, ACT_RELU), false, true), s));
         return conv256(W_CONVC2, W[B_CONVC2], ws.cor1, Out{ws.corflo, 256, 192}, pair);
     }
-    int motion_encoder(Coords &x, bool last) const {
+    int motion_encoder(Coords &x, bool first, bool last) const {
         const int strips = cdiv(w, F1_CELLS);
         const ConvF1Args f1{x.cur, W[W_CONVF1], W[B_CONVF1], ws.flo1, ws.hx, h, w, strips, P * h * strips, plan.SP ? 1 : 0};
         const int f1_blocks = cdiv(f1.n_strips, 2);
@@ -520,7 +559,12 @@
         const mftx_conv_desc f2 = gemm(conv_desc(Seg{ws.flo1, 128, 128}, Seg{}, G[W_CONVF2], W[B_CONVF2], flo, 3, 3, ACT_RELU), true, true);
         switch (plan.flow) {
         case FLOW_FUSED:
-            if (x.pending) {
+            if (first && zero_flow) {
+                ProfScope prof(PC_GLUE, s, 0);
+                hipLaunchKernelGGL(zero_flow_broadcast_kernel, dim3((unsigned)cdiv(h * w * 16, 256)), dim3(256), 0, s, reinterpret_cast<const uint4 *>(zero_flow),
+                                   flo.p, flo.ld, ws.hx, 384, h * w, P);
+                TRY(check_launch("zero_flow_broadcast"));
+            } else if (x.pending) {
                 TRY(launch_flow_branch(x.cur, P, h, w, r->wflow, W[B_CONVF1], W[B_CONVF2], flo.p, flo.ld, ws.hx, 384, s, ws.fh, W[B_FH2], x.alt, ws.delta));
                 x = Coords{x.alt, x.cur, false};
             } else TRY(launch_flow_branch(x.cur, P, h, w, r->wflow, W[B_CONVF1], W[B_CONVF2], flo.p, flo.ld, ws.hx, 384, s));
@@ -617,7 +661,7 @@
             const bool last = (it == iters - 1);
             if (trace && hipMemcpyAsync(trace + it * n, x.cur, n * 4, hipMemcpyDeviceToDevice, s) != hipSuccess)
                 return fail(MFTX_E_STATE, "raft_refine: coords trace copy failed");
-            TRY(motion_encoder(x, last));
+            TRY(motion_encoder(x, it == 0, last));
             TRY(gru());
             TRY(flow_head(x, last));
         }
@@ -626,6 +670,42 @@
         return final_heads(x.cur);
     }
 };
+
+static int zero_flow_block(mftx_raft *r, int h, int w, const float *grid, hipStream_t s, const float **block) {
+    *block = nullptr;
+    mftx_raft::ZeroFlow *z = nullptr;
+    for (int i = 0; i < r->zero_flow_n; ++i)
+        if (r->zero_flow[i].h == h && r->zero_flow[i].w == w) z = &r->zero_flow[i];
+    if (z && !z->done) {
+        if (hipEventQuery(z->ev) == hipSuccess) z->done = true;
+        else (void)hipGetLastError();
+    }
+    if (z && (z->done || z->made_on == s)) { *block = z->block; return 0; }
+    hipStreamCaptureStatus st = hipStreamCaptureStatusNone;
+    if (s != nullptr && (hipStreamIsCapturing(s, &st) != hipSuccess || st != hipStreamCaptureStatusNone)) { (void)hipGetLastError(); return 0; }
+    if (z) {
+        if (hipStreamWaitEvent(s, z->ev, 0) != hipSuccess) return fail(MFTX_E_STATE, "raft_refine: cannot wait for the zero-flow block");
+        *block = z->block;
+        return 0;
+    }
+    if (r->zero_flow_n == mftx_raft::ZERO_FLOW_SHAPES) clear_caches(r);
+    mftx_raft::ZeroFlow n{h, w, nullptr, nullptr, s, false};
+    if (hipMalloc(reinterpret_cast<void **>(&n.block), (size_t)h * w * 64 * sizeof(float)) != hipSuccess) {
+        (void)hipGetLastError();
+        return fail(MFTX_E_WORKSPACE, "raft_refine: no memory for the zero-flow block (%d x %d cells)", h, w);
+    }
+    int rc = hipEventCreateWithFlags(&n.ev, hipEventDisableTiming) == hipSuccess ? 0 : fail(MFTX_E_STATE, "raft_refine: zero-flow event");
+    if (!rc) rc = launch_flow_branch(grid, 1, h, w, r->wflow, r->w[B_CONVF1], r->w[B_CONVF2], n.block, 64, nullptr, 0, s);
+    if (!rc && hipEventRecord(n.ev, s) != hipSuccess) rc = fail(MFTX_E_STATE, "raft_refine: zero-flow event");
+    if (rc) {
+        if (n.ev) (void)hipEventDestroy(n.ev);
+        (void)hipFree(n.block);
+        return rc;
+    }
+    r->zero_flow[r->zero_flow_n++] = n;
+    *block = n.block;
+    return 0;
+}
 
 static int refine_impl(mftx_raft *r, int P, int h, int w, int iters, const float *fmap1, const float *fmap2, const float *net,
                        const float *inp, const float *flow_init, int pad_left, int pad_right, int pad_top, int pad_bottom, float *flow, float *occl,
@@ -642,7 +722,7 @@
         return fail(MFTX_E_ALIGN, "raft_refine: inputs must be 16-byte and the workspace 256-byte aligned");
     if (pad_left < 0 || pad_right < 0 || pad_top < 0 || pad_bottom < 0 || pad_left + pad_right >= 8 || pad_top + pad_bottom >= 8)
         return fail(MFTX_E_ARG, "raft_refine: bad padding");
-    const RefinePlan plan = refine_plan(*r, P, h, w, gather && gather->has_ctx, prof_enabled(), r->coords_trace != nullptr);
+    RefinePlan plan = refine_plan(*r, P, h, w, gather && gather->has_ctx, prof_enabled(), r->coords_trace != nullptr, flow_init != nullptr);
     const Workspace ws = carve(workspace, P, h, w, r->ondemand != 0, r->arith == MFTX_ARITH_SPLIT);
     if (ws.bytes > workspace_bytes)
         return fail(MFTX_E_WORKSPACE, "raft_refine: workspace %zu < %zu bytes", workspace_bytes, ws.bytes);
@@ -653,10 +733,12 @@
         if (own) { s = own; proxied = true; }
     }
     struct Leave { GraphCache *g; hipStream_t caller; bool on; ~Leave() { if (on) g->proxy.leave(caller); } } leave{r->graphs, caller, proxied};
-    const RefineCall c{r, r->w, r->wg, plan, s, P, h, w, iters, ws, {ws.lvl[0], ws.lvl[1], ws.lvl[2], ws.lvl[3]},
-                       fmap1, {fmap2, ws.f2l[0], ws.f2l[1], ws.f2l[2]}, flow_lr_out ? flow_lr_out : ws.flow_lr};
+    RefineCall c{r, r->w, r->wg, plan, s, P, h, w, iters, ws, {ws.lvl[0], ws.lvl[1], ws.lvl[2], ws.lvl[3]},
+                 fmap1, {fmap2, ws.f2l[0], ws.f2l[1], ws.f2l[2]}, flow_lr_out ? flow_lr_out : ws.flow_lr};
     TRY(c.volume(fmap2, gather));
     TRY(c.init_state(net, inp, flow_init, gather));
+    if (plan.zero_flow_cached) TRY(zero_flow_block(r, h, w, ws.coords1, s, &c.zero_flow));
+    if (!c.zero_flow) c.plan.zero_flow_cached = plan.zero_flow_cached = false;
     if (plan.use_graph) {
         if (plan.side_stream) TRY(ensure_side_stream(r));
         GraphKey key{};
@@ -665,6 +747,7 @@
         key.v[6] = (uintptr_t)r->arith; key.v[7] = reinterpret_cast<uintptr_t>(r->wfused); key.v[8] = reinterpret_cast<uintptr_t>(s);
         key.v[9] = reinterpret_cast<uintptr_t>(r->wflow); key.v[10] = reinterpret_cast<uintptr_t>(r->wt[W_ZR1_DYN]); key.v[11] = reinterpret_cast<uintptr_t>(r->wproj);
         key.v[12] = reinterpret_cast<uintptr_t>(r->wou); key.v[13] = plan.ctx_supplied ? 1 : 0;
+        key.v[14] = reinterpret_cast<uintptr_t>(c.zero_flow);
         TRY(r->graphs->run(key, s, [&c]() { return c.core(); }));
     } else TRY(c.core());
     return launch_convex_upsample(c.flow_lr, ws.ou, 4, ws.mask, P, h, w, pad_left, pad_right, pad_top, pad_bottom,
diff --git a/mft_amd/csrc/volume_tile.hip b/mft_amd/csrc/volume_tile.hip
--- a/mft_amd/csrc/volume_tile.hip
+++ b/mft_amd/csrc/volume_tile.hip
@@ -299,3 +299,21 @@
 }
 
 }
+
+extern "C" int mftx_volume_tile(const float *const *f1, int f1_split, const void *f2s, long long f2_stride, int P, int h, int w, float *lvl0, float *lvl1,
+                                float *lvl2, float *lvl3, void *stream) {
+    using namespace mftx;
+    if (!f1 || !f2s || !lvl0 || !lvl1 || !lvl2 || !lvl3) return fail(MFTX_E_ARG, "volume_tile: null pointer");
+    if (P < 1 || P > MFTX_MAX_GATHER || h < 8 || w < 8 || f2_stride < 0) return fail(MFTX_E_ARG, "volume_tile: 1 .. %d pairs, h, w >= 8", MFTX_MAX_GATHER);
+    if ((long long)h * w * VT_C * 4 > 0x7fffffffLL) return fail(MFTX_E_ARG, "volume_tile: feature map exceeds 2 GiB");
+    if (f2_stride != 0 && f2_stride < (long long)h * w * VT_C) return fail(MFTX_E_ARG, "volume_tile: the pairs' target maps overlap");
+    PairPtrs pp{};
+    for (int b = 0; b < P; ++b) {
+        if (!f1[b] || !aligned16(f1[b])) return fail(MFTX_E_ALIGN, "volume_tile: query map %d null or not 16-byte aligned", b);
+        pp.p[b] = f1[b];
+    }
+    if (!aligned16(f2s) || (f2_stride & 3) || !aligned16(lvl0) || !aligned16(lvl1) || !aligned16(lvl2) || !aligned16(lvl3))
+        return fail(MFTX_E_ALIGN, "volume_tile: operands must be 16-byte aligned");
+    float *const lv[4] = {lvl0, lvl1, lvl2, lvl3};
+    return launch_volume_tile(nullptr, static_cast<const float *>(f2s), P, h, w, lv, (hipStream_t)stream, &pp, f2_stride, f1_split != 0);
+}
diff --git a/mft_amd/ops.py b/mft_amd/ops.py
--- a/mft_amd/ops.py
+++ b/mft_amd/ops.py
@@ -303,6 +303,21 @@
     return lv
 
 
+def volume_tile(f1, f2s: torch.Tensor, h: int, w: int, f1_split: bool = False):
+    lib = _lib.load()
+    P, N = len(f1), h * w
+    shared = f2s.dim() == 2
+    if tuple(f2s.shape) != ((N, 256) if shared else (P, N, 256)) or any(tuple(t.shape) != (N, 256) for t in f1):
+        raise MftxError("volume_tile: maps must be [h*w, 256]")
+    stride, _ = pyramid_layout(h, w)
+    lv = [torch.empty(P, N, stride[l], dtype=torch.float32, device=f2s.device) for l in range(4)]
+    arr, keep = _lib.ptr_array([_chk(t, "query map") for t in f1])
+    check(lib.mftx_volume_tile(arr, int(bool(f1_split)), _chk(f2s, "f2s"), 0 if shared else N * 256, P, h, w,
+                               *[t.data_ptr() for t in lv], _stream()), "mftx_volume_tile")
+    del keep
+    return lv
+
+
 def corr_lookup(lv, coords: torch.Tensor, h: int, w: int, r: int = 4):
     lib = _lib.load()
     P = coords.shape[0]
@@ -439,14 +454,23 @@
 
 
 def flow_branch(coords: torch.Tensor, h: int, w: int, wflow: torch.Tensor, b1: torch.Tensor, b2: torch.Tensor,
-                out: torch.Tensor = None, hx: torch.Tensor = None) -> torch.Tensor:
+                out: torch.Tensor = None, hx: torch.Tensor = None, update=None):
     lib = _lib.load()
     P = coords.shape[0]
     if out is None:
         out = torch.empty(P * h * w, 64, dtype=torch.float32, device=coords.device)
+    hxp, ldhx = (hx.data_ptr(), hx.stride(0)) if hx is not None else (None, 0)
+    if update is not None:
+        T, b2h = update
+        if tuple(T.shape) != (P * h * w, 18):
+            raise MftxError("flow_branch: the pending update must be [P*h*w, 18]")
+        coords_out, delta = torch.empty_like(coords), torch.empty_like(coords)
+        check(lib.mftx_flow_branch_update(_chk(coords, "coords"), P, h, w, _chk(wflow, "wflow", torch.uint8), _chk(b1, "b1"),
+                                          _chk(b2, "b2"), out.data_ptr(), out.stride(0), hxp, ldhx, _chk(T, "T"), _chk(b2h, "b2h"),
+                                          coords_out.data_ptr(), delta.data_ptr(), _stream()), "mftx_flow_branch_update")
+        return out, coords_out, delta
     check(lib.mftx_flow_branch(_chk(coords, "coords"), P, h, w, _chk(wflow, "wflow", torch.uint8), _chk(b1, "b1"),
-                               _chk(b2, "b2"), out.data_ptr(), out.stride(0),
-                               hx.data_ptr() if hx is not None else None, hx.stride(0) if hx is not None else 0, _stream()),
+                               _chk(b2, "b2"), out.data_ptr(), out.stride(0), hxp, ldhx, _stream()),
           "mftx_flow_branch")
     return out
 
@@ -1131,6 +1155,11 @@
         plan["flow"] = self.FLOW_SCHEDULES[out[self.PLAN_FIELDS.index("flow")]]
         return plan
 
+    def zero_flow_cached(self, P, h, w, flow_init=False):
+        out = (C.c_int * (len(self.PLAN_FIELDS) + 1))()
+        check(_lib.load().mftx_raft_plan(self._h, P, h, w, 2 if flow_init else 0, out, len(out)), "mftx_raft_plan")
+        return bool(out[len(self.PLAN_FIELDS)])
+
     def graph_stats(self):
         c, r = C.c_ulonglong(), C.c_ulonglong()
         check(_lib.load().mftx_raft_graph_stats(self._h, C.byref(c), C.byref(r)), "mftx_raft_graph_stats")
@@ -1146,6 +1175,9 @@
         copy_bytes(self._nonfinite, host_words)
 
     def set_option(self, name, value):
+        if name == "zero_flow_cache":
+            check(_lib.load().mftx_raft_set_zero_flow_cache(self._h, int(value)), "mftx_raft_set_zero_flow_cache")
+            return
         if name not in self.OPTIONS:
             raise MftxError(f"unknown engine option {name!r} (known: {', '.join(sorted(self.OPTIONS))}, gather)")
         check(_lib.load().mftx_raft_set_option(self._h, self.OPTIONS[name], int(value)), "mftx_raft_set_option")
```

Result: no change. 194.9 frames/s, median of 6 (+0.3%).
